# Nobita421/signature-Gan

Hardware: AMD Instinct MI355X
Metric: signature images/sec (G+D train step, bs64 64x64 z=100) (higher is better)
Workload: dtype f32; 1 GPU; configs[1]: reference conv G/D 64x64x1, z=100, batch 64 per GPU, f32, n_critic=1; global_batch=64, parallelism=dp1

## Files before the change

include/siggan.h:

```cpp
#ifndef SIGGAN_H
#define SIGGAN_H

#include <stddef.h>
#include <stdint.h>

#ifdef __cplusplus
extern "C" {
#endif

#define SIGGAN_ABI_VERSION 4

enum {
    SIGGAN_OK = 0,
    SIGGAN_E_INVALID = -1,
    SIGGAN_E_STATE = -2,
    SIGGAN_E_HIP = -3,
    SIGGAN_E_NOMEM = -4
};

typedef struct siggan_ctx siggan_ctx;

typedef struct siggan_config {
    int32_t device;
    int32_t latent_dim;
    int32_t image_size;
    int32_t image_channels;
    int32_t max_batch;
    float   dropout;
    float   leaky_slope;
    uint64_t seed;
    int32_t dtype;
    float   f16_grad_scale;
    int32_t spectral_norm;
    float   g_leaky_slope;
} siggan_config;
enum { SIGGAN_DTYPE_F32 = 0, SIGGAN_DTYPE_BF16 = 1, SIGGAN_DTYPE_F16 = 2 };

typedef struct siggan_storage {
    float *g_params, *g_grads, *g_exp_avg, *g_exp_avg_sq, *g_adam_steps;
    float *g_bn_running_mean, *g_bn_running_var;
    int64_t *g_bn_batches;
    float *d_params, *d_grads, *d_exp_avg, *d_exp_avg_sq, *d_adam_steps;
    float *d_sn_u, *d_sn_v;
} siggan_storage;

typedef struct siggan_hyper {
    double lr, beta1, beta2, eps;
    float label_smoothing;
    float clip_max_norm;
    float grad_scale;
} siggan_hyper;

enum {
    SIGGAN_M_D_LOSS = 0, SIGGAN_M_D_LOSS_REAL, SIGGAN_M_D_LOSS_FAKE, SIGGAN_M_D_REAL_MEAN,
    SIGGAN_M_D_FAKE_MEAN, SIGGAN_M_D_REAL_ACC, SIGGAN_M_D_FAKE_ACC, SIGGAN_M_D_GRAD_NORM,
    SIGGAN_M_G_LOSS, SIGGAN_M_G_FAKE_MEAN, SIGGAN_M_G_GRAD_NORM,
    SIGGAN_M_D_SKIPPED, SIGGAN_M_G_SKIPPED,
    SIGGAN_M_COUNT = 16
};

int siggan_abi_version(void);
const char *siggan_last_error(void);
int siggan_create(const siggan_config *cfg, siggan_ctx **out);
int siggan_destroy(siggan_ctx *ctx);

int64_t siggan_param_count(const siggan_ctx *ctx, int which);
int32_t siggan_param_tensors(const siggan_ctx *ctx, int which);
int siggan_param_span(const siggan_ctx *ctx, int which, int32_t idx, int64_t *offset, int64_t *numel);
int64_t siggan_bn_count(const siggan_ctx *ctx);
int64_t siggan_sn_count(const siggan_ctx *ctx, int which);
int32_t siggan_bn_layers(const siggan_ctx *ctx);
int64_t siggan_workspace_bytes(const siggan_ctx *ctx);

int siggan_bind(siggan_ctx *ctx, const siggan_storage *st);
int siggan_params_changed(siggan_ctx *ctx);
int siggan_seed(siggan_ctx *ctx, uint64_t seed, uint64_t offset);
int siggan_rng_state(siggan_ctx *ctx, uint64_t *seed, uint64_t *offset);
#define SIGGAN_MODE_GRAPH 1
#define SIGGAN_MODE_OVERLAP 2
int siggan_set_mode(siggan_ctx *ctx, int32_t mode);

enum { SIGGAN_STEP_TRAINER = 0, SIGGAN_STEP_ABLATION = 1 };
int siggan_set_step_variant(siggan_ctx *ctx, int32_t variant);

int siggan_g_forward(siggan_ctx *ctx, const float *z_dev, int32_t batch, int32_t training,
                     float *images_dev, void *stream);

int siggan_d_forward(siggan_ctx *ctx, const float *x_dev, int32_t batch, int32_t training,
                     const float *masks_dev, float *probs_dev, float *features_dev, void *stream);

int siggan_d_step(siggan_ctx *ctx, const float *real_dev, int32_t batch, const float *z_dev,
                  const float *masks_dev, const siggan_hyper *hp, float *metrics_dev,
                  float *metrics_host, void *stream);
int siggan_g_step(siggan_ctx *ctx, int32_t batch, const float *z_dev, const siggan_hyper *hp,
                  float *metrics_dev, float *metrics_host, void *stream);

#define SIGGAN_COMM_ID_BYTES 128
int siggan_comm_unique_id(void *id_out);
int siggan_comm_init(siggan_ctx *ctx, int32_t rank, int32_t world, const void *id);
int siggan_comm_destroy(siggan_ctx *ctx);
int32_t siggan_comm_world(const siggan_ctx *ctx);
int siggan_comm_broadcast(siggan_ctx *ctx, void *buf_dev, int64_t bytes, int32_t root, void *stream);

int siggan_d_grads(siggan_ctx *ctx, const float *real_dev, int32_t batch, const float *z_dev,
                   const float *masks_dev, const siggan_hyper *hp, float *metrics_dev, void *stream);
int siggan_step_begin(siggan_ctx *ctx, const float *real_dev, int32_t batch, const float *z_dev,
                      const float *masks_dev, const float *zg_dev, const siggan_hyper *hp,
                      float *metrics_dev, void *stream);
int siggan_stage_real(siggan_ctx *ctx, const float *real_dev, int32_t batch, void *stream);
int siggan_d_apply(siggan_ctx *ctx, const siggan_hyper *hp, float *metrics_dev, float *metrics_host,
                   void *stream);
int siggan_g_grads(siggan_ctx *ctx, int32_t batch, const float *z_dev, const siggan_hyper *hp,
                   float *metrics_dev, void *stream);
int siggan_g_apply(siggan_ctx *ctx, const siggan_hyper *hp, float *metrics_dev, float *metrics_host,
                   void *stream);

int siggan_op_conv4x4s2(siggan_ctx *ctx, int32_t form, const void *in_dev, const float *w_dev,
                        void *out_dev, int32_t batch, int32_t h_in, int32_t c_in, int32_t c_out,
                        void *stream);
int siggan_op_conv4x4s2_wgrad(siggan_ctx *ctx, const void *small_dev, const void *large_dev,
                              float *dw_dev, int32_t batch, int32_t h_small, int32_t c_small,
                              int32_t c_large, void *stream);
int siggan_op_adam(siggan_ctx *ctx, float *p_dev, float *g_dev, float *m_dev, float *v_dev,
                   int64_t n, int32_t step, const siggan_hyper *hp, void *stream);
int siggan_op_randn(siggan_ctx *ctx, float *out_dev, int64_t n, void *stream);
int siggan_augment_batch(int32_t device, const uint8_t *cache_dev, int64_t n_images, const int32_t *index_dev,
                         const int32_t *params_dev, const int16_t *tables_dev, const float *lut_dev,
                         float *out_dev, int32_t batch, int32_t size, int32_t augment, int32_t fill,
                         void *stream);
int siggan_device_info(int32_t device, int32_t *compute_units, int32_t *clock_khz, int64_t *hbm_bytes);
int siggan_prof_enable(siggan_ctx *ctx, int32_t on);
int32_t siggan_prof_slots(void);
int siggan_prof_read(siggan_ctx *ctx, int32_t idx, char *name, int32_t name_cap, int64_t *launches,
                     double *ms, double *flops, double *bytes);
int siggan_prof_launch(siggan_ctx *ctx, int64_t idx, int32_t *fields, int32_t n, int64_t *count);

int siggan_debug_tensor(siggan_ctx *ctx, const char *name, int32_t index, float *out_dev, int64_t n, void *stream);

#ifdef __cplusplus
}
#endif
#endif
```

signature-gan_amd/_lib.py:

```python
import ctypes as C
import os

import torch

_HERE = os.path.dirname(os.path.abspath(__file__))
LIB_PATH = os.environ.get("SIGGAN_LIB_PATH") or os.path.join(_HERE, "libsiggan_hip.so")
ABI_VERSION = 4
M_COUNT = 16
EPILOGUES = ("raw", "bias_lrelu_drop", "affine_relu", "lrelu_bwd", "bn_bwd_stats")
METRIC_INDEX = {"d_loss": 0, "d_loss_real": 1, "d_loss_fake": 2, "d_real_mean": 3, "d_fake_mean": 4,
                "d_real_acc": 5, "d_fake_acc": 6, "d_grad_norm": 7, "g_loss": 8, "g_fake_mean": 9,
                "g_grad_norm": 10, "d_skipped": 11, "g_skipped": 12}


class Config(C.Structure):
    _fields_ = [("device", C.c_int32), ("latent_dim", C.c_int32), ("image_size", C.c_int32),
                ("image_channels", C.c_int32), ("max_batch", C.c_int32), ("dropout", C.c_float),
                ("leaky_slope", C.c_float), ("seed", C.c_uint64), ("dtype", C.c_int32), ("f16_grad_scale", C.c_float),
                ("spectral_norm", C.c_int32), ("g_leaky_slope", C.c_float)]


DTYPES = {"f32": 0, "fp32": 0, "float32": 0, "bf16": 1, "bfloat16": 1, "f16": 2, "fp16": 2, "float16": 2}


class Storage(C.Structure):
    _fields_ = [(n, C.c_void_p) for n in (
        "g_params", "g_grads", "g_exp_avg", "g_exp_avg_sq", "g_adam_steps", "g_bn_running_mean",
        "g_bn_running_var", "g_bn_batches", "d_params", "d_grads", "d_exp_avg", "d_exp_avg_sq", "d_adam_steps",
        "d_sn_u", "d_sn_v")]


class Hyper(C.Structure):
    _fields_ = [("lr", C.c_double), ("beta1", C.c_double), ("beta2", C.c_double), ("eps", C.c_double),
                ("label_smoothing", C.c_float), ("clip_max_norm", C.c_float), ("grad_scale", C.c_float)]


class MlpConfig(C.Structure):
    _fields_ = [("device", C.c_int32), ("latent_dim", C.c_int32), ("image_size", C.c_int32), ("n_hidden", C.c_int32),
                ("hidden", C.c_int32 * 4), ("max_batch", C.c_int32), ("leaky_slope", C.c_float), ("seed", C.c_uint64)]


class MlpStorage(C.Structure):
    _fields_ = [(n, C.c_void_p) for n in (
        "g_params", "g_grads", "g_exp_avg", "g_exp_avg_sq", "g_adam_steps", "g_bn_running_mean",
        "g_bn_running_var", "g_bn_batches", "d_params", "d_grads", "d_exp_avg", "d_exp_avg_sq", "d_adam_steps")]


_P, _I32, _I64 = C.c_void_p, C.c_int32, C.c_int64
_SIGNATURES = {
    "siggan_abi_version": (C.c_int, []),
    "siggan_last_error": (C.c_char_p, []),
    "siggan_create": (C.c_int, [C.POINTER(Config), C.POINTER(_P)]),
    "siggan_destroy": (C.c_int, [_P]),
    "siggan_param_count": (_I64, [_P, C.c_int]),
    "siggan_param_tensors": (_I32, [_P, C.c_int]),
    "siggan_param_span": (C.c_int, [_P, C.c_int, _I32, C.POINTER(_I64), C.POINTER(_I64)]),
    "siggan_bn_count": (_I64, [_P]),
    "siggan_bn_layers": (_I32, [_P]),
    "siggan_sn_count": (_I64, [_P, C.c_int]),
    "siggan_workspace_bytes": (_I64, [_P]),
    "siggan_bind": (C.c_int, [_P, C.POINTER(Storage)]),
    "siggan_params_changed": (C.c_int, [_P]),
    "siggan_seed": (C.c_int, [_P, C.c_uint64, C.c_uint64]),
    "siggan_rng_state": (C.c_int, [_P, C.POINTER(C.c_uint64), C.POINTER(C.c_uint64)]),
    "siggan_set_mode": (C.c_int, [_P, _I32]),
    "siggan_set_step_variant": (C.c_int, [_P, _I32]),
    "siggan_g_forward": (C.c_int, [_P, _P, _I32, _I32, _P, _P]),
    "siggan_d_forward": (C.c_int, [_P, _P, _I32, _I32, _P, _P, _P, _P]),
    "siggan_d_step": (C.c_int, [_P, _P, _I32, _P, _P, C.POINTER(Hyper), _P, _P, _P]),
    "siggan_g_step": (C.c_int, [_P, _I32, _P, C.POINTER(Hyper), _P, _P, _P]),
    "siggan_d_grads": (C.c_int, [_P, _P, _I32, _P, _P, C.POINTER(Hyper), _P, _P]),
    "siggan_step_begin": (C.c_int, [_P, _P, _I32, _P, _P, _P, C.POINTER(Hyper), _P, _P]),
    "siggan_stage_real": (C.c_int, [_P, _P, _I32, _P]),
    "siggan_d_apply": (C.c_int, [_P, C.POINTER(Hyper), _P, _P, _P]),
    "siggan_g_grads": (C.c_int, [_P, _I32, _P, C.POINTER(Hyper), _P, _P]),
    "siggan_g_apply": (C.c_int, [_P, C.POINTER(Hyper), _P, _P, _P]),
    "siggan_op_conv4x4s2": (C.c_int, [_P, _I32, _P, _P, _P, _I32, _I32, _I32, _I32, _P]),
    "siggan_op_conv4x4s2_wgrad": (C.c_int, [_P, _P, _P, _P, _I32, _I32, _I32, _I32, _P]),
    "siggan_op_adam": (C.c_int, [_P, _P, _P, _P, _P, _I64, _I32, C.POINTER(Hyper), _P]),
    "siggan_op_randn": (C.c_int, [_P, _P, _I64, _P]),
    "siggan_augment_batch": (C.c_int, [_I32, _P, _I64, _P, _P, _P, _P, _P, _I32, _I32, _I32, _I32, _P]),
    "siggan_comm_unique_id": (C.c_int, [_P]),
    "siggan_comm_init": (C.c_int, [_P, _I32, _I32, _P]),
    "siggan_comm_destroy": (C.c_int, [_P]),
    "siggan_comm_world": (_I32, [_P]),
    "siggan_comm_broadcast": (C.c_int, [_P, _P, _I64, _I32, _P]),
    "siggan_device_info": (C.c_int, [_I32, C.POINTER(_I32), C.POINTER(_I32), C.POINTER(_I64)]),
    "siggan_prof_enable": (C.c_int, [_P, _I32]),
    "siggan_prof_slots": (_I32, []),
    "siggan_prof_launch": (C.c_int, [_P, _I64, C.POINTER(_I32), _I32, C.POINTER(_I64)]),
    "siggan_prof_read": (C.c_int, [_P, _I32, C.c_char_p, _I32, C.POINTER(_I64), C.POINTER(C.c_double), C.POINTER(C.c_double),
                                   C.POINTER(C.c_double)]),
    "siggan_debug_tensor": (C.c_int, [_P, C.c_char_p, _I32, _P, _I64, _P]),
    "mlpgan_create": (C.c_int, [C.POINTER(MlpConfig), C.POINTER(_P)]),
    "mlpgan_destroy": (C.c_int, [_P]),
    "mlpgan_param_count": (_I64, [_P, C.c_int]),
    "mlpgan_param_tensors": (_I32, [_P, C.c_int]),
    "mlpgan_bn_count": (_I64, [_P]),
    "mlpgan_bind": (C.c_int, [_P, C.POINTER(MlpStorage)]),
    "mlpgan_seed": (C.c_int, [_P, C.c_uint64, C.c_uint64]),
    "mlpgan_g_forward": (C.c_int, [_P, _P, _I32, _I32, _P, _P]),
    "mlpgan_d_forward": (C.c_int, [_P, _P, _I32, _P, _P]),
    "mlpgan_d_step": (C.c_int, [_P, _P, _I32, _P, C.POINTER(Hyper), _P, _P]),
    "mlpgan_g_step": (C.c_int, [_P, _I32, _P, C.POINTER(Hyper), _P, _P]),
    "mlpgan_op_gemm": (C.c_int, [_I32, _I32, _P, _P, _P, _I32, _I32, _I32, _P]),
}
EXPORTS = tuple(_SIGNATURES)

_lib = None


def load():
    global _lib
    if _lib is not None:
        return _lib
    if not os.path.exists(LIB_PATH):
        raise RuntimeError(
            f"{LIB_PATH} is missing: build it with `python -c 'import __graft_entry__ as g; g.build()'` "
            "(or `make -C signature-gan_amd/csrc`). This path has no CPU/PyTorch fallback.")
    lib = C.CDLL(LIB_PATH)
    for name, (res, args) in _SIGNATURES.items():
        fn = getattr(lib, name)
        fn.restype, fn.argtypes = res, args
    if lib.siggan_abi_version() != ABI_VERSION:
        raise RuntimeError(f"libsiggan_hip.so ABI {lib.siggan_abi_version()} != expected {ABI_VERSION}; rebuild")
    _lib = lib
    return lib


class SigganError(RuntimeError):
    pass


def check(rc):
    if rc == 0:
        return
    msg = load().siggan_last_error().decode("utf-8", "replace")
    if rc == -1:
        raise ValueError(msg)
    raise SigganError(f"siggan error {rc}: {msg}")
```

signature-gan_amd/csrc/gconv.h:

```cpp
#pragma once
#include <hip/hip_runtime.h>
#include <stdint.h>
#include <vector>

#include "act.h"

namespace siggan {

enum Epilogue : int {
    EPI_RAW = 0,
    EPI_BIAS_LRELU_DROP,
    EPI_AFFINE_RELU,
    EPI_LRELU_BWD,
    EPI_BN_BWD_STATS,
};

struct GConvArgs {
    int dt;
    const void* in;
    const void* wp;
    void* out;
    int B, Hi, Wi, Ci, Co;
    int lgHr, lgWr;
    int Ho, Wo;
    int form;
    int M;
    int epi;
    const float* bias;
    const float* noise;
    const float* scale;
    const float* shift;
    const void* aref;
    const float* bnp;
    float* stat0;
    float* stat1;
    int64_t stat_cap;
    const float* cls_w;
    float* cls_part;
    float slope;
    float gslope;
    float* slab;
    int64_t slab_floats;
    size_t slab_stride;
    const float* zeros;
};

struct BnBwdParams { f32x4 sc, sf, mu, rs; };
__device__ __forceinline__ BnBwdParams bn_bwd_params(const float* __restrict__ bnp, int Co, int co) {
    BnBwdParams q;
    q.sc = *reinterpret_cast<const f32x4*>(bnp + co); q.sf = *reinterpret_cast<const f32x4*>(bnp + Co + co);
    q.mu = *reinterpret_cast<const f32x4*>(bnp + 2 * Co + co); q.rs = *reinterpret_cast<const f32x4*>(bnp + 3 * Co + co);
    return q;
}
template <class T, bool LK>
__device__ __forceinline__ void bn_bwd_stat_terms(const f32x4 v, const f32x4 y, const BnBwdParams& q, float gs, f32x4& s0, f32x4& s1) {
#pragma unroll
    for (int e = 0; e < 4; ++e) {
        const float vq = (float)(T)v[e];
        const float d = g_dact<LK>(fmaf(y[e], q.sc[e], q.sf[e]), vq, gs);
        s0[e] += d;
        s1[e] = fmaf(d, (y[e] - q.mu[e]) * q.rs[e], s1[e]);
    }
}
__host__ __device__ inline bool gen_lk(const GConvArgs& a) {
    return a.gslope != 0.f && (a.epi == EPI_AFFINE_RELU || a.epi == EPI_BN_BWD_STATS);
}

struct WgradArgs {
    int dt;
    const void* S;
    const void* L;
    float* slab;
    float* dw;
    float* db;
    int B, Cs, Cl;
    int lgHs, lgWs, lgCl;
    int K;
    int kchunk;
    const float* zeros;
};

struct Prof {
    struct Rec {
        int id; double flops, bytes; hipEvent_t e0, e1;
        int form, epi_req, epi, M, Ci, Co;
    };
    static constexpr int NID = 8;
    std::vector<Rec> recs;
    static const char* name(int id);
    void begin(int id, double flops, double bytes, hipStream_t st);
    void shape(const GConvArgs& a, int epi_req);
    void clear();
};
extern Prof* g_prof;

int launch_gconv(const GConvArgs& a, hipStream_t st);
void launch_gconv16(int cfg, const GConvArgs& a, dim3 grid, hipStream_t st, hipEvent_t e0, hipEvent_t e1, int kq = 1);
void launch_wgrad16(bool small, const WgradArgs& a, dim3 grid, hipStream_t st, hipEvent_t e0, hipEvent_t e1);
int launch_wgrad(WgradArgs a, int max_splits, hipStream_t st);

}
```

signature-gan_amd/csrc/gconv.hip:

```cpp
#include "gconv.h"
#include <hip/hip_ext.h>

namespace siggan {


static constexpr int BK = 32;
static constexpr int PAD = 4;

__device__ __forceinline__ int xcd_remap(int bid, int nwg) {
    const int q = nwg >> 3, r = nwg & 7, xcd = bid & 7, idx = bid >> 3;
    return (xcd < r ? xcd * (q + 1) : r * (q + 1) + (xcd - r) * q) + idx;
}

template <int BM, int BN, int WM, int WN, int BK = 32, int DEEP = 0, int KQ = 1, bool LK = false>
__global__ __launch_bounds__(256 * KQ) void k_gconv(const GConvArgs a) {
    constexpr int TM = BM / (32 * WM), TN = BN / (32 * WN);
    constexpr int PA = BM / 32, PB = BN / 32;
    constexpr int KC = BK / 32;
    constexpr int LD = BK + 4;
    __shared__ __attribute__((aligned(16))) float smem[KQ * 2 * LD * (BM + BN)];
    const int quad = KQ > 1 ? (int)(threadIdx.x >> 8) : 0;
    float* const sA = smem + quad * (2 * LD * (BM + BN));
    float* const sB = sA + 2 * LD * BM;

    const int tid = threadIdx.x & 255, lane = tid & 63, wave = tid >> 6;
    const int li = lane & 31, lh = lane >> 5;
    const int wm = wave / WN, wn = wave % WN;
    const float* const a_in = static_cast<const float*>(a.in);
    const float* const a_wp = static_cast<const float*>(a.wp);

    const int tiles_n = a.Co / BN;
    const int bid = xcd_remap(blockIdx.x, gridDim.x);
    const int m0 = (bid / tiles_n) * BM, n0 = (bid % tiles_n) * BN;
    const int cls = blockIdx.z, ph = cls >> 1, pw = cls & 1;
    const int Hr = 1 << a.lgHr, Wr = 1 << a.lgWr;
    const int ntaps = a.form == 0 ? 16 : 4;
    const int Ktot = ntaps * a.Ci;
    const int lgcpt = 31 - __builtin_clz(a.Ci / BK);
    const int nk_all = ntaps << lgcpt;
    const int kper = (nk_all + gridDim.y * KQ - 1) / (gridDim.y * KQ);
    const int k_lo = (blockIdx.y * KQ + quad) * kper;
    const int k_hi = min(nk_all, k_lo + kper);
    const int nk = k_hi - k_lo;

    const int kc = tid & 7, rloc = tid >> 3;
    const float* a_base[PA];
    int a_ih0[PA], a_iw0[PA];
#pragma unroll
    for (int p = 0; p < PA; ++p) {
        const int m = m0 + rloc + 32 * p;
        if (m < a.M) {
            const int n = m >> (a.lgHr + a.lgWr);
            const int rh = (m >> a.lgWr) & (Hr - 1), rw = m & (Wr - 1);
            a_base[p] = a_in + (size_t)n * a.Hi * a.Wi * a.Ci + kc * 4;
            if (a.form == 0) { a_ih0[p] = 2 * rh - 1; a_iw0[p] = 2 * rw - 1; }
            else             { a_ih0[p] = rh + ph;    a_iw0[p] = rw + pw; }
        } else {
            a_base[p] = a_in; a_ih0[p] = -(1 << 20); a_iw0[p] = -(1 << 20);
        }
    }
    const float* wcur = a_wp + ((size_t)cls * a.Co + n0 + rloc) * Ktot + kc * 4 + (size_t)k_lo * BK;

    const float* a_cur[PA];
    int a_step[PA];
    int l_tap = k_lo >> lgcpt, l_cc = k_lo & ((1 << lgcpt) - 1);
    auto set_tap = [&]() __attribute__((always_inline)) {
        int dh, dw;
        if (a.form == 0) { dh = l_tap >> 2; dw = l_tap & 3; } else { dh = -(l_tap >> 1); dw = -(l_tap & 1); }
#pragma unroll
        for (int p = 0; p < PA; ++p) {
            const int ih = a_ih0[p] + dh, iw = a_iw0[p] + dw;
            const bool ok = (unsigned)ih < (unsigned)a.Hi && (unsigned)iw < (unsigned)a.Wi;
            a_cur[p] = ok ? a_base[p] + ((size_t)(ih * a.Wi + iw) * a.Ci + l_cc * BK) : a.zeros;
            a_step[p] = ok ? BK : 0;
        }
    };
    constexpr int NSET = DEEP ? 2 : 1;
    f32x4 ra[NSET][PA][KC], rb[NSET][PB][KC];
    auto load_tile = [&](int set = 0) __attribute__((always_inline)) {
#pragma unroll
        for (int p = 0; p < PA; ++p) {
#pragma unroll
            for (int q = 0; q < KC; ++q) ra[set][p][q] = *reinterpret_cast<const f32x4*>(a_cur[p] + 32 * q);
            a_cur[p] += a_step[p];
        }
#pragma unroll
        for (int p = 0; p < PB; ++p)
#pragma unroll
            for (int q = 0; q < KC; ++q) rb[set][p][q] = *reinterpret_cast<const f32x4*>(wcur + (size_t)(32 * p) * Ktot + 32 * q);
        wcur += BK;
        if (++l_cc == (1 << lgcpt)) { l_cc = 0; ++l_tap; set_tap(); }
    };
    auto store_tile = [&](int buf, int set = 0) __attribute__((always_inline)) {
        float* dA = sA + buf * LD * BM + rloc * LD + kc * 4;
        float* dB = sB + buf * LD * BN + rloc * LD + kc * 4;
#pragma unroll
        for (int p = 0; p < PA; ++p)
#pragma unroll
            for (int q = 0; q < KC; ++q) *reinterpret_cast<f32x4*>(dA + 32 * p * LD + 32 * q) = ra[set][p][q];
#pragma unroll
        for (int p = 0; p < PB; ++p)
#pragma unroll
            for (int q = 0; q < KC; ++q) *reinterpret_cast<f32x4*>(dB + 32 * p * LD + 32 * q) = rb[set][p][q];
    };

    f32x16 acc[TM][TN];
#pragma unroll
    for (int i = 0; i < TM; ++i)
#pragma unroll
        for (int j = 0; j < TN; ++j)
#pragma unroll
            for (int r = 0; r < 16; ++r) acc[i][j][r] = 0.f;

    if (DEEP && nk >= 5) {
        auto tile = [&](const int h, const int kt, const bool st, const bool ld) __attribute__((always_inline)) {
            const float* pA = sA + h * LD * BM + (wm * (32 * TM) + li) * LD + 4 * lh;
            const float* pB = sB + h * LD * BN + (wn * (32 * TN) + li) * LD + 4 * lh;
            f32x4 fa[2][TM], fb[2][TN];
#pragma unroll
            for (int i = 0; i < TM; ++i) fa[0][i] = *reinterpret_cast<const f32x4*>(pA + 32 * i * LD);
#pragma unroll
            for (int j = 0; j < TN; ++j) fb[0][j] = *reinterpret_cast<const f32x4*>(pB + 32 * j * LD);
#pragma unroll
            for (int c = 0; c < BK / 8; ++c) {
                const int cur = c & 1, nxt = cur ^ 1;
                if (c + 1 < BK / 8) {
#pragma unroll
                    for (int i = 0; i < TM; ++i) fa[nxt][i] = *reinterpret_cast<const f32x4*>(pA + 32 * i * LD + 8 * (c + 1));
#pragma unroll
                    for (int j = 0; j < TN; ++j) fb[nxt][j] = *reinterpret_cast<const f32x4*>(pB + 32 * j * LD + 8 * (c + 1));
                }
                __builtin_amdgcn_sched_barrier(0);
#pragma unroll
                for (int t = 0; t < 4; ++t)
#pragma unroll
                    for (int i = 0; i < TM; ++i)
#pragma unroll
                        for (int j = 0; j < TN; ++j)
                            acc[i][j] = __builtin_amdgcn_mfma_f32_32x32x2f32(fa[cur][i][t], fb[cur][j][t], acc[i][j], 0, 0, 0);
                if (c == 0 && st) store_tile(h ^ 1, h ^ 1);
                if (c == 1 && ld) load_tile(h ^ 1);
            }
            __syncthreads();
        };
        set_tap();
        load_tile(0);
        load_tile(1);
        store_tile(0, 0);
        load_tile(0);
        __syncthreads();
        int kt = 0;
        for (; kt + 4 < nk; kt += 2) {
            tile(0, kt, true, true);
            tile(1, kt + 1, true, true);
        }
        for (; kt < nk; kt += 2) {
            tile(0, kt, kt + 1 < nk, kt + 3 < nk);
            if (kt + 1 < nk) tile(1, kt + 1, kt + 2 < nk, kt + 4 < nk);
        }
    } else {
    if (nk > 0) {
        set_tap();
        load_tile();
        store_tile(0);
        if (nk > 1) load_tile();
    }
    __syncthreads();

    for (int kt = 0; kt < nk; ++kt) {
        const int buf = kt & 1;
        const float* pA = sA + buf * LD * BM + (wm * (32 * TM) + li) * LD + 4 * lh;
        const float* pB = sB + buf * LD * BN + (wn * (32 * TN) + li) * LD + 4 * lh;
        f32x4 fa[2][TM], fb[2][TN];
#pragma unroll
        for (int i = 0; i < TM; ++i) fa[0][i] = *reinterpret_cast<const f32x4*>(pA + 32 * i * LD);
#pragma unroll
        for (int j = 0; j < TN; ++j) fb[0][j] = *reinterpret_cast<const f32x4*>(pB + 32 * j * LD);
#pragma unroll
        for (int c = 0; c < BK / 8; ++c) {
            const int cur = c & 1, nxt = cur ^ 1;
            if (c + 1 < BK / 8) {
#pragma unroll
                for (int i = 0; i < TM; ++i) fa[nxt][i] = *reinterpret_cast<const f32x4*>(pA + 32 * i * LD + 8 * (c + 1));
#pragma unroll
                for (int j = 0; j < TN; ++j) fb[nxt][j] = *reinterpret_cast<const f32x4*>(pB + 32 * j * LD + 8 * (c + 1));
            }
            __builtin_amdgcn_sched_barrier(0);
#pragma unroll
            for (int t = 0; t < 4; ++t)
#pragma unroll
                for (int i = 0; i < TM; ++i)
#pragma unroll
                    for (int j = 0; j < TN; ++j)
                        acc[i][j] = __builtin_amdgcn_mfma_f32_32x32x2f32(fa[cur][i][t], fb[cur][j][t], acc[i][j], 0, 0, 0);
            if (c == 0 && kt + 1 < nk) store_tile(buf ^ 1);
            if (c == 1 && kt + 2 < nk) load_tile();
        }
        __syncthreads();
    }
    }

    float* const outp = gridDim.y > 1 ? a.slab + (size_t)blockIdx.y * a.slab_stride : static_cast<float*>(a.out);
    const int epi = gridDim.y > 1 ? (int)EPI_RAW : a.epi;
    constexpr int LDT = BN + 4;
    static_assert(BM * LDT <= 2 * LD * (BM + BN), "output tile must fit the staging buffers");
    float* const sT = smem;
    if (KQ > 1) {
        float* const red = smem + 2 * LD * (BM + BN);
        if (quad == 1) {
#pragma unroll
            for (int i = 0; i < TM; ++i)
#pragma unroll
                for (int j = 0; j < TN; ++j)
#pragma unroll
                    for (int r = 0; r < 16; ++r) red[(((wave * TM + i) * TN + j) * 16 + r) * 64 + lane] = acc[i][j][r];
        }
        __syncthreads();
        if (quad == 0) {
#pragma unroll
            for (int i = 0; i < TM; ++i)
#pragma unroll
                for (int j = 0; j < TN; ++j)
#pragma unroll
                    for (int r = 0; r < 16; ++r) acc[i][j][r] += red[(((wave * TM + i) * TN + j) * 16 + r) * 64 + lane];
        }
    }
    if (quad == 0) {
#pragma unroll
        for (int i = 0; i < TM; ++i)
#pragma unroll
            for (int j = 0; j < TN; ++j)
#pragma unroll
                for (int r = 0; r < 16; ++r)
                    sT[(wm * (32 * TM) + 32 * i + (r & 3) + 8 * (r >> 2) + 4 * lh) * LDT + wn * (32 * TN) + 32 * j + li] = acc[i][j][r];
    }
    __syncthreads();
    if (quad != 0 && epi != EPI_BN_BWD_STATS) return;
    constexpr int C4 = BN / 4, RPP = 256 / C4;
    const int c4 = tid % C4, r0 = tid / C4;
    const int co = n0 + c4 * 4;
    BnBwdParams bq;
    f32x4 st0 = {0.f, 0.f, 0.f, 0.f}, st1 = st0;
    if (epi == EPI_BN_BWD_STATS) bq = bn_bwd_params(a.bnp, a.Co, co);
    const f32x4 bias4 = epi == EPI_BIAS_LRELU_DROP ? *reinterpret_cast<const f32x4*>(a.bias + co) : f32x4{0.f, 0.f, 0.f, 0.f};
    f32x4 sc4 = {1.f, 1.f, 1.f, 1.f}, sh4 = {0.f, 0.f, 0.f, 0.f};
    if (epi == EPI_AFFINE_RELU) { sc4 = *reinterpret_cast<const f32x4*>(a.scale + co); sh4 = *reinterpret_cast<const f32x4*>(a.shift + co); }
    const bool use_noise = (epi == EPI_BIAS_LRELU_DROP || epi == EPI_LRELU_BWD) && a.noise != nullptr;
#pragma unroll
    for (int p = 0; p < BM / RPP; ++p) {
        const int row = r0 + RPP * p, m = m0 + row;
        if (m >= a.M || quad != 0) continue;
        const int n = m >> (a.lgHr + a.lgWr);
        size_t opix;
        if (a.form == 0) {
            opix = (size_t)m;
        } else {
            const int rh = (m >> a.lgWr) & (Hr - 1), rw = m & (Wr - 1);
            opix = ((size_t)n * a.Ho + 2 * rh + ph) * a.Wo + 2 * rw + pw;
        }
        const size_t o = opix * a.Co + co;
        f32x4 v = *reinterpret_cast<const f32x4*>(sT + row * LDT + c4 * 4);
        if (epi == EPI_BN_BWD_STATS) {
            bn_bwd_stat_terms<float, LK>(v, *reinterpret_cast<const f32x4*>(static_cast<const float*>(a.aref) + o), bq, a.gslope, st0, st1);
        } else if (epi == EPI_BIAS_LRELU_DROP) {
#pragma unroll
            for (int e = 0; e < 4; ++e) { float t = v[e] + bias4[e]; v[e] = t > 0.f ? t : t * a.slope; }
            if (use_noise) {
                const f32x4 nz = *reinterpret_cast<const f32x4*>(a.noise + (size_t)n * a.Co + co);
#pragma unroll
                for (int e = 0; e < 4; ++e) v[e] *= nz[e];
            }
        } else if (epi == EPI_AFFINE_RELU) {
#pragma unroll
            for (int e = 0; e < 4; ++e) v[e] = g_act<LK>(fmaf(v[e], sc4[e], sh4[e]), a.gslope);
        } else if (epi == EPI_LRELU_BWD) {
            const f32x4 ar = *reinterpret_cast<const f32x4*>(static_cast<const float*>(a.aref) + o);
#pragma unroll
            for (int e = 0; e < 4; ++e) v[e] *= ar[e] > 0.f ? 1.f : a.slope;
            if (use_noise) {
                const f32x4 nz = *reinterpret_cast<const f32x4*>(a.noise + (size_t)n * a.Co + co);
#pragma unroll
                for (int e = 0; e < 4; ++e) v[e] *= nz[e];
            }
        }
        *reinterpret_cast<f32x4*>(outp + o) = v;
    }
    if (epi == EPI_BN_BWD_STATS) {
        __syncthreads();
        if (quad == 0) {
            *reinterpret_cast<f32x4*>(sT + (size_t)tid * 8) = st0;
            *reinterpret_cast<f32x4*>(sT + (size_t)tid * 8 + 4) = st1;
        }
        __syncthreads();
        if (quad == 0 && r0 == 0) {
#pragma unroll 4
            for (int k = 1; k < RPP; ++k) {
                st0 += *reinterpret_cast<const f32x4*>(sT + (size_t)(k * C4 + c4) * 8);
                st1 += *reinterpret_cast<const f32x4*>(sT + (size_t)(k * C4 + c4) * 8 + 4);
            }
            const size_t prow = (size_t)cls * (gridDim.x / tiles_n) + bid / tiles_n;
            *reinterpret_cast<f32x4*>(a.stat0 + prow * a.Co + co) = st0;
            *reinterpret_cast<f32x4*>(a.stat1 + prow * a.Co + co) = st1;
        }
    }
}

template <int CI, bool LK>
__global__ __launch_bounds__(256) void k_gconv_up4(const GConvArgs a) {
    constexpr int BM = 128, BN = 32, LD = BK + 4, LP = CI + 4, NCC = CI / BK;
    constexpr int PATCH_PIX = 264;
    constexpr int SMEM = (PATCH_PIX * LP + 2 * 4 * BN * LD) > (BM * 4 * BN) ? (PATCH_PIX * LP + 2 * 4 * BN * LD) : (BM * 4 * BN);
    __shared__ __attribute__((aligned(16))) float smem[SMEM];
    float* const sP = smem;
    float* const sB = smem + PATCH_PIX * LP;
    const int tid = threadIdx.x, lane = tid & 63, wave = tid >> 6;
    const int li = lane & 31, lh = lane >> 5;
    const int m0 = xcd_remap(blockIdx.x, gridDim.x) * BM;
    const int Hr = 1 << a.lgHr, Wr = 1 << a.lgWr, Wp = Wr + 2;
    const int Ktot = 4 * CI;
    const int n_img = m0 >> (a.lgHr + a.lgWr), rh0 = (m0 >> a.lgWr) & (Hr - 1), rows = BM >> a.lgWr;

    {
        const float* const img = static_cast<const float*>(a.in) + (size_t)n_img * a.Hi * a.Wi * CI;
        const int nchunk = (rows + 2) * Wp * (CI / 4);
        constexpr int NI = (PATCH_PIX * (CI / 4) + 255) / 256;
        f32x4 v[NI];
#pragma unroll
        for (int q = 0; q < NI; ++q) {
            const int i = tid + 256 * q;
            const int pix = i / (CI / 4), ch = i - pix * (CI / 4);
            const int pr = pix / Wp, pc = pix - pr * Wp;
            const int ih = rh0 - 1 + pr, iw = pc - 1;
            const bool ok = i < nchunk && (unsigned)ih < (unsigned)a.Hi && (unsigned)iw < (unsigned)a.Wi;
            const float* src = ok ? img + ((size_t)ih * a.Wi + iw) * CI + ch * 4 : a.zeros;
            v[q] = *reinterpret_cast<const f32x4*>(src);
        }
#pragma unroll
        for (int q = 0; q < NI; ++q) {
            const int i = tid + 256 * q;
            if (i < nchunk) {
                const int pix = i / (CI / 4), ch = i - pix * (CI / 4);
                *reinterpret_cast<f32x4*>(sP + pix * LP + ch * 4) = v[q];
            }
        }
    }
    const int kc = tid & 7, rloc = tid >> 3;
    const float* const w_row = static_cast<const float*>(a.wp) + (size_t)rloc * Ktot + kc * 4;
    f32x4 rb[4];
    int l_k = 0;
    auto load_tile = [&]() __attribute__((always_inline)) {
        const int cls = l_k / NCC, cc = l_k - cls * NCC;
#pragma unroll
        for (int t = 0; t < 4; ++t)
            rb[t] = *reinterpret_cast<const f32x4*>(w_row + (size_t)cls * a.Co * Ktot + t * CI + cc * BK);
        ++l_k;
    };
    auto store_tile = [&](int buf) __attribute__((always_inline)) {
#pragma unroll
        for (int t = 0; t < 4; ++t)
            *reinterpret_cast<f32x4*>(sB + ((buf * 4 + t) * BN + rloc) * LD + kc * 4) = rb[t];
    };

    f32x16 acc[4];
#pragma unroll
    for (int cls = 0; cls < 4; ++cls)
#pragma unroll
        for (int r = 0; r < 16; ++r) acc[cls][r] = 0.f;

    load_tile();
    store_tile(0);
    load_tile();
    __syncthreads();

    const int ml = wave * 32 + li;
    const float* const pP = sP + (((ml >> a.lgWr) + 1) * Wp + (ml & (Wr - 1)) + 1) * LP + 4 * lh;

#pragma unroll
    for (int cls = 0; cls < 4; ++cls) {
        const int ph = cls >> 1, pw = cls & 1;
        for (int cc = 0; cc < NCC; ++cc) {
            const int kt = cls * NCC + cc, buf = kt & 1;
            const float* pA[4];
#pragma unroll
            for (int t = 0; t < 4; ++t) pA[t] = pP + ((ph - (t >> 1)) * Wp + (pw - (t & 1))) * LP + cc * BK;
            const float* pB = sB + (buf * 4 * BN + li) * LD + 4 * lh;
            f32x4 fa[2][4], fb[2][4];
#pragma unroll
            for (int t = 0; t < 4; ++t) {
                fa[0][t] = *reinterpret_cast<const f32x4*>(pA[t]);
                fb[0][t] = *reinterpret_cast<const f32x4*>(pB + t * BN * LD);
            }
#pragma unroll
            for (int c = 0; c < BK / 8; ++c) {
                const int cur = c & 1, nxt = cur ^ 1;
                if (c + 1 < BK / 8) {
#pragma unroll
                    for (int t = 0; t < 4; ++t) {
                        fa[nxt][t] = *reinterpret_cast<const f32x4*>(pA[t] + 8 * (c + 1));
                        fb[nxt][t] = *reinterpret_cast<const f32x4*>(pB + t * BN * LD + 8 * (c + 1));
                    }
                }
                __builtin_amdgcn_sched_barrier(0);
#pragma unroll
                for (int t = 0; t < 4; ++t)
#pragma unroll
                    for (int u = 0; u < 4; ++u)
                        acc[cls] = __builtin_amdgcn_mfma_f32_32x32x2f32(fa[cur][t][u], fb[cur][t][u], acc[cls], 0, 0, 0);
                if (c == 0 && kt + 1 < 4 * NCC) store_tile(buf ^ 1);
                if (c == 1 && kt + 2 < 4 * NCC) load_tile();
            }
            __syncthreads();
        }
    }

    const float sc = a.epi == EPI_AFFINE_RELU ? a.scale[li] : 1.f, sf = a.epi == EPI_AFFINE_RELU ? a.shift[li] : 0.f;
    const int Wo = 2 * Wr;
    float* const so = smem;
#pragma unroll
    for (int r = 0; r < 16; ++r) {
        const int mr = wave * 32 + (r & 3) + 8 * (r >> 2) + 4 * lh;
        const int rl = mr >> a.lgWr, rw = mr & (Wr - 1);
#pragma unroll
        for (int cls = 0; cls < 4; ++cls) {
            float v = acc[cls][r];
            if (a.epi == EPI_AFFINE_RELU) v = g_act<LK>(fmaf(v, sc, sf), a.gslope);
            so[(((2 * rl + (cls >> 1)) * Wo) + 2 * rw + (cls & 1)) * BN + li] = v;
        }
    }
    __syncthreads();
    f32x4* const dst = reinterpret_cast<f32x4*>(static_cast<float*>(a.out) + ((size_t)n_img * a.Ho + 2 * rh0) * a.Wo * BN);
    const f32x4* const src = reinterpret_cast<const f32x4*>(so);
#pragma unroll
    for (int q = 0; q < (BM * 4 * BN / 4) / 256; ++q) dst[q * 256 + tid] = src[q * 256 + tid];
}

template <class T, bool LK>
__global__ __launch_bounds__(256) void k_splitk_epilogue(const GConvArgs a, int nsplit, int64_t total4) {
    const int64_t i = (int64_t)blockIdx.x * 256 + threadIdx.x;
    if (a.epi == EPI_BN_BWD_STATS) {
        __shared__ __attribute__((aligned(16))) float sh[256 * 8];
        const int C4 = a.Co / 4, c4 = threadIdx.x & (C4 - 1);
        f32x4 s0 = {0.f, 0.f, 0.f, 0.f}, s1 = s0;
        if (i < total4) {
            const f32x4* sl = reinterpret_cast<const f32x4*>(a.slab);
            const size_t stride4 = a.slab_stride / 4;
            f32x4 v = sl[i];
            for (int z = 1; z < nsplit; ++z) v += sl[(size_t)z * stride4 + i];
            bn_bwd_stat_terms<T, LK>(v, ld4<T>(static_cast<const T*>(a.aref) + i * 4), bn_bwd_params(a.bnp, a.Co, c4 * 4), a.gslope, s0, s1);
            st4<T>(static_cast<T*>(a.out) + i * 4, v);
        }
        *reinterpret_cast<f32x4*>(sh + threadIdx.x * 8) = s0;
        *reinterpret_cast<f32x4*>(sh + threadIdx.x * 8 + 4) = s1;
        __syncthreads();
        if ((int)threadIdx.x < C4) {
            for (int k = 1; k < 256 / C4; ++k) {
                s0 += *reinterpret_cast<const f32x4*>(sh + (k * C4 + c4) * 8);
                s1 += *reinterpret_cast<const f32x4*>(sh + (k * C4 + c4) * 8 + 4);
            }
            *reinterpret_cast<f32x4*>(a.stat0 + (size_t)blockIdx.x * a.Co + c4 * 4) = s0;
            *reinterpret_cast<f32x4*>(a.stat1 + (size_t)blockIdx.x * a.Co + c4 * 4) = s1;
        }
        return;
    }
    if (i >= total4) return;
    const float4* sl = reinterpret_cast<const float4*>(a.slab);
    const size_t stride4 = a.slab_stride / 4;
    float4 v = sl[i];
    for (int z = 1; z < nsplit; ++z) {
        const float4 w = sl[(size_t)z * stride4 + i];
        v.x += w.x; v.y += w.y; v.z += w.z; v.w += w.w;
    }
    const int C4 = a.Co / 4;
    const int64_t per_img = (int64_t)C4 * a.Ho * a.Wo;
    const bool p2 = (C4 & (C4 - 1)) == 0 && (per_img & (per_img - 1)) == 0;
    const int c = (p2 ? (int)(i & (C4 - 1)) : (int)(i % C4)) * 4;
    const int64_t n = p2 ? i >> (63 - __builtin_clzll(per_img)) : i / per_img;
    float* e = reinterpret_cast<float*>(&v);
    if (a.epi == EPI_BIAS_LRELU_DROP) {
#pragma unroll
        for (int k = 0; k < 4; ++k) {
            float x = e[k] + a.bias[c + k];
            x = x > 0.f ? x : x * a.slope;
            if (a.noise) x *= a.noise[n * a.Co + c + k];
            e[k] = x;
        }
    } else if (a.epi == EPI_AFFINE_RELU) {
#pragma unroll
        for (int k = 0; k < 4; ++k) e[k] = g_act<LK>(fmaf(e[k], a.scale[c + k], a.shift[c + k]), a.gslope);
    } else if (a.epi == EPI_LRELU_BWD) {
        const f32x4 ar = ld4<T>(static_cast<const T*>(a.aref) + i * 4);
        const float* r = reinterpret_cast<const float*>(&ar);
#pragma unroll
        for (int k = 0; k < 4; ++k) {
            float x = e[k] * (r[k] > 0.f ? 1.f : a.slope);
            if (a.noise) x *= a.noise[n * a.Co + c + k];
            e[k] = x;
        }
    }
    st4<T>(static_cast<T*>(a.out) + i * 4, f32x4{v.x, v.y, v.z, v.w});
    if (a.cls_w) {
        __shared__ float shc[4];
        const f32x4 w4 = *reinterpret_cast<const f32x4*>(a.cls_w + (size_t)(p2 ? (i & (per_img - 1)) : (i % per_img)) * 4);
        float d = (float)(T)v.x * w4[0];
        d = fmaf((float)(T)v.y, w4[1], d); d = fmaf((float)(T)v.z, w4[2], d); d = fmaf((float)(T)v.w, w4[3], d);
#pragma unroll
        for (int o = 32; o > 0; o >>= 1) d += __shfl_down(d, o, 64);
        if ((threadIdx.x & 63) == 0) shc[threadIdx.x >> 6] = d;
        __syncthreads();
        if (threadIdx.x == 0) a.cls_part[blockIdx.x] = ((shc[0] + shc[1]) + shc[2]) + shc[3];
    }
}

Prof* g_prof = nullptr;

const char* Prof::name(int id) {
    static const char* n[NID] = {"k_gconv<128,128>", "k_gconv<128,64>", "k_gconv<64,64>", "k_gconv<128,32>",
                                 "k_wgrad<64,64>", "k_gconv_up4", "k_wgrad<32,128>", "?"};
    return n[id < 0 || id >= NID ? NID - 1 : id];
}
void Prof::begin(int id, double flops, double bytes, hipStream_t) {
    Rec r; r.id = id; r.flops = flops; r.bytes = bytes;
    r.form = r.epi_req = r.epi = r.M = r.Ci = r.Co = -1;
    (void)hipEventCreate(&r.e0); (void)hipEventCreate(&r.e1);
    recs.push_back(r);
}
void Prof::shape(const GConvArgs& a, int epi_req) {
    Rec& r = recs.back();
    r.form = a.form; r.epi_req = epi_req; r.epi = a.epi; r.M = a.M; r.Ci = a.Ci; r.Co = a.Co;
}
void Prof::clear() {
    for (auto& r : recs) { (void)hipEventDestroy(r.e0); (void)hipEventDestroy(r.e1); }
    recs.clear();
}

static double gconv_bytes(const GConvArgs& a) {
    const double es = (double)dt_size(a.dt);
    const double in = (double)a.B * a.Hi * a.Wi * a.Ci, out = (double)a.B * a.Ho * a.Wo * a.Co, w = 16.0 * a.Ci * a.Co;
    return es * (in + w + out * (a.epi == EPI_LRELU_BWD ? 2.0 : 1.0));
}
static double wgrad_bytes(const WgradArgs& a) {
    const double es = (double)dt_size(a.dt);
    return es * ((double)a.K * a.Cs + 4.0 * a.K * a.Cl) + 4.0 * 16.0 * a.Cs * a.Cl;
}

template <int BM, int BN, int WM, int WN, int BKT = 32, int DEEP = 0, int KQ = 1>
static int launch_cfg(const GConvArgs& a_in, hipStream_t st, int id, int nsplit) {
    GConvArgs a = a_in;
    const int tiles = ((a.M + BM - 1) / BM) * (a.Co / BN);
    const int ncls = a.form == 0 ? 1 : 4;
    const int64_t total4 = (int64_t)a.B * a.Ho * a.Wo * a.Co / 4;
    int rows = 0;
    if (a.epi == EPI_BN_BWD_STATS) {
        if (nsplit > 1 && (256 % (a.Co / 4)) != 0) nsplit = 1;
        rows = nsplit > 1 ? (int)((total4 + 255) / 256) : ((a.M + BM - 1) / BM) * ncls;
        if ((int64_t)2 * rows * a.Co > a.stat_cap) { a.epi = EPI_RAW; rows = 0; }
        else a.stat1 = a.stat0 + (size_t)rows * a.Co;
    }
    if (a.cls_w) {
        const int64_t per_img4 = (int64_t)a.Ho * a.Wo * a.Co / 4;
        if (nsplit > 1 && a.epi != EPI_BN_BWD_STATS && total4 % 256 == 0 && per_img4 % 256 == 0) rows = (int)(per_img4 / 256);
        else a.cls_w = nullptr;
    }
    dim3 grid(tiles, nsplit, ncls);
    if (g_prof) {
        g_prof->begin(id, 2.0 * a.M * a.Co * (double)((a.form == 0 ? 16 : 4) * a.Ci) * ncls, gconv_bytes(a), st);
        g_prof->shape(a, a_in.epi);
    }
    hipEvent_t e0 = g_prof ? g_prof->recs.back().e0 : nullptr, e1 = g_prof ? g_prof->recs.back().e1 : nullptr;
    if (a.dt != DT_F32) {
        launch_gconv16(id, a, grid, st, e0, e1, KQ);
    } else if (gen_lk(a)) {
        hipExtLaunchKernelGGL((k_gconv<BM, BN, WM, WN, BKT, DEEP, KQ, true>), grid, dim3(256 * KQ), 0, st, e0, e1, 0, a);
    } else if (g_prof) {
        hipExtLaunchKernelGGL((k_gconv<BM, BN, WM, WN, BKT, DEEP, KQ>), grid, dim3(256 * KQ), 0, st, e0, e1, 0, a);
    } else {
        hipLaunchKernelGGL((k_gconv<BM, BN, WM, WN, BKT, DEEP, KQ>), grid, dim3(256 * KQ), 0, st, a);
    }
    if (nsplit > 1)
        SIGGAN_GS_SWITCH(gen_lk(a) ? 1.f : 0.f, LK, SIGGAN_DT_SWITCH(a.dt, T, hipLaunchKernelGGL((k_splitk_epilogue<T, LK>),
            dim3((unsigned)((total4 + 255) / 256)), dim3(256), 0, st, a, nsplit, total4)));
    return rows;
}

int launch_gconv(const GConvArgs& a_in, hipStream_t st) {
    GConvArgs a = a_in;
    if (a.epi == EPI_BN_BWD_STATS && (a.stat0 == nullptr || a.stat_cap <= 0)) return -1;
    const int ncls = a.form == 0 ? 1 : 4;
    auto blocks = [&](int bm, int bn) { return ((a.M + bm - 1) / bm) * (a.Co / bn) * ncls; };
    const int nk = (a.form == 0 ? 16 : 4) * (a.Ci / BK);
    auto splits = [&](int nblk) {
        int ns = 1;
        if (a.slab && nblk < 384) {
            ns = (512 + nblk - 1) / nblk;
            if (ns > nk / 4) ns = nk / 4;
            if (ns > 8) ns = 8;
            const int64_t out_floats = (int64_t)a.B * a.Ho * a.Wo * a.Co;
            if (ns > 1 && (int64_t)ns * out_floats > a.slab_floats) ns = (int)(a.slab_floats / out_floats);
            if (ns < 1) ns = 1;
        }
        a.slab_stride = (size_t)a.B * a.Ho * a.Wo * a.Co;
        return ns;
    };
    if (a.Co >= 64) {
        if (a.Co >= 128 && blocks(128, 128) >= 512) return launch_cfg<128, 128, 2, 2, 32, 1>(a, st, 0, 1);
        const int ns = splits(blocks(64, 64));
        if (ns == 2 && (nk & 1) == 0) return launch_cfg<64, 64, 2, 2, 32, 1, 2>(a, st, 2, 1);
        if (ns == 4 && !a.cls_w && a.dt != DT_F32 && (nk & 1) == 0) return launch_cfg<64, 64, 2, 2, 32, 1, 2>(a, st, 2, 1);
        return launch_cfg<64, 64, 2, 2, 32, 1>(a, st, 2, ns);
    }
    if (a.dt == DT_F32 && a.form == 1 && a.Co == 32 && (a.epi == EPI_RAW || a.epi == EPI_AFFINE_RELU) && (a.Ci == 32 || a.Ci == 64) &&
        a.M / 128 >= (a.Ci == 32 ? 384 : 768) && a.M % 128 == 0 &&
        ((1 << (a.lgHr + a.lgWr)) % 128) == 0 && a.lgWr >= 4 && a.lgWr <= 6) {
        dim3 grid(a.M / 128);
        if (g_prof) {
            g_prof->begin(5, 2.0 * a.M * a.Co * (double)(4 * a.Ci) * 4, gconv_bytes(a), st);
            g_prof->shape(a, a.epi);
        }
        hipEvent_t e0 = g_prof ? g_prof->recs.back().e0 : nullptr, e1 = g_prof ? g_prof->recs.back().e1 : nullptr;
        if (gen_lk(a)) {
            if (a.Ci == 32) hipExtLaunchKernelGGL((k_gconv_up4<32, true>), grid, dim3(256), 0, st, e0, e1, 0, a);
            else hipExtLaunchKernelGGL((k_gconv_up4<64, true>), grid, dim3(256), 0, st, e0, e1, 0, a);
        } else {
            if (a.Ci == 32) hipExtLaunchKernelGGL((k_gconv_up4<32, false>), grid, dim3(256), 0, st, e0, e1, 0, a);
            else hipExtLaunchKernelGGL((k_gconv_up4<64, false>), grid, dim3(256), 0, st, e0, e1, 0, a);
        }
        return 0;
    }
    const int ns = splits(blocks(128, 32));
    return launch_cfg<128, 32, 4, 1, 32, 1>(a, st, 3, ns);
}

template <int BM, int BN, int WM, int WN>
__global__ __launch_bounds__(256) void k_wgrad(const WgradArgs a) {
    constexpr int TM = BM / (32 * WM), TN = BN / (32 * WN);
    constexpr int LDA = BM + PAD, LDB = BN + PAD;
    constexpr int CA = BM / 4, RA = 256 / CA, PA = BK / RA;
    constexpr int CB = BN / 4, RB = 256 / CB, PB = BK / RB;
    __shared__ __attribute__((aligned(16))) float smem[2 * BK * (LDA + LDB)];
    float* const sA = smem;
    float* const sB = smem + 2 * BK * LDA;

    const int tid = threadIdx.x, lane = tid & 63, wave = tid >> 6;
    const int li = lane & 31, lh = lane >> 5;
    const int wm = wave / WN, wn = wave % WN;
    const int N = 16 << a.lgCl;
    const int tiles_n = N / BN;
    const int lin = blockIdx.z * gridDim.x + blockIdx.x;
    const int lid = xcd_remap(lin, gridDim.x * gridDim.z);
    const int bx = lid % gridDim.x, bz = lid / gridDim.x;
    const int i0 = (bx / tiles_n) * BM, j0 = (bx % tiles_n) * BN;
    const int kbeg = bz * a.kchunk;
    const int kend = min(a.K, kbeg + a.kchunk);
    const int nk = (kend - kbeg + BK - 1) / BK;
    const int Hs = 1 << a.lgHs, Ws = 1 << a.lgWs, Hl = 2 * Hs, Wl = 2 * Ws, Cl = 1 << a.lgCl;

    const int ca = tid % CA, ka = tid / CA;
    const int cb = tid % CB, kb = tid / CB;
    const float* const a_S = static_cast<const float*>(a.S);
    const float* const a_L = static_cast<const float*>(a.L);
    const int jj = j0 + cb * 4, tap = jj >> a.lgCl, lch = jj & (Cl - 1);
    const int kh = tap >> 2, kw = tap & 3;

    f32x4 ra[2][PA], rb[2][PB];
    size_t a_off[PA];
    int a_pix[PA], b_pix[PB];
#pragma unroll
    for (int p = 0; p < PA; ++p) { a_pix[p] = kbeg + ka + RA * p; a_off[p] = (size_t)a_pix[p] * a.Cs + i0 + ca * 4; }
#pragma unroll
    for (int p = 0; p < PB; ++p) b_pix[p] = kbeg + kb + RB * p;
    const int a_adv = BK * a.Cs;
    const int lgWl = a.lgWs + 1;
#define WG_LOAD_TILE(KT, SET)                                                                         \
    {                                                                                                 \
        _Pragma("unroll") for (int p = 0; p < PA; ++p) {                                              \
            const float* src = a_pix[p] < kend ? a_S + a_off[p] : a.zeros;                            \
            ra[SET][p] = *reinterpret_cast<const f32x4*>(src);                                       \
            a_off[p] += a_adv; a_pix[p] += BK;                                                        \
        }                                                                                             \
        _Pragma("unroll") for (int p = 0; p < PB; ++p) {                                              \
            const int pix = b_pix[p];                                                                 \
            const int y = pix >> a.lgWs;                                              \
            const int ih = 2 * (y & (Hs - 1)) - 1 + kh, iw = 2 * (pix & (Ws - 1)) - 1 + kw;           \
            const bool ok = pix < kend && (unsigned)ih < (unsigned)Hl && (unsigned)iw < (unsigned)Wl; \
                          \
            const unsigned off = (((unsigned)(2 * y - 1 + kh) << lgWl) + (unsigned)iw) << a.lgCl;     \
            const float* src = ok ? a_L + ((size_t)off + lch) : a.zeros;                              \
            rb[SET][p] = *reinterpret_cast<const f32x4*>(src);                                       \
            b_pix[p] += BK;                                                                           \
        }                                                                                             \
    }
#define WG_STORE_TILE(BUF, SET)                                                                       \
    {                                                                                                 \
        _Pragma("unroll") for (int p = 0; p < PA; ++p)                                                \
            *reinterpret_cast<f32x4*>(sA + (BUF) * BK * LDA + (ka + RA * p) * LDA + ca * 4) = ra[SET][p]; \
        _Pragma("unroll") for (int p = 0; p < PB; ++p)                                                \
            *reinterpret_cast<f32x4*>(sB + (BUF) * BK * LDB + (kb + RB * p) * LDB + cb * 4) = rb[SET][p]; \
    }

    f32x16 acc[TM][TN];
#pragma unroll
    for (int i = 0; i < TM; ++i)
#pragma unroll
        for (int j = 0; j < TN; ++j)
#pragma unroll
            for (int r = 0; r < 16; ++r) acc[i][j][r] = 0.f;

    constexpr int NQ = 256 / BM, KQ = BK / NQ;
    const bool bias_blk = a.db != nullptr && j0 == 0;
    const int bcol = tid % BM, kq = tid / BM;
    float bsum = 0.f;
#define WG_TILE(BUF, ST, LD)                                                                          \
    {                                                                                                 \
        if (bias_blk) {                                                                               \
            const float* col = sA + (BUF) * BK * LDA + kq * KQ * LDA + bcol;                          \
            _Pragma("unroll") for (int k = 0; k < KQ; ++k) bsum += col[k * LDA];                      \
        }                                                                                             \
        const float* pA = sA + (BUF) * BK * LDA + lh * LDA + wm * (32 * TM) + li;                     \
        const float* pB = sB + (BUF) * BK * LDB + lh * LDB + wn * (32 * TN) + li;                     \
                          \
        float fa[2][4][TM], fb[2][4][TN];                                                             \
        _Pragma("unroll") for (int q = 0; q < 4; ++q) {                                               \
            _Pragma("unroll") for (int i = 0; i < TM; ++i) fa[0][q][i] = pA[(2 * q) * LDA + 32 * i];  \
            _Pragma("unroll") for (int j = 0; j < TN; ++j) fb[0][q][j] = pB[(2 * q) * LDB + 32 * j];  \
        }                                                                                             \
        _Pragma("unroll") for (int c = 0; c < BK / 8; ++c) {                                          \
            const int cur = c & 1, nxt = cur ^ 1;                                                     \
            if (c + 1 < BK / 8) {                                                                     \
                _Pragma("unroll") for (int q = 0; q < 4; ++q) {                                       \
                    _Pragma("unroll") for (int i = 0; i < TM; ++i) fa[nxt][q][i] = pA[(8 * c + 8 + 2 * q) * LDA + 32 * i]; \
                    _Pragma("unroll") for (int j = 0; j < TN; ++j) fb[nxt][q][j] = pB[(8 * c + 8 + 2 * q) * LDB + 32 * j]; \
                }                                                                                     \
            }                                                                                         \
            __builtin_amdgcn_sched_barrier(0);                                                        \
            _Pragma("unroll") for (int q = 0; q < 4; ++q)                                             \
                _Pragma("unroll") for (int i = 0; i < TM; ++i)                                        \
                    _Pragma("unroll") for (int j = 0; j < TN; ++j)                                    \
                        acc[i][j] = __builtin_amdgcn_mfma_f32_32x32x2f32(fa[cur][q][i], fb[cur][q][j], acc[i][j], 0, 0, 0); \
            if (c == 0) { ST }                                                                        \
            if (c == 1) { LD }                                                                        \
        }                                                                                             \
        __syncthreads();                                                                              \
    }
    if (nk >= 5) {
        WG_LOAD_TILE(0, 0)
        WG_LOAD_TILE(1, 1)
        WG_STORE_TILE(0, 0)
        WG_LOAD_TILE(2, 0)
        __syncthreads();
        int kt = 0;
        for (; kt + 4 < nk; kt += 2) {
            WG_TILE(0, WG_STORE_TILE(1, 1), WG_LOAD_TILE(kt + 3, 1))
            WG_TILE(1, WG_STORE_TILE(0, 0), WG_LOAD_TILE(kt + 4, 0))
        }
        for (; kt < nk; kt += 2) {
            WG_TILE(0, if (kt + 1 < nk) WG_STORE_TILE(1, 1), if (kt + 3 < nk) WG_LOAD_TILE(kt + 3, 1))
            if (kt + 1 < nk) WG_TILE(1, if (kt + 2 < nk) WG_STORE_TILE(0, 0), if (kt + 4 < nk) WG_LOAD_TILE(kt + 4, 0))
        }
    } else {
        if (nk > 0) {
            WG_LOAD_TILE(0, 0)
            WG_STORE_TILE(0, 0)
            if (nk > 1) WG_LOAD_TILE(1, 0)
        }
        __syncthreads();
        for (int kt = 0; kt < nk; ++kt) {
            if (kt & 1) WG_TILE(1, if (kt + 1 < nk) WG_STORE_TILE(0, 0), if (kt + 2 < nk) WG_LOAD_TILE(kt + 2, 0))
            else WG_TILE(0, if (kt + 1 < nk) WG_STORE_TILE(1, 0), if (kt + 2 < nk) WG_LOAD_TILE(kt + 2, 0))
        }
    }
#undef WG_TILE

#undef WG_LOAD_TILE
#undef WG_STORE_TILE
    if (bias_blk) {
        smem[kq * BM + bcol] = bsum;
        __syncthreads();
        if (tid < BM) {
            float t = smem[tid];
#pragma unroll
            for (int q = 1; q < NQ; ++q) t += smem[q * BM + tid];
            if (gridDim.z == 1) a.db[i0 + tid] = t;
            else a.slab[(size_t)gridDim.z * a.Cs * N + (size_t)bz * a.Cs + i0 + tid] = t;
        }
    }
    if (gridDim.z == 1 && a.dw) {
#pragma unroll
        for (int i = 0; i < TM; ++i)
#pragma unroll
            for (int r = 0; r < 16; ++r) {
                const int row = i0 + wm * (32 * TM) + 32 * i + (r & 3) + 8 * (r >> 2) + 4 * lh;
#pragma unroll
                for (int j = 0; j < TN; ++j) {
                    const int col = j0 + wn * (32 * TN) + 32 * j + li;
                    a.dw[((size_t)row * Cl + (col & (Cl - 1))) * 16 + (col >> a.lgCl)] = acc[i][j][r];
                }
            }
        return;
    }
    float* const out = a.slab + (size_t)bz * a.Cs * N;
#pragma unroll
    for (int i = 0; i < TM; ++i)
#pragma unroll
        for (int r = 0; r < 16; ++r) {
            const int row = i0 + wm * (32 * TM) + 32 * i + (r & 3) + 8 * (r >> 2) + 4 * lh;
#pragma unroll
            for (int j = 0; j < TN; ++j)
                out[(size_t)row * N + j0 + wn * (32 * TN) + 32 * j + li] = acc[i][j][r];
        }
}

static void launch_wgrad_reduce(const float* slab, float* dw, float* db, int nsplit, int Cs, int Cl, hipStream_t st);

int launch_wgrad(WgradArgs a, int max_splits, hipStream_t st) {
    const int N = 16 << a.lgCl;
    const bool small = a.Cs < 64;
    const int tiles = small ? (N / 128) : (a.Cs / 64) * (N / 64);
    int ktiles = (a.K + BK - 1) / BK;
    int nsplit = (512 + tiles - 1) / tiles;
    if (nsplit > ktiles / 4) nsplit = ktiles / 4;
    if (nsplit > max_splits) nsplit = max_splits;
    if (nsplit < 1) nsplit = 1;
    int per = (ktiles + nsplit - 1) / nsplit;
    a.kchunk = per * BK;
    nsplit = (ktiles + per - 1) / per;
    dim3 grid(tiles, 1, nsplit);
    if (g_prof) g_prof->begin(small ? 6 : 4, 2.0 * a.Cs * (double)N * a.K, wgrad_bytes(a), st);
    hipEvent_t e0 = g_prof ? g_prof->recs.back().e0 : nullptr, e1 = g_prof ? g_prof->recs.back().e1 : nullptr;
    if (a.dt != DT_F32) {
        launch_wgrad16(small, a, grid, st, e0, e1);
    } else if (g_prof) {
        if (small) hipExtLaunchKernelGGL((k_wgrad<32, 128, 1, 4>), grid, dim3(256), 0, st, e0, e1, 0, a);
        else hipExtLaunchKernelGGL((k_wgrad<64, 64, 2, 2>), grid, dim3(256), 0, st, e0, e1, 0, a);
    } else if (small) {
        hipLaunchKernelGGL((k_wgrad<32, 128, 1, 4>), grid, dim3(256), 0, st, a);
    } else {
        hipLaunchKernelGGL((k_wgrad<64, 64, 2, 2>), grid, dim3(256), 0, st, a);
    }
    if (nsplit > 1) launch_wgrad_reduce(a.slab, a.dw, a.db, nsplit, a.Cs, 1 << a.lgCl, st);
    return nsplit;
}

__global__ __launch_bounds__(1024) void k_wgrad_reduce(const float* __restrict__ slab, float* __restrict__ dw, float* __restrict__ db,
                                                       int nsplit, int Cs, int lgCl) {
    __shared__ float sh[16][64];
    const int N = 16 << lgCl, Cl = 1 << lgCl;
    const size_t total = (size_t)Cs * N;
    const int cl = threadIdx.x & 63, zl = threadIdx.x >> 6, SL = blockDim.x >> 6;
    const size_t wblocks = total / 64;
    const bool bias = blockIdx.x >= wblocks;
    const size_t idx = bias ? (size_t)(blockIdx.x - wblocks) * 64 + cl : (size_t)blockIdx.x * 64 + cl;
    const float* src = bias ? slab + (size_t)nsplit * total : slab;
    const size_t zstride = bias ? (size_t)Cs : total;
    const bool live = !bias || idx < (size_t)Cs;
    float acc = 0.f;
    if (live) {
#pragma unroll 8
        for (int z = zl; z < nsplit; z += SL) acc += src[(size_t)z * zstride + idx];
    }
    if (SL > 1) {
        sh[zl][cl] = acc;
        __syncthreads();
        if (zl != 0) return;
        for (int k = 1; k < SL; ++k) acc += sh[k][cl];
    }
    if (!live) return;
    if (bias) { db[idx] = acc; return; }
    const int j = (int)(idx & (size_t)(N - 1)), s_ = (int)(idx >> (4 + lgCl));
    const int tap = j >> lgCl, l = j & (Cl - 1);
    dw[((size_t)s_ * Cl + l) * 16 + tap] = acc;
}

static int ilog2(int v) { int l = 0; while ((1 << l) < v) ++l; return l; }

static void launch_wgrad_reduce(const float* slab, float* dw, float* db, int nsplit, int Cs, int Cl, hipStream_t st) {
    const size_t total = (size_t)Cs * 16 * Cl;
    int SL = 1;
    while (SL < 16 && SL < nsplit) SL *= 2;
    const unsigned blocks = (unsigned)(total / 64) + (db ? (unsigned)((Cs + 63) / 64) : 0u);
    hipLaunchKernelGGL(k_wgrad_reduce, dim3(blocks), dim3(64 * SL), 0, st, slab, dw, db, nsplit, Cs, ilog2(Cl));
}

}
```

signature-gan_amd/csrc/siggan.hip:

```cpp
#include <hip/hip_runtime.h>
#include <dlfcn.h>
#include <math.h>
#include <stdarg.h>
#include <stdio.h>
#include <stdlib.h>
#include <string.h>
#include <new>
#include <vector>

#include "../../include/siggan.h"
#include "gconv.h"
#include "ops.h"

using namespace siggan;

static thread_local char g_err[512] = "";
static int fail(int code, const char* fmt, ...) {
    va_list ap;
    va_start(ap, fmt);
    vsnprintf(g_err, sizeof g_err, fmt, ap);
    va_end(ap);
    return code;
}
int siggan_set_error(int code, const char* fmt, ...) {
    va_list ap;
    va_start(ap, fmt);
    vsnprintf(g_err, sizeof g_err, fmt, ap);
    va_end(ap);
    return code;
}
#define HIPCHK(x)                                                                                   \
    do {                                                                                            \
        hipError_t e_ = (x);                                                                        \
        if (e_ != hipSuccess) return fail(SIGGAN_E_HIP, "%s -> %s (%s:%d)", #x, hipGetErrorString(e_), __FILE__, __LINE__); \
    } while (0)
#define LAUNCHCHK()                                                                                 \
    do {                                                                                            \
        hipError_t e_ = hipGetLastError();                                                          \
        if (e_ != hipSuccess) return fail(SIGGAN_E_HIP, "kernel launch -> %s (%s:%d)", hipGetErrorString(e_), __FILE__, __LINE__); \
    } while (0)

struct DevGuard {
    int prev = -1, dev;
    hipError_t err = hipSuccess;
    explicit DevGuard(int d) : dev(d) {
        if (hipGetDevice(&prev) != hipSuccess) prev = -1;
        if (prev != dev) err = hipSetDevice(dev);
    }
    ~DevGuard() { if (prev >= 0 && prev != dev) (void)hipSetDevice(prev); }
};

static const float BN_MOMENTUM = 0.1f, BN_EPS = 1e-5f;
static const int MAXL = 6;
static const int64_t PARTIAL_FLOATS = (int64_t)2 << 20;
#define EV_FLAGS (hipEventDisableTiming | hipEventDisableSystemFence)
#define ENTER(c)                                                     \
    if (!(c)) return fail(SIGGAN_E_INVALID, "null context");          \
    DevGuard dg_((c)->cfg.device);                                    \
    HIPCHK(dg_.err)

static int ilog2i(int v) { int l = 0; while ((1 << l) < v) ++l; return l; }

typedef struct ncclComm* ncclComm_t;
typedef struct { char internal[128]; } ncclUniqueId_t;
enum { NCCL_SUCCESS = 0, NCCL_CHAR = 0, NCCL_FLOAT32 = 7, NCCL_SUM = 0 };
struct Rccl {
    void* h = nullptr;
    int (*GetUniqueId)(ncclUniqueId_t*) = nullptr;
    int (*CommInitRank)(ncclComm_t*, int, ncclUniqueId_t, int) = nullptr;
    int (*CommDestroy)(ncclComm_t) = nullptr;
    int (*AllReduce)(const void*, void*, size_t, int, int, ncclComm_t, hipStream_t) = nullptr;
    int (*Broadcast)(const void*, void*, size_t, int, int, ncclComm_t, hipStream_t) = nullptr;
    const char* (*GetErrorString)(int) = nullptr;
    const char* err = nullptr;
};
static Rccl* rccl() {
    static Rccl r;
    if (r.h || r.err) return &r;
    const char* names[] = {"librccl.so.1", "librccl.so"};
    for (const char* n : names) if (!r.h) r.h = dlopen(n, RTLD_NOW | RTLD_NOLOAD);
    for (const char* n : names) if (!r.h) r.h = dlopen(n, RTLD_NOW | RTLD_GLOBAL);
    if (!r.h) { r.err = "librccl.so was not found (load it, or import torch, before siggan_comm_*)"; return &r; }
    r.GetUniqueId = (decltype(r.GetUniqueId))dlsym(r.h, "ncclGetUniqueId");
    r.CommInitRank = (decltype(r.CommInitRank))dlsym(r.h, "ncclCommInitRank");
    r.CommDestroy = (decltype(r.CommDestroy))dlsym(r.h, "ncclCommDestroy");
    r.AllReduce = (decltype(r.AllReduce))dlsym(r.h, "ncclAllReduce");
    r.Broadcast = (decltype(r.Broadcast))dlsym(r.h, "ncclBroadcast");
    r.GetErrorString = (decltype(r.GetErrorString))dlsym(r.h, "ncclGetErrorString");
    if (!r.GetUniqueId || !r.CommInitRank || !r.CommDestroy || !r.AllReduce || !r.Broadcast || !r.GetErrorString)
        r.err = "librccl.so lacks one of ncclGetUniqueId / CommInitRank / CommDestroy / AllReduce / Broadcast / GetErrorString";
    return &r;
}
#define NCCLCHK(x)                                                                                  \
    do {                                                                                            \
        int e_ = (x);                                                                               \
        if (e_ != NCCL_SUCCESS) return fail(SIGGAN_E_HIP, "%s -> %s (%s:%d)", #x, rccl()->GetErrorString(e_), __FILE__, __LINE__); \
    } while (0)

struct PhaseKey {
    int phase, B, has_z, has_masks, g_dirty, d_dirty, spec_g, has_zg, pre_real, variant, coll;
    float* mt;
    double lr, beta1, beta2, eps;
    double fused_t;
    int pack;
    int ride;
    int rode;
    float ls, clip, gs;
    bool operator==(const PhaseKey& o) const {
        return phase == o.phase && B == o.B && has_z == o.has_z && has_masks == o.has_masks && g_dirty == o.g_dirty &&
               d_dirty == o.d_dirty && spec_g == o.spec_g && has_zg == o.has_zg && pre_real == o.pre_real && variant == o.variant && coll == o.coll && mt == o.mt && lr == o.lr && beta1 == o.beta1 && beta2 == o.beta2 && eps == o.eps && ls == o.ls &&
               clip == o.clip && gs == o.gs && fused_t == o.fused_t && pack == o.pack && ride == o.ride && rode == o.rode;
    }
};

struct siggan_ctx {
    siggan_config cfg;
    int S, latent, Lg, Ld, Bm;
    int dt;
    size_t es;
    bool sn;
    SnTable snt;
    float *sn_tbuf, *sn_wbuf, *sn_sig, *sn_us, *sn_vs, *sn_dots, *sn_g[2], *d_w1s;
    int variant;
    bool abl_masks;
    bool fc_fused;
    float gscale;
    int gC[MAXL + 1];
    int dC[MAXL + 1];
    int F;
    std::vector<int64_t> g_off, g_num, d_off, d_num;
    int64_t g_total, d_total, bn_total;
    int64_t g_bn_off[MAXL + 1];
    siggan_storage st;
    bool bound;
    bool g_dirty, d_dirty;
    char* ws; size_t ws_bytes;
    float *z, *g_bn[MAXL + 1], *g_bne[MAXL + 1];
    char *fc_y, *g_y[MAXL + 1], *g_a[MAXL + 1], *g_da[MAXL + 1];
    char *g_ae[MAXL + 1];
    float *img, *dpre;
    char *d_a[MAXL + 1], *d_dv[MAXL + 1];
    float *d_noise[MAXL + 1];
    float *logits, *probs, *dlogit;
    float* lparts;
    int lP[2];
    char *g_up[MAXL + 1], *g_dn[MAXL + 1], *d_dn[MAXL + 1], *d_up[MAXL + 1];
    float *wcp;
    float *slab, *slab_k, *slab_k2, *slab_k3, *partial, *partial_b, *partial_c, *z_g, *img_g, *metrics, *zeros, *wfc_t, *wfin_t, *d_w1t, *real_stage, *mask_stage;
    char *op_pack;
    int64_t slab_floats, slab_k_floats;
    DevState* dev;
    int pending;
    float* metrics_last;
    static constexpr int NEV = 96;
    int mode;
    hipStream_t s_m, s_a, s_b, s_c, s_n;
    hipEvent_t ev_gfwd, ev_dreal, ev_ar, ev_sys[2];
    bool early_ar;
    bool dreal_orphan;
    hipError_t lane_err;
    const char* refused;
    ncclComm_t comm; int comm_rank, comm_world; int comm_err;
    int staged_B;
    bool gfwd_joined;
    bool dreal_joined;
    bool dreal_noise2;
    float* slab_b;
    const float* staged_src;
    int dreal_B;
    int zg_stash;
    int g_fwd_pending;
    int conv1_rode;
    float* ride_ctr;
    unsigned* ride_late;
    unsigned* ride_late_dev;
    int g_rode, g_pre_real;
    double adam_t[2];
    bool adam_t_known[2];
    int g_r0;
    int ga_last_B;
    hipEvent_t ev[NEV], ev_fenced[NEV], ev_bridge[2];
    int evi;
    std::vector<std::pair<PhaseKey, hipGraphExec_t>> graphs;
};

static inline int gi_fc_w() { return 0; }
static inline int gi_fc_b() { return 1; }
static inline int gi_bn0_w() { return 2; }
static inline int gi_bn0_b() { return 3; }
static inline int gi_up_w(int l) { return 4 + 3 * (l - 1); }
static inline int gi_bn_w(int l) { return l == 0 ? 2 : 5 + 3 * (l - 1); }
static inline int gi_bn_b(int l) { return l == 0 ? 3 : 6 + 3 * (l - 1); }
static inline int gi_fin_w(const siggan_ctx* c) { return 4 + 3 * c->Lg; }
static inline int gi_fin_b(const siggan_ctx* c) { return 5 + 3 * c->Lg; }
static inline int di_w(int l) { return 2 * (l - 1); }
static inline int di_b(int l) { return 2 * (l - 1) + 1; }
static inline int di_cls_w(const siggan_ctx* c) { return 2 * c->Ld; }
static inline int di_cls_b(const siggan_ctx* c) { return 2 * c->Ld + 1; }

#define GP(c, i) ((c)->st.g_params + (c)->g_off[i])
#define GG(c, i) ((c)->st.g_grads + (c)->g_off[i])
#define DP(c, i) ((c)->st.d_params + (c)->d_off[i])
#define DG(c, i) ((c)->st.d_grads + (c)->d_off[i])

extern "C" int siggan_abi_version(void) { return SIGGAN_ABI_VERSION; }
extern "C" const char* siggan_last_error(void) { return g_err; }

static void build_layout(siggan_ctx* c) {
    static const int g64[] = {256, 128, 64, 32, 32}, g128[] = {512, 256, 128, 64, 32, 32};
    static const int d64[] = {1, 64, 128, 256, 512}, d128[] = {1, 64, 128, 256, 512, 512};
    if (c->S == 64) { c->Lg = 4; c->Ld = 4; memcpy(c->gC, g64, sizeof g64); memcpy(c->dC, d64, sizeof d64); }
    else            { c->Lg = 5; c->Ld = 5; memcpy(c->gC, g128, sizeof g128); memcpy(c->dC, d128, sizeof d128); }
    c->F = c->gC[0] * 16;
    auto push = [](std::vector<int64_t>& off, std::vector<int64_t>& num, int64_t& tot, int64_t n) {
        off.push_back(tot); num.push_back(n); tot += n;
    };
    c->g_total = 0;
    push(c->g_off, c->g_num, c->g_total, (int64_t)c->F * c->latent);
    push(c->g_off, c->g_num, c->g_total, c->F);
    push(c->g_off, c->g_num, c->g_total, c->F);
    push(c->g_off, c->g_num, c->g_total, c->F);
    for (int l = 1; l <= c->Lg; ++l) {
        push(c->g_off, c->g_num, c->g_total, (int64_t)c->gC[l - 1] * c->gC[l] * 16);
        push(c->g_off, c->g_num, c->g_total, c->gC[l]);
        push(c->g_off, c->g_num, c->g_total, c->gC[l]);
    }
    push(c->g_off, c->g_num, c->g_total, (int64_t)c->gC[c->Lg] * 9);
    push(c->g_off, c->g_num, c->g_total, 1);
    c->d_total = 0;
    for (int l = 1; l <= c->Ld; ++l) {
        push(c->d_off, c->d_num, c->d_total, (int64_t)c->dC[l] * c->dC[l - 1] * 16);
        push(c->d_off, c->d_num, c->d_total, c->dC[l]);
    }
    push(c->d_off, c->d_num, c->d_total, (int64_t)c->dC[c->Ld] * 16);
    push(c->d_off, c->d_num, c->d_total, 1);
    c->bn_total = 0;
    c->g_bn_off[0] = 0; c->bn_total = c->F;
    for (int l = 1; l <= c->Lg; ++l) { c->g_bn_off[l] = c->bn_total; c->bn_total += c->gC[l]; }
}

extern "C" int siggan_create(const siggan_config* cfg, siggan_ctx** out) {
    if (!cfg || !out) return fail(SIGGAN_E_INVALID, "null argument");
    if (cfg->image_size != 64 && cfg->image_size != 128)
        return fail(SIGGAN_E_INVALID, "output_size must be 64 or 128, got %d", cfg->image_size);
    if (cfg->image_channels != 1) return fail(SIGGAN_E_INVALID, "only image_channels == 1 is built, got %d", cfg->image_channels);
    if (cfg->latent_dim < 1 || cfg->latent_dim > 4096) return fail(SIGGAN_E_INVALID, "latent_dim out of range: %d", cfg->latent_dim);
    if (cfg->max_batch < 1 || cfg->max_batch > 4096) return fail(SIGGAN_E_INVALID, "max_batch out of range: %d", cfg->max_batch);
    if (!(cfg->dropout >= 0.f && cfg->dropout < 1.f)) return fail(SIGGAN_E_INVALID, "dropout must be in [0,1)");
    if (cfg->dtype != SIGGAN_DTYPE_F32 && cfg->dtype != SIGGAN_DTYPE_BF16 && cfg->dtype != SIGGAN_DTYPE_F16)
        return fail(SIGGAN_E_INVALID, "dtype must be SIGGAN_DTYPE_F32, _BF16 or _F16, got %d", cfg->dtype);
    if (!(cfg->f16_grad_scale >= 0.f) || cfg->f16_grad_scale > 65536.f)
        return fail(SIGGAN_E_INVALID, "f16_grad_scale must be in [0, 65536] (0 = default)");
    if (!(cfg->g_leaky_slope >= 0.f) || !isfinite(cfg->g_leaky_slope))
        return fail(SIGGAN_E_INVALID, "g_leaky_slope must be finite and >= 0 (0 = ReLU), got %g", (double)cfg->g_leaky_slope);
    DevGuard dg(cfg->device);
    HIPCHK(dg.err);
    siggan_ctx* c = new (std::nothrow) siggan_ctx();
    if (!c) return fail(SIGGAN_E_NOMEM, "out of host memory");
    c->cfg = *cfg; c->S = cfg->image_size; c->latent = cfg->latent_dim; c->Bm = cfg->max_batch;
    c->dt = cfg->dtype; c->es = dt_size(c->dt);
    c->fc_fused = cfg->max_batch <= 256 && (cfg->latent_dim & 3) == 0;
    c->variant = SIGGAN_STEP_TRAINER; c->abl_masks = false;
    c->sn = cfg->spectral_norm != 0;
    c->gscale = c->dt == DT_F16 ? (cfg->f16_grad_scale > 0.f ? cfg->f16_grad_scale : 1024.f) : 1.0f;
    c->bound = false; c->g_dirty = c->d_dirty = true; c->pending = 0; c->metrics_last = nullptr;
    build_layout(c);

    const int64_t Bm = c->Bm, Bd = 2 * Bm;
    size_t off = 0;
    char* base = nullptr;
    auto carve = [&](float** p, int64_t nfloats) {
        if (base) *p = (float*)(base + off);
        off += ((size_t)nfloats * sizeof(float) + 255) & ~(size_t)255;
    };
    auto carve_t = [&](char** p, int64_t nelem) {
        if (base) *p = base + off;
        off += ((size_t)nelem * c->es + 255) & ~(size_t)255;
    };
    c->slab_floats = (int64_t)16 << 20;
    c->slab_k_floats = (int64_t)16 << 20;
    for (int pass = 0; pass < 2; ++pass) {
        off = 0;
        carve(&c->z, Bm * c->latent);
        carve_t(&c->fc_y, Bm * c->F);
        for (int l = 0; l <= c->Lg; ++l) {
            const int64_t H = 4 << l, n = Bm * H * H * c->gC[l];
            if (l == 0) c->g_y[0] = c->fc_y; else carve_t(&c->g_y[l], n);
            carve_t(&c->g_a[l], n);
            if (c->dt != DT_F32) carve_t(&c->g_ae[l], n); else if (pass == 1) c->g_ae[l] = c->g_a[l];
            carve_t(&c->g_da[l], n);
            carve(&c->g_bn[l], 6 * (int64_t)(l == 0 ? c->F : c->gC[l]));
            carve(&c->g_bne[l], 4 * (int64_t)(l == 0 ? c->F : c->gC[l]));
        }
        if (pass == 1) c->g_y[0] = c->fc_y;
        carve(&c->img, Bm * c->S * c->S);
        carve(&c->dpre, Bm * c->S * c->S);
        for (int l = 1; l <= c->Ld; ++l) {
            const int64_t H = c->S >> l, n = Bd * H * H * c->dC[l];
            carve_t(&c->d_a[l], n);
            carve_t(&c->d_dv[l], n);
            carve(&c->d_noise[l], Bd * c->dC[l]);
        }
        carve(&c->logits, Bd); carve(&c->probs, Bd); carve(&c->dlogit, Bd);
        carve(&c->lparts, (int64_t)Bd * 16);
        for (int l = 1; l <= c->Lg; ++l) {
            carve_t(&c->g_up[l], (int64_t)c->gC[l - 1] * c->gC[l] * 16);
            carve_t(&c->g_dn[l], (int64_t)c->gC[l - 1] * c->gC[l] * 16);
        }
        for (int l = 2; l <= c->Ld; ++l) {
            carve_t(&c->d_dn[l], (int64_t)c->dC[l - 1] * c->dC[l] * 16);
            carve_t(&c->d_up[l], (int64_t)c->dC[l - 1] * c->dC[l] * 16);
        }
        carve(&c->wcp, (int64_t)c->dC[c->Ld] * 16);
        carve(&c->slab, c->slab_floats);
        carve(&c->slab_k, c->slab_k_floats);
        if (c->dt != DT_F32) carve(&c->slab_b, c->slab_floats); else if (pass == 1) c->slab_b = c->slab;
        carve(&c->slab_k2, c->slab_k_floats);
        if (c->dt != DT_F32) carve(&c->slab_k3, c->slab_k_floats); else if (pass == 1) c->slab_k3 = c->slab_k2;
        carve(&c->partial, PARTIAL_FLOATS);
        carve(&c->partial_b, PARTIAL_FLOATS);
        carve(&c->partial_c, PARTIAL_FLOATS);
        carve(&c->z_g, Bm * c->latent);
        carve(&c->img_g, Bm * c->S * c->S);
        carve(&c->real_stage, Bm * c->S * c->S);
        { int64_t sumC = 0; for (int l = 1; l <= c->Ld; ++l) sumC += c->dC[l]; carve(&c->mask_stage, 3 * Bm * sumC); }
        if (c->sn) {
            int64_t ut = 1, vt = (int64_t)c->dC[c->Ld] * 16;
            for (int l = 1; l <= c->Ld; ++l) { ut += c->dC[l]; vt += (int64_t)c->dC[l - 1] * 16; }
            carve(&c->sn_tbuf, vt); carve(&c->sn_wbuf, ut);
            carve(&c->sn_sig, 3 * 2 * SnTable::MAXS);
            carve(&c->sn_us, 3 * ut); carve(&c->sn_vs, 3 * vt);
            carve(&c->sn_dots, 2 * SnTable::MAXS * 64);
            carve(&c->sn_g[0], c->d_total); carve(&c->sn_g[1], c->d_total);
            carve(&c->d_w1s, (int64_t)c->dC[1] * 16);
        }
        carve(&c->metrics, SIGGAN_M_COUNT);
        carve_t(&c->op_pack, (int64_t)512 * 512 * 16);
        carve(&c->zeros, 64);
        carve(&c->wfc_t, (int64_t)c->F * c->latent);
        carve(&c->wfin_t, (int64_t)9 * c->gC[c->Lg]);
        carve(&c->d_w1t, (int64_t)16 * c->dC[1]);
        carve(&c->ride_ctr, 64);
        float* devp = nullptr;
        carve(&devp, 64);
        if (pass == 1) c->dev = (DevState*)devp;
        if (pass == 0) {
            c->ws_bytes = off;
            hipError_t e = hipMalloc((void**)&base, off);
            if (e != hipSuccess) { delete c; return fail(SIGGAN_E_NOMEM, "hipMalloc(%zu) -> %s", off, hipGetErrorString(e)); }
            c->ws = base;
        }
    }
    HIPCHK(hipMemset(c->ws, 0, c->ws_bytes));
    DevState h; memset(&h, 0, sizeof h);
    h.seed = cfg->seed; h.rng_ctr = 0; h.grad_mul = 1.f;
    HIPCHK(hipMemcpy(c->dev, &h, sizeof h, hipMemcpyHostToDevice));
    c->mode = SIGGAN_MODE_OVERLAP;
    c->evi = 0;
    HIPCHK(hipStreamCreateWithFlags(&c->s_m, hipStreamNonBlocking));
    HIPCHK(hipStreamCreateWithFlags(&c->s_a, hipStreamNonBlocking));
    HIPCHK(hipStreamCreateWithFlags(&c->s_b, hipStreamNonBlocking));
    HIPCHK(hipStreamCreateWithFlags(&c->s_c, hipStreamNonBlocking));
    HIPCHK(hipStreamCreateWithFlags(&c->s_n, hipStreamNonBlocking));
    HIPCHK(hipEventCreateWithFlags(&c->ev_gfwd, EV_FLAGS));
    HIPCHK(hipEventCreateWithFlags(&c->ev_dreal, EV_FLAGS));
    HIPCHK(hipEventCreateWithFlags(&c->ev_ar, hipEventDisableTiming));
    for (int i = 0; i < 2; ++i) HIPCHK(hipEventCreateWithFlags(&c->ev_sys[i], hipEventDisableTiming));
    c->early_ar = false;
    c->staged_B = c->dreal_B = 0; c->staged_src = nullptr; c->dreal_joined = c->dreal_noise2 = c->gfwd_joined = false;
    c->dreal_orphan = false; c->lane_err = hipSuccess;
    c->comm = nullptr; c->comm_rank = 0; c->comm_world = 1; c->comm_err = 0;
    c->g_fwd_pending = 0; c->conv1_rode = 0;
    c->g_rode = c->g_pre_real = 0;
    HIPCHK(hipHostMalloc((void**)&c->ride_late, sizeof(unsigned), hipHostMallocCoherent | hipHostMallocMapped));
    *c->ride_late = 0u;
    HIPCHK(hipHostGetDevicePointer((void**)&c->ride_late_dev, c->ride_late, 0));
    c->zg_stash = 0;
    c->ga_last_B = 0; c->g_r0 = 0;
    c->adam_t_known[0] = c->adam_t_known[1] = false;
    for (int i = 0; i < siggan_ctx::NEV; ++i) HIPCHK(hipEventCreateWithFlags(&c->ev[i], EV_FLAGS));
    for (int i = 0; i < siggan_ctx::NEV; ++i) HIPCHK(hipEventCreateWithFlags(&c->ev_fenced[i], hipEventDisableTiming));
    for (int i = 0; i < 2; ++i) HIPCHK(hipEventCreateWithFlags(&c->ev_bridge[i], hipEventDisableTiming));
    *out = c;
    return SIGGAN_OK;
}

extern "C" int siggan_destroy(siggan_ctx* c) {
    if (!c) return SIGGAN_OK;
    DevGuard dg(c->cfg.device);
    (void)hipDeviceSynchronize();
    if (c->comm) { (void)rccl()->CommDestroy(c->comm); c->comm = nullptr; }
    for (auto& e : c->graphs) (void)hipGraphExecDestroy(e.second);
    for (int i = 0; i < siggan_ctx::NEV; ++i) if (c->ev[i]) (void)hipEventDestroy(c->ev[i]);
    for (int i = 0; i < siggan_ctx::NEV; ++i) if (c->ev_fenced[i]) (void)hipEventDestroy(c->ev_fenced[i]);
    for (int i = 0; i < 2; ++i) if (c->ev_bridge[i]) (void)hipEventDestroy(c->ev_bridge[i]);
    if (c->s_m) (void)hipStreamDestroy(c->s_m);
    if (c->s_a) (void)hipStreamDestroy(c->s_a);
    if (c->s_b) (void)hipStreamDestroy(c->s_b);
    if (c->s_c) (void)hipStreamDestroy(c->s_c);
    if (c->s_n) (void)hipStreamDestroy(c->s_n);
    if (c->ev_ar) (void)hipEventDestroy(c->ev_ar);
    for (int i = 0; i < 2; ++i) if (c->ev_sys[i]) (void)hipEventDestroy(c->ev_sys[i]);
    if (c->ev_gfwd) (void)hipEventDestroy(c->ev_gfwd);
    if (c->ev_dreal) (void)hipEventDestroy(c->ev_dreal);
    if (c->ws) (void)hipFree(c->ws);
    if (c->ride_late) (void)hipHostFree(c->ride_late);
    delete c;
    return SIGGAN_OK;
}

extern "C" int64_t siggan_param_count(const siggan_ctx* c, int which) { return !c ? -1 : (which == 0 ? c->g_total : c->d_total); }
extern "C" int32_t siggan_param_tensors(const siggan_ctx* c, int which) {
    return !c ? -1 : (int32_t)(which == 0 ? c->g_off.size() : c->d_off.size());
}
extern "C" int siggan_param_span(const siggan_ctx* c, int which, int32_t idx, int64_t* offset, int64_t* numel) {
    if (!c || !offset || !numel) return fail(SIGGAN_E_INVALID, "null argument");
    const auto& o = which == 0 ? c->g_off : c->d_off;
    const auto& n = which == 0 ? c->g_num : c->d_num;
    if (idx < 0 || idx >= (int32_t)o.size()) return fail(SIGGAN_E_INVALID, "tensor index %d out of range", idx);
    *offset = o[idx]; *numel = n[idx];
    return SIGGAN_OK;
}
extern "C" int64_t siggan_bn_count(const siggan_ctx* c) { return c ? c->bn_total : -1; }
extern "C" int64_t siggan_sn_count(const siggan_ctx* c, int which) {
    if (!c) return -1;
    int64_t ut = 1, vt = (int64_t)c->dC[c->Ld] * 16;
    for (int l = 1; l <= c->Ld; ++l) { ut += c->dC[l]; vt += (int64_t)c->dC[l - 1] * 16; }
    return which == 0 ? ut : vt;
}
extern "C" int32_t siggan_bn_layers(const siggan_ctx* c) { return c ? c->Lg + 1 : -1; }
extern "C" int64_t siggan_workspace_bytes(const siggan_ctx* c) { return c ? (int64_t)c->ws_bytes : -1; }

static void drop_dreal(siggan_ctx* c) {
    if (c->dreal_B) { c->dreal_orphan = true; c->dreal_B = 0; }
}
static int settle(siggan_ctx* c, hipStream_t s) {
    if (c->dreal_orphan) {
        HIPCHK(hipStreamWaitEvent(s, c->ev_dreal, 0));
        c->dreal_orphan = false;
    }
    return SIGGAN_OK;
}

extern "C" int siggan_bind(siggan_ctx* c, const siggan_storage* st) {
    if (!c || !st) return fail(SIGGAN_E_INVALID, "null argument");
    const void* need[] = {st->g_params, st->g_bn_running_mean, st->g_bn_running_var, st->d_params};
    for (const void* p : need)
        if (!p) return fail(SIGGAN_E_INVALID, "siggan_bind: parameters and BatchNorm buffers are required");
    const void* all[] = {st->g_params, st->g_grads, st->g_exp_avg, st->g_exp_avg_sq, st->d_params, st->d_grads,
                         st->d_exp_avg, st->d_exp_avg_sq};
    for (const void* p : all)
        if (((uintptr_t)p & 15) != 0) return fail(SIGGAN_E_INVALID, "siggan_bind: arenas must be 16-byte aligned");
    c->st = *st;
    if (c->sn) {
        if (!st->d_sn_u || !st->d_sn_v) return fail(SIGGAN_E_INVALID, "siggan_bind: a spectral-norm context needs d_sn_u / d_sn_v");
        SnTable& t = c->snt; memset(&t, 0, sizeof t);
        t.n = c->Ld + 1;
        int uo = 0, vo = 0;
        t.pre_k[0] = t.pre_r[0] = 0;
        for (int i = 0; i < t.n; ++i) {
            SnLayer& L = t.layer[i];
            const bool cls = i == c->Ld;
            const int pi = cls ? di_cls_w(c) : di_w(i + 1);
            L.W = st->d_params + c->d_off[pi]; L.w_off = c->d_off[pi];
            L.rows = cls ? 1 : c->dC[i + 1]; L.K = cls ? c->dC[c->Ld] * 16 : c->dC[i] * 16;
            L.u_off = uo; L.v_off = vo; uo += L.rows; vo += L.K;
            t.pre_k[i + 1] = t.pre_k[i] + (L.K + 255) / 256;
            t.pre_r[i + 1] = t.pre_r[i] + (L.rows + 3) / 4;
        }
        t.u = st->d_sn_u; t.v = st->d_sn_v; t.tbuf = c->sn_tbuf; t.wbuf = c->sn_wbuf; t.sig = c->sn_sig;
        t.u_saved = c->sn_us; t.v_saved = c->sn_vs; t.dots = c->sn_dots; t.u_total = uo; t.v_total = vo;
    }
    c->bound = true; c->g_dirty = c->d_dirty = true; c->pending = 0; c->staged_B = 0; c->conv1_rode = 0;
    c->adam_t_known[0] = c->adam_t_known[1] = false;
    c->early_ar = false;
    drop_dreal(c);
    return SIGGAN_OK;
}
extern "C" int siggan_params_changed(siggan_ctx* c) {
    if (!c) return fail(SIGGAN_E_INVALID, "null context");
    c->g_dirty = c->d_dirty = true;
    c->conv1_rode = 0;
    c->adam_t_known[0] = c->adam_t_known[1] = false;
    c->early_ar = false;
    drop_dreal(c);
    return SIGGAN_OK;
}
extern "C" int siggan_seed(siggan_ctx* c, uint64_t seed, uint64_t offset) {
    if (!c) return fail(SIGGAN_E_INVALID, "null context");
    DevGuard dg_(c->cfg.device); HIPCHK(dg_.err);
    unsigned long long v[2] = {seed, offset};
    HIPCHK(hipMemcpy(c->dev, v, sizeof v, hipMemcpyHostToDevice));
    drop_dreal(c);
    return SIGGAN_OK;
}

extern "C" int siggan_rng_state(siggan_ctx* c, uint64_t* seed, uint64_t* offset) {
    ENTER(c);
    if (!seed || !offset) return fail(SIGGAN_E_INVALID, "null argument");
    HIPCHK(hipDeviceSynchronize());
    unsigned long long v[2];
    HIPCHK(hipMemcpy(v, c->dev, sizeof v, hipMemcpyDeviceToHost));
    *seed = v[0]; *offset = v[1];
    return SIGGAN_OK;
}

static int check_bn_batch(const siggan_ctx* c, int batch) {
    if (batch == 1)
        return fail(SIGGAN_E_INVALID, "Expected more than 1 value per channel when training, got input size torch.Size([1, %d])", c->F);
    return SIGGAN_OK;
}
static int check_call(siggan_ctx* c, int batch, bool need_bound = true) {
    if (!c) return fail(SIGGAN_E_INVALID, "null context");
    if (need_bound && !c->bound) return fail(SIGGAN_E_STATE, "siggan_bind has not been called");
    if (batch < 1 || batch > c->Bm) return fail(SIGGAN_E_INVALID, "batch %d outside [1, max_batch=%d]", batch, c->Bm);
    return SIGGAN_OK;
}

static void repack(siggan_ctx* c, hipStream_t sg, hipStream_t sd, bool do_g, bool do_d, int sn_slot = 0, const float* conv1_x = nullptr,
                   int conv1_r0 = 0, int conv1_B = 0) {
    if (do_g) {
        PrepTable t; t.njobs = 0; t.overflow = 0;
        PrepJob j; memset(&j, 0, sizeof j);
        if (!c->fc_fused) {
            j.type = PREP_FC_T; j.O = c->latent; j.I = c->gC[0]; j.src = GP(c, gi_fc_w()); j.dst = c->wfc_t;
            prep_add(t, j, (long long)c->latent * c->F);
        }
        for (int l = 1; l <= c->Lg; ++l) {
            const long long n = (long long)c->gC[l - 1] * c->gC[l] * 16;
            memset(&j, 0, sizeof j);
            j.src = GP(c, gi_up_w(l)); j.dt = c->dt;
            j.type = PREP_PACK_UP; j.I = c->gC[l - 1]; j.O = c->gC[l]; j.dst = (float*)c->g_up[l];
            prep_add(t, j, n);
            j.type = PREP_PACK_DOWN; j.O = c->gC[l - 1]; j.I = c->gC[l]; j.dst = (float*)c->g_dn[l];
            prep_add(t, j, n);
        }
        for (int l = 0; l <= c->Lg; ++l) {
            const int C = l == 0 ? c->F : c->gC[l];
            memset(&j, 0, sizeof j);
            j.type = PREP_BN_EVAL; j.O = C; j.perm = l == 0 ? c->gC[0] : 0;
            j.src = GP(c, gi_bn_w(l)); j.src2 = GP(c, gi_bn_b(l));
            j.src3 = c->st.g_bn_running_mean + c->g_bn_off[l]; j.src4 = c->st.g_bn_running_var + c->g_bn_off[l];
            j.dst = c->g_bne[l];
            prep_add(t, j, C);
        }
        memset(&j, 0, sizeof j);
        j.type = PREP_TAPS; j.I = 9; j.O = c->gC[c->Lg]; j.src = GP(c, gi_fin_w(c)); j.dst = c->wfin_t;
        prep_add(t, j, 9 * j.O);
        if (!launch_prepare(t, BN_EPS, sg)) c->lane_err = hipErrorInvalidValue;
    }
    if (do_d) {
        PrepTable t; t.njobs = 0; t.overflow = 0;
        PrepJob j;
        for (int l = 2; l <= c->Ld; ++l) {
            const long long n = (long long)c->dC[l - 1] * c->dC[l] * 16;
            memset(&j, 0, sizeof j);
            j.src = DP(c, di_w(l)); j.dt = c->dt;
            if (c->sn) j.mul = c->sn_sig + (sn_slot * 2 + 1) * SnTable::MAXS + (l - 1);
            j.type = PREP_PACK_DOWN; j.O = c->dC[l]; j.I = c->dC[l - 1]; j.dst = (float*)c->d_dn[l];
            prep_add(t, j, n);
            j.type = PREP_PACK_UP; j.I = c->dC[l]; j.O = c->dC[l - 1]; j.dst = (float*)c->d_up[l];
            prep_add(t, j, n);
        }
        memset(&j, 0, sizeof j);
        j.type = PREP_CLS; j.O = c->dC[c->Ld]; j.src = DP(c, di_cls_w(c)); j.dst = c->wcp;
        if (c->sn) j.mul = c->sn_sig + (sn_slot * 2 + 1) * SnTable::MAXS + c->Ld;
        prep_add(t, j, (long long)c->dC[c->Ld] * 16);
        if (c->sn) {
            memset(&j, 0, sizeof j);
            j.type = PREP_SCALE; j.O = c->dC[1] * 16; j.src = DP(c, di_w(1)); j.dst = c->d_w1s;
            j.mul = c->sn_sig + (sn_slot * 2 + 1) * SnTable::MAXS;
            prep_add(t, j, j.O);
        }
        memset(&j, 0, sizeof j);
        j.type = PREP_TAPS; j.I = 16; j.O = c->dC[1]; j.src = DP(c, di_w(1)); j.dst = c->d_w1t;
        if (c->sn) j.mul = c->sn_sig + (sn_slot * 2 + 1) * SnTable::MAXS;
        prep_add(t, j, j.O * 16);
        bool ok;
        if (conv1_x && !c->sn) {
            const int64_t H = c->S >> 1;
            char* out = c->d_a[1] + (size_t)((int64_t)conv1_r0 * H * H * c->dC[1]) * c->es;
            ok = launch_prepare_conv1(t, BN_EPS, c->dt, conv1_x, DP(c, di_w(1)), DP(c, di_b(1)), c->cfg.leaky_slope, out, conv1_B, c->S, sd);
        } else {
            ok = launch_prepare(t, BN_EPS, sd);
        }
        if (!ok) c->lane_err = hipErrorInvalidValue;
    }
}

static bool ap_table_g(siggan_ctx* c, ApTable& t) {
    if (!c->fc_fused || c->gC[c->Lg] * 9 > 1024) return false;
    for (int l = 0; l <= c->Lg; ++l) if (c->gC[l] % 16) return false;
    t.njobs = 0; t.overflow = 0;
    ApJob j;
    memset(&j, 0, sizeof j);
    j.type = AP_FLAT; j.off = c->g_off[gi_fc_w()]; j.n = c->g_num[gi_fc_w()] + c->g_num[gi_fc_b()];
    ap_add(t, j);
    for (int l = 0; l <= c->Lg; ++l) {
        if (l > 0) {
            memset(&j, 0, sizeof j);
            j.type = AP_CONV; j.A = c->gC[l - 1]; j.Bc = c->gC[l]; j.dt = c->dt; j.off = c->g_off[gi_up_w(l)];
            j.dst = (float*)c->g_dn[l]; j.dst2 = (float*)c->g_up[l];
            ap_add(t, j);
        }
        memset(&j, 0, sizeof j);
        j.type = AP_BN; j.A = l == 0 ? c->F : c->gC[l]; j.Bc = l == 0 ? c->gC[0] : 0;
        j.off = c->g_off[gi_bn_w(l)]; j.off2 = c->g_off[gi_bn_b(l)];
        j.rmean = c->st.g_bn_running_mean + c->g_bn_off[l]; j.rvar = c->st.g_bn_running_var + c->g_bn_off[l];
        j.dst = c->g_bne[l];
        ap_add(t, j);
    }
    memset(&j, 0, sizeof j);
    j.type = AP_TAPS; j.A = c->gC[c->Lg]; j.Bc = 9; j.off = c->g_off[gi_fin_w(c)]; j.n = 9 * c->gC[c->Lg];
    j.off2 = c->g_off[gi_fin_b(c)]; j.n2 = 1; j.dst = c->wfin_t;
    ap_add(t, j);
    return !t.overflow;
}
static bool ap_table_d(siggan_ctx* c, ApTable& t, int nride) {
    if (c->sn || c->dC[1] * 16 > 1024 || c->dC[1] > 256) return false;
    for (int l = 1; l <= c->Ld; ++l) if (c->dC[l] % 16) return false;
    t.njobs = 0; t.overflow = 0;
    ApJob j;
    memset(&j, 0, sizeof j);
    j.type = AP_TAPS; j.A = c->dC[1]; j.Bc = 16; j.off = c->d_off[di_w(1)]; j.n = 16 * c->dC[1];
    j.off2 = c->d_off[di_b(1)]; j.n2 = c->dC[1]; j.dst = c->d_w1t; j.wait = nride;
    ap_add(t, j);
    for (int l = 2; l <= c->Ld; ++l) {
        memset(&j, 0, sizeof j);
        j.type = AP_CONV; j.A = c->dC[l]; j.Bc = c->dC[l - 1]; j.dt = c->dt; j.off = c->d_off[di_w(l)];
        j.dst = (float*)c->d_dn[l]; j.dst2 = (float*)c->d_up[l];
        ap_add(t, j);
        memset(&j, 0, sizeof j);
        j.type = AP_FLAT; j.off = c->d_off[di_b(l)]; j.n = c->dC[l];
        ap_add(t, j);
    }
    memset(&j, 0, sizeof j);
    j.type = AP_T16; j.A = c->dC[c->Ld]; j.off = c->d_off[di_cls_w(c)]; j.dst = c->wcp;
    ap_add(t, j);
    memset(&j, 0, sizeof j);
    j.type = AP_FLAT; j.off = c->d_off[di_cls_b(c)]; j.n = 1;
    ap_add(t, j);
    return !t.overflow;
}

static int lane_check(siggan_ctx* c) {
    if (c->comm_err)
        return fail(SIGGAN_E_HIP, "ncclAllReduce of the gradient bucket failed (the optimiser update was skipped): %s",
                    rccl()->GetErrorString(c->comm_err));
    if (c->ride_late && __atomic_load_n(c->ride_late, __ATOMIC_ACQUIRE))
        return fail(SIGGAN_E_STATE, "riders did not report: the optimiser update's owner of the first Discriminator block stopped "
                                    "waiting for them (a G step's first block may have used twice-updated weights)");
    if (c->refused) return fail(SIGGAN_E_STATE, "%s", c->refused);
    if (c->lane_err == hipSuccess) return SIGGAN_OK;
    const hipError_t e = c->lane_err; c->lane_err = hipSuccess;
    return fail(SIGGAN_E_HIP, "an event record / stream wait / prepare table of the step failed: %s", hipGetErrorString(e));
}
struct Lanes {
    siggan_ctx* c;
    hipStream_t m, a, b;
    bool ext;
    hipEvent_t tail_wait;
    hipEvent_t fork_event(hipStream_t to) { return (ext && to != m) ? next() : nullptr; }
    void fork_after(hipStream_t to, hipEvent_t done) {
        if (to == m) return;
        if (done) note(hipStreamWaitEvent(to, done, 0)); else fork(to);
    }
    hipEvent_t next() { hipEvent_t e = (c->comm ? c->ev_fenced : c->ev)[c->evi]; c->evi = (c->evi + 1) % siggan_ctx::NEV; return e; }
    void fork(hipStream_t to) {
        if (to == m) return;
        hipEvent_t e = next();
        note(hipEventRecord(e, m)); note(hipStreamWaitEvent(to, e, 0));
    }
    void join(hipStream_t from) {
        if (from == m) return;
        hipEvent_t e = next();
        note(hipEventRecord(e, from)); note(hipStreamWaitEvent(m, e, 0));
    }
    void note(hipError_t e) { if (e != hipSuccess && c->lane_err == hipSuccess) c->lane_err = e; }
    void record(hipEvent_t e, hipStream_t s) { note(hipEventRecord(e, s)); }
    void wait(hipStream_t s, hipEvent_t e) { note(hipStreamWaitEvent(s, e, 0)); }
};

static GConvArgs gconv_args(siggan_ctx* c) {
    GConvArgs a; memset(&a, 0, sizeof a);
    a.dt = c->dt; a.gslope = c->cfg.g_leaky_slope;
    a.slab = c->slab_k; a.slab_floats = c->slab_k_floats; a.zeros = c->zeros;
    return a;
}

static void g_forward_pass(siggan_ctx* c, const float* z, int B, bool training, float* img, hipStream_t s,
                           float* partial = nullptr, float* slab_k = nullptr, uint32_t rng_sid = 0, float* z_out = nullptr,
                           hipEvent_t done = nullptr) {
    if (!partial) partial = c->partial;
    char* const* const A = training ? c->g_a : c->g_ae;
    const float gs = c->cfg.g_leaky_slope;
    if (c->fc_fused && launch_fc_fwd_fused(c->dt, z, GP(c, gi_fc_w()), GP(c, gi_fc_b()), c->fc_y, A[0], GP(c, gi_bn0_w()),
                                          GP(c, gi_bn0_b()), c->st.g_bn_running_mean, c->st.g_bn_running_var, c->st.g_bn_batches,
                                          c->g_bn[0], training ? nullptr : c->g_bne[0], z_out, c->dev, rng_sid, B, c->latent,
                                          c->gC[0], BN_MOMENTUM, BN_EPS, gs, s)) {
    } else if (!training) {
        launch_fc_fwd(c->dt, z, c->wfc_t, GP(c, gi_fc_b()), A[0], B, c->latent, c->gC[0], gs, s, c->g_bne[0], c->dev, rng_sid, z_out);
    } else {
        launch_fc_fwd(c->dt, z, c->wfc_t, GP(c, gi_fc_b()), c->fc_y, B, c->latent, c->gC[0], gs, s, nullptr, c->dev, rng_sid, z_out);
        launch_bn_train_stats(c->dt, c->fc_y, B, c->F, GP(c, gi_bn0_w()), GP(c, gi_bn0_b()), c->st.g_bn_running_mean,
                              c->st.g_bn_running_var, c->st.g_bn_batches, c->g_bn[0], partial, c->gC[0], BN_MOMENTUM,
                              BN_EPS, s);
        launch_bn_relu(c->dt, c->fc_y, A[0], B, c->F, c->g_bn[0], gs, s);
    }
    for (int l = 1; l <= c->Lg; ++l) {
        const int Hi = 4 << (l - 1), Ci = c->gC[l - 1], Co = c->gC[l];
        GConvArgs a = gconv_args(c);
        if (slab_k) a.slab = slab_k;
        a.in = A[l - 1]; a.wp = c->g_up[l]; a.B = B; a.Hi = Hi; a.Wi = Hi; a.Ci = Ci; a.Co = Co;
        a.lgHr = ilog2i(Hi); a.lgWr = a.lgHr; a.Ho = 2 * Hi; a.Wo = 2 * Hi; a.form = 1; a.M = B * Hi * Hi;
        const int C = Co;
        const int64_t off = c->g_bn_off[l];
        if (training) {
            a.out = c->g_y[l]; a.epi = EPI_RAW;
            launch_gconv(a, s);
            const int64_t R = (int64_t)B * 4 * Hi * Hi;
            launch_bn_train_stats(c->dt, c->g_y[l], R, C, GP(c, gi_bn_w(l)), GP(c, gi_bn_b(l)), c->st.g_bn_running_mean + off,
                                  c->st.g_bn_running_var + off, c->st.g_bn_batches + l, c->g_bn[l], partial, 0,
                                  BN_MOMENTUM, BN_EPS, s);
            if (l < c->Lg) launch_bn_relu(c->dt, c->g_y[l], A[l], R, C, c->g_bn[l], gs, s);
        } else {
            a.out = A[l]; a.epi = EPI_AFFINE_RELU; a.scale = c->g_bne[l]; a.shift = c->g_bne[l] + C;
            launch_gconv(a, s);
        }
    }
    if (training)
        launch_final_fwd(c->dt, c->g_y[c->Lg], c->wfin_t, GP(c, gi_fin_b(c)), img, B, c->S, c->gC[c->Lg], gs, s, c->g_bn[c->Lg], done);
    else
        launch_final_fwd(c->dt, A[c->Lg], c->wfin_t, GP(c, gi_fin_b(c)), img, B, c->S, c->gC[c->Lg], gs, s, nullptr, done);
    c->ga_last_B = training ? B : 0;
}

static void d_forward_rows(siggan_ctx* c, const float* x, int r0, int nB, bool dropout, hipStream_t s, float* slab_k,
                           bool fuse_cls = false, bool conv1_done = false) {
    const float slope = c->cfg.leaky_slope;
    auto act = [&](int l) { const int64_t H = c->S >> l; return c->d_a[l] + (size_t)((int64_t)r0 * H * H * c->dC[l]) * c->es; };
    auto nz = [&](int l) { return dropout ? c->d_noise[l] + (int64_t)r0 * c->dC[l] : nullptr; };
    if (!conv1_done)
        launch_conv1_fwd(c->dt, x, nB, x, c->sn ? c->d_w1s : DP(c, di_w(1)), DP(c, di_b(1)), nz(1), slope, act(1), nB, c->S, c->dC[1], s);
    for (int l = 2; l <= c->Ld; ++l) {
        const int Hi = c->S >> (l - 1), Ho = Hi / 2;
        GConvArgs a = gconv_args(c);
        a.slab = slab_k;
        a.in = act(l - 1); a.wp = c->d_dn[l]; a.out = act(l);
        a.B = nB; a.Hi = Hi; a.Wi = Hi; a.Ci = c->dC[l - 1]; a.Co = c->dC[l];
        a.lgHr = ilog2i(Ho); a.lgWr = a.lgHr; a.Ho = Ho; a.Wo = Ho; a.form = 0; a.M = nB * Ho * Ho;
        a.epi = EPI_BIAS_LRELU_DROP; a.bias = DP(c, di_b(l)); a.noise = nz(l); a.slope = slope;
        const int P_max = c->dC[c->Ld] * 16 / 1024;
        if (l == c->Ld && fuse_cls && P_max >= 1 && P_max <= 16) { a.cls_w = c->wcp; a.cls_part = c->lparts + (size_t)r0 * P_max; }
        const int P = launch_gconv(a, s);
        if (l == c->Ld) c->lP[r0 == 0 ? 0 : 1] = a.cls_w ? P : 0;
    }
    if (c->lP[r0 == 0 ? 0 : 1] == 0)
        launch_cls_fwd(c->dt, act(c->Ld), c->wcp, DP(c, di_cls_b(c)), c->logits + r0, nB, c->dC[c->Ld] * 16, s);
}

struct BceSpec { int n0; float y0, y1; float* mt; int is_g; };

static void d_backward_pass(siggan_ctx* c, Lanes& L, const float* x0, int n0, const float* x1, int Bd, bool dropout,
                            bool want_wgrad, bool want_dimage, const BceSpec& bce, int r0 = 0, float* garena = nullptr,
                            bool early_allreduce = false) {
    const float slope = c->cfg.leaky_slope;
    const int Ld = c->Ld;
    float* const ga = garena ? garena : c->st.d_grads;
    auto G_ = [&](int i) { return ga + c->d_off[i]; };
    auto act = [&](int l) { const int64_t H = c->S >> l; return c->d_a[l] + (size_t)((int64_t)r0 * H * H * c->dC[l]) * c->es; };
    auto dvp = [&](int l) { const int64_t H = c->S >> l; return c->d_dv[l] + (size_t)((int64_t)r0 * H * H * c->dC[l]) * c->es; };
    auto nz = [&](int l) { return dropout ? c->d_noise[l] + (int64_t)r0 * c->dC[l] : nullptr; };
    hipStream_t const sb = want_wgrad ? L.b : L.m;
    const int hP = c->lP[r0 == 0 ? 0 : 1];
    const int P = (r0 == 0 && Bd > bce.n0 && bce.n0 > 0 && c->lP[1] != hP) ? -1 : hP;
    if (P < 0) { c->lane_err = hipErrorInvalidValue; return; }
    const float* const parts = P ? c->lparts + (size_t)r0 * P : nullptr;
    const float* const bc = DP(c, di_cls_b(c));
    if (sb != L.m) {
        L.fork(L.b);
        launch_bce(c->logits + r0, Bd, bce.n0, bce.y0, bce.y1, c->probs + r0, c->dlogit + r0, bce.mt, bce.is_g, sb, c->gscale, parts, P, bc);
    }
    launch_cls_bwd(c->dt, c->logits + r0, bce.n0, bce.y0, bce.y1, c->wcp, act(Ld), nz(Ld), slope, dvp(Ld), Bd,
                   c->dC[Ld], L.m, c->gscale, c->probs + r0, c->dlogit + r0, bce.mt, bce.is_g, sb == L.m, parts, P, bc);
    if (want_wgrad)
        launch_cls_wgrad(c->dt, c->dlogit + r0, act(Ld), G_(di_cls_w(c)), G_(di_cls_b(c)), Bd, c->dC[Ld], sb);
    for (int l = Ld; l >= 2; --l) {
        const int Ho = c->S >> l, Hi = 2 * Ho, Co = c->dC[l], Ci = c->dC[l - 1];
        const bool w_main = want_wgrad && l == 2 && c->dt != DT_F32 && garena == nullptr;
        auto wgrad_l = [&](hipStream_t st, float* slab) {
            WgradArgs w; memset(&w, 0, sizeof w); w.zeros = c->zeros; w.dt = c->dt;
            w.S = dvp(l); w.L = act(l - 1); w.slab = slab; w.dw = G_(di_w(l)); w.B = Bd; w.Cs = Co; w.Cl = Ci;
            w.lgHs = ilog2i(Ho); w.lgWs = w.lgHs; w.lgCl = ilog2i(Ci); w.K = Bd * Ho * Ho;
            w.db = G_(di_b(l));
            const int max_splits = (int)(c->slab_floats / ((int64_t)Co * (16 * Ci + 1)));
            launch_wgrad(w, max_splits, st);
        };
        if (want_wgrad && !w_main) {
            L.fork(L.a);
            wgrad_l(L.a, c->slab);
            if (early_allreduce && l == Ld && c->comm && !c->comm_err && garena == nullptr) {
                hipEvent_t ea = c->ev_sys[0], eb = c->ev_sys[1];
                L.record(ea, L.a); L.record(eb, sb);
                L.wait(c->s_n, ea); L.wait(c->s_n, eb);
                const int64_t o = c->d_off[di_w(l)];
                const int rc = rccl()->AllReduce(ga + o, ga + o, (size_t)(c->d_total - o), NCCL_FLOAT32, NCCL_SUM, c->comm, c->s_n);
                if (rc != NCCL_SUCCESS) c->comm_err = rc;
                else { L.record(c->ev_ar, c->s_n); c->early_ar = true; }
            }
        }
        GConvArgs a = gconv_args(c);
        a.in = dvp(l); a.wp = c->d_up[l]; a.out = dvp(l - 1);
        a.B = Bd; a.Hi = Ho; a.Wi = Ho; a.Ci = Co; a.Co = Ci;
        a.lgHr = ilog2i(Ho); a.lgWr = a.lgHr; a.Ho = Hi; a.Wo = Hi; a.form = 1; a.M = Bd * Ho * Ho;
        a.epi = EPI_LRELU_BWD; a.aref = act(l - 1); a.noise = nz(l - 1); a.slope = slope;
        launch_gconv(a, L.m);
        if (w_main) {
            L.fork(L.b);
            launch_conv1_wgrad(c->dt, dvp(1), x0, n0, x1, G_(di_w(1)), G_(di_b(1)), c->partial_b, Bd, c->S, c->dC[1], L.b);
            wgrad_l(L.m, c->slab_b);
        }
    }
    if (want_wgrad && c->dt != DT_F32 && garena == nullptr) {
        L.join(L.a);
        L.join(L.b);
    } else if (want_wgrad) {
        launch_conv1_wgrad(c->dt, dvp(1), x0, n0, x1, G_(di_w(1)), G_(di_b(1)), c->partial_b, Bd, c->S, c->dC[1], L.m);
        L.join(L.b);
        if (L.tail_wait) L.wait(L.m, L.tail_wait);
        L.join(L.a);
    }
    if (want_dimage)
        launch_conv1_dgrad_tanh(c->dt, dvp(1), c->d_w1t, x0, c->dpre, Bd, c->S, c->dC[1], L.m);
}

static void g_backward_pass(siggan_ctx* c, Lanes& L, const float* z, int B) {
    const float gs = c->cfg.g_leaky_slope;
    const int Lg = c->Lg, S = c->S;
    int pre_rows = 0;
    for (int l = Lg; l >= 1; --l) {
        const int Hi = 4 << (l - 1), Ho = 2 * Hi, Ci = c->gC[l - 1], Co = c->gC[l];
        const int64_t R = (int64_t)B * Ho * Ho;
        hipEvent_t const ef = L.fork_event(L.a);
        if (l == Lg) {
            launch_final_bwd_reduce(c->dt, c->dpre, c->wfin_t, c->g_y[l], B, S, Co, c->g_bn[l], c->partial, c->partial_b, gs, L.m);
            launch_final_bn_bwd_apply(c->dt, c->dpre, c->wfin_t, c->g_y[l], c->g_da[l], B, S, Co, c->g_bn[l], c->partial, c->partial_b,
                                      GG(c, gi_fin_w(c)), GG(c, gi_fin_b(c)), GG(c, gi_bn_w(l)), GG(c, gi_bn_b(l)), gs, L.m, ef);
        } else
            launch_bn_bwd(c->dt, c->g_da[l], c->g_y[l], R, Co, c->g_bn[l], c->partial, GG(c, gi_bn_w(l)), GG(c, gi_bn_b(l)), 0, gs, L.m, pre_rows, ef);
        L.fork_after(L.a, ef);
        WgradArgs w; memset(&w, 0, sizeof w); w.zeros = c->zeros; w.dt = c->dt;
        w.S = c->g_a[l - 1]; w.L = c->g_da[l]; w.slab = c->slab; w.dw = GG(c, gi_up_w(l)); w.B = B; w.Cs = Ci; w.Cl = Co;
        w.lgHs = ilog2i(Hi); w.lgWs = w.lgHs; w.lgCl = ilog2i(Co); w.K = B * Hi * Hi;
        const int max_splits = (int)(c->slab_floats / ((int64_t)Ci * (16 * Co + 1)));
        launch_wgrad(w, max_splits, L.a);
        GConvArgs a = gconv_args(c);
        a.in = c->g_da[l]; a.wp = c->g_dn[l]; a.out = c->g_da[l - 1];
        a.B = B; a.Hi = Ho; a.Wi = Ho; a.Ci = Co; a.Co = Ci;
        a.lgHr = ilog2i(Hi); a.lgWr = a.lgHr; a.Ho = Hi; a.Wo = Hi; a.form = 0; a.M = B * Hi * Hi; a.epi = EPI_RAW;
        if (l >= 2) {
            a.epi = EPI_BN_BWD_STATS; a.aref = c->g_y[l - 1]; a.bnp = c->g_bn[l - 1]; a.stat0 = c->partial; a.stat_cap = PARTIAL_FLOATS;
        }
        pre_rows = launch_gconv(a, L.m);
        if (pre_rows < 0) {
            c->refused = "the Generator's input-gradient GEMM was refused: its BatchNorm-backward sums had no carve (stat_cap)";
            pre_rows = 0;
        }
    }
    if (!(c->fc_fused && launch_fc_bwd_fused(c->dt, c->g_da[0], c->fc_y, z, c->g_bn[0], GG(c, gi_fc_w()), GG(c, gi_fc_b()),
                                             GG(c, gi_bn0_w()), GG(c, gi_bn0_b()), B, c->latent, c->gC[0], gs, L.m))) {
        launch_bn_bwd(c->dt, c->g_da[0], c->fc_y, B, c->F, c->g_bn[0], c->partial, GG(c, gi_bn0_w()), GG(c, gi_bn0_b()),
                      c->gC[0], gs, L.m);
        launch_fc_wgrad(c->dt, c->g_da[0], z, GG(c, gi_fc_w()), GG(c, gi_fc_b()), B, c->latent, c->gC[0], L.m);
    }
    L.join(L.a);
}

static void make_noise(siggan_ctx* c, const float* masks, int B, int p0, int p1, hipStream_t s, uint32_t ctr_add = 0) {
    const float keep = 1.0f - c->cfg.dropout;
    int64_t sumC = 0;
    for (int l = 1; l <= c->Ld; ++l) sumC += c->dC[l];
    if (!masks) {
        float* out[8]; int64_t n[8], e0[8]; uint32_t sid[8];
        for (int l = 1; l <= c->Ld; ++l) {
            const int64_t nl = (int64_t)B * c->dC[l];
            out[l - 1] = c->d_noise[l] + p0 * nl; n[l - 1] = nl * (p1 - p0); e0[l - 1] = p0 * nl; sid[l - 1] = 16 + l;
        }
        launch_dropnoise_multi(c->Ld, out, n, e0, sid, keep, c->dev, s, ctr_add);
        return;
    }
    int64_t pre = 0;
    for (int l = 1; l <= c->Ld; ++l) {
        const int64_t n = (int64_t)B * c->dC[l];
        for (int p = p0; p < p1; ++p)
            launch_mask_to_noise(masks + (int64_t)p * B * sumC + (int64_t)B * pre, c->d_noise[l] + p * n, n, keep, s);
        pre += c->dC[l];
    }
}

static int check_hyper(const siggan_hyper* hp) {
    if (!hp) return fail(SIGGAN_E_INVALID, "null hyper-parameters");
    if (!(hp->lr >= 0.0) || !(hp->beta1 >= 0.0 && hp->beta1 < 1.0) || !(hp->beta2 >= 0.0 && hp->beta2 < 1.0) || !(hp->eps >= 0.0))
        return fail(SIGGAN_E_INVALID, "invalid Adam hyper-parameters");
    return SIGGAN_OK;
}

static const float SN_EPS = 1e-12f;

static void phase_d_grads_sn(siggan_ctx* c, Lanes& L, const PhaseKey& k) {
    const int B = k.B;
    const bool drop = c->cfg.dropout > 0.f;
    repack(c, L.m, L.m, k.g_dirty != 0, false);
    if (k.pre_real)
        L.note(hipMemcpyAsync(c->real_stage, c->staged_src, (size_t)B * c->S * c->S * sizeof(float), hipMemcpyDeviceToDevice, L.m));
    if (drop) make_noise(c, k.has_masks ? c->mask_stage : nullptr, B, 0, 2, L.m);
    const float* fake = c->img;
    if (k.variant == SIGGAN_STEP_ABLATION) {
        g_forward_pass(c, k.has_zg ? c->z_g : nullptr, B, true, c->img_g, L.m, nullptr, nullptr, 2, c->z_g);
        L.record(c->ev_gfwd, L.m);
        fake = c->img_g;
    } else {
        g_forward_pass(c, k.has_z ? c->z : nullptr, B, false, c->img, L.m, nullptr, nullptr, 1, c->z);
    }
    launch_sn_sigma(c->snt, 1, 0, SN_EPS, L.m);
    repack(c, L.m, L.m, false, true, 0);
    d_forward_rows(c, c->real_stage, 0, B, drop, L.m, c->slab_k);
    launch_sn_sigma(c->snt, 1, 1, SN_EPS, L.m);
    repack(c, L.m, L.m, false, true, 1);
    d_forward_rows(c, fake, B, B, drop, L.m, c->slab_k);
    launch_bce(c->logits, 2 * B, B, k.ls, 0.f, c->probs, c->dlogit, k.mt, 0, L.m, c->gscale);
    d_backward_pass(c, L, fake, B, fake, B, drop, true, false, BceSpec{B, 0.f, 0.f, nullptr, 0}, B, c->sn_g[1]);
    repack(c, L.m, L.m, false, true, 0);
    d_backward_pass(c, L, c->real_stage, B, c->real_stage, B, drop, true, false, BceSpec{B, k.ls, k.ls, nullptr, 0}, 0, c->sn_g[0]);
    c->snt.slot[0] = 0; c->snt.slot[1] = 1;
    launch_sn_combine(c->snt, c->sn_g[0], c->sn_g[1], c->st.d_grads, c->d_total, 2, L.m);
}

static void phase_d_grads(siggan_ctx* c, Lanes& L, const PhaseKey& k) {
    c->early_ar = false;
    if (c->sn) return phase_d_grads_sn(c, L, k);
    const int B = k.B;
    const bool drop = c->cfg.dropout > 0.f;
    const bool nolane = k.pre_real == 2 && !k.d_dirty && (!drop || c->dreal_noise2);
    const float* xreal = c->real_stage;
    if (nolane) {
        repack(c, L.m, L.m, k.g_dirty != 0, false);
        xreal = c->staged_src;
    } else {
    L.fork(L.a);
    repack(c, L.m, L.a, k.g_dirty != 0, k.d_dirty != 0);
    if (k.pre_real)
        L.note(hipMemcpyAsync(c->real_stage, c->staged_src, (size_t)B * c->S * c->S * sizeof(float), hipMemcpyDeviceToDevice, L.a));
    if (drop && !(k.pre_real == 2 && c->dreal_noise2))
        make_noise(c, k.has_masks ? c->mask_stage : nullptr, B, k.pre_real == 2 ? 1 : 0, 2, L.a);
    if (k.pre_real != 2) d_forward_rows(c, c->real_stage, 0, B, drop, L.a, c->slab_k2, true);
    }
    const float* fake = c->img;
    const bool spec_fwd = k.spec_g && k.variant != SIGGAN_STEP_ABLATION;
    const bool spec_early = spec_fwd && c->dt != DT_F32;
    hipEvent_t e_early = nullptr, e_eval = nullptr;
    if (spec_early) { e_early = L.next(); L.record(e_early, L.m); }
    if (k.variant == SIGGAN_STEP_ABLATION) {
        g_forward_pass(c, k.has_zg ? c->z_g : nullptr, B, true, c->img_g, L.m, nullptr, nullptr, 2, c->z_g);
        L.record(c->ev_gfwd, L.m);
        fake = c->img_g;
    } else {
        if (spec_fwd && !spec_early && nolane) e_eval = L.fork_event(c->s_c);
        g_forward_pass(c, k.has_z ? c->z : nullptr, B, false, c->img, L.m, nullptr, nullptr, 1, c->z, e_eval);
    }
    if (spec_early) {
        L.wait(c->s_c, e_early);
        g_forward_pass(c, k.has_zg ? c->z_g : nullptr, B, true, c->img_g, c->s_c, c->partial_c, c->slab_k3, 2, c->z_g);
        L.record(c->ev_gfwd, c->s_c);
    }
    if (!nolane) L.join(L.a);
    hipEvent_t e_spec = nullptr;
    if (spec_fwd && !spec_early) { e_spec = e_eval; if (!e_spec) { e_spec = L.next(); L.record(e_spec, L.m); } }
    const bool join_early = k.pre_real == 2 && !c->dreal_joined && drop && c->dreal_noise2;
    if (join_early) L.wait(L.m, c->ev_dreal);
    d_forward_rows(c, fake, B, B, drop, L.m, c->slab_k, true);
    if (k.pre_real == 2 && !c->dreal_joined && !join_early) L.wait(L.m, c->ev_dreal);
    c->dreal_joined = c->dreal_noise2 = false;
    if (spec_fwd && !spec_early) {
        L.wait(c->s_c, e_spec);
        g_forward_pass(c, k.has_zg ? c->z_g : nullptr, B, true, c->img_g, c->s_c, c->partial_c, c->slab_k2, 2, c->z_g);
        L.record(c->ev_gfwd, c->s_c);
    }
    c->gfwd_joined = false;
    if (spec_fwd && c->dt == DT_F32) { L.tail_wait = c->ev_gfwd; c->gfwd_joined = true; }
    d_backward_pass(c, L, xreal, B, fake, 2 * B, drop, true, false, BceSpec{B, k.ls, 0.f, k.mt, 0}, 0, nullptr, k.coll != 0);
    L.tail_wait = nullptr;
    if (spec_fwd && c->dt != DT_F32) { L.wait(L.m, c->ev_gfwd); c->gfwd_joined = true; }
}

static void phase_g_grads(siggan_ctx* c, Lanes& L, const PhaseKey& k) {
    const int B = k.B;
    const float* zg; float* img;
    const bool d_pack = !c->sn && k.d_dirty != 0;
    bool conv1_done = false;
    if (k.spec_g) {
        if (!c->gfwd_joined) L.wait(L.m, c->ev_gfwd);
        c->gfwd_joined = false;
        conv1_done = k.rode || (d_pack && k.variant != SIGGAN_STEP_ABLATION);
        repack(c, L.m, L.m, false, d_pack, 0, (conv1_done && !k.rode) ? c->img_g : nullptr, B, B);
        zg = c->z_g; img = c->img_g;
    } else {
        L.fork(L.a);
        repack(c, L.m, L.a, k.g_dirty != 0, d_pack);
        g_forward_pass(c, k.has_z ? c->z : nullptr, B, true, c->img, L.m, nullptr, nullptr, 2, c->z);
        L.join(L.a);
        zg = c->z; img = c->img;
    }
    const bool abl = k.variant == SIGGAN_STEP_ABLATION;
    const bool gdrop = abl && c->cfg.dropout > 0.f;
    if (c->sn) {
        launch_sn_sigma(c->snt, abl ? 1 : 0, 2, SN_EPS, L.m);
        repack(c, L.m, L.m, false, true, 2);
    }
    if (gdrop) {
        int64_t sumC = 0;
        for (int l = 1; l <= c->Ld; ++l) sumC += c->dC[l];
        make_noise(c, k.has_masks ? c->mask_stage + (int64_t)2 * B * sumC : nullptr, B, 0, 1, L.m);
    }
    const float gy = abl ? k.ls : 1.0f;
    const int r0g = (!abl && !c->sn) ? B : 0;
    c->g_r0 = r0g;
    const bool real_early = k.pre_real && r0g != 0;
    if (real_early) {
        const bool drop = c->cfg.dropout > 0.f;
        L.fork(c->s_c);
        if (drop) make_noise(c, nullptr, B, 0, 2, c->s_c, 1);
        c->dreal_noise2 = drop;
        d_forward_rows(c, c->staged_src, 0, B, drop, c->s_c, c->slab_k2, true);
        L.record(c->ev_dreal, c->s_c);
    }
    d_forward_rows(c, img, r0g, B, gdrop, L.m, c->slab_k, true, conv1_done);
    d_backward_pass(c, L, img, B, img, B, gdrop, false, true, BceSpec{B, gy, gy, k.mt, 1}, r0g);
    if (k.pre_real && !real_early) {
        const bool drop = c->cfg.dropout > 0.f;
        L.fork(c->s_c);
        if (drop) make_noise(c, nullptr, B, 0, 1, c->s_c, 1);
        d_forward_rows(c, c->staged_src, 0, B, drop, c->s_c, c->slab_k2, true);
        L.record(c->ev_dreal, c->s_c);
    }
    g_backward_pass(c, L, zg, B);
    if (real_early && c->dt != DT_F32) { L.wait(L.m, c->ev_dreal); c->dreal_joined = true; }
}

static void phase_apply(siggan_ctx* c, Lanes& L, const PhaseKey& k) {
    const int which = k.phase == 2 ? 1 : 0;
    float* p = which == 0 ? c->st.g_params : c->st.d_params;
    float* g = which == 0 ? c->st.g_grads : c->st.d_grads;
    float* m = which == 0 ? c->st.g_exp_avg : c->st.d_exp_avg;
    float* v = which == 0 ? c->st.g_exp_avg_sq : c->st.d_exp_avg_sq;
    float* steps = which == 0 ? c->st.g_adam_steps : c->st.d_adam_steps;
    const int64_t n = which == 0 ? c->g_total : c->d_total;
    const int nt = (int)(which == 0 ? c->g_off.size() : c->d_off.size());
    const bool clip = k.clip > 0.f;
    float gs = k.gs / c->gscale;
    if (c->comm) {
        if (c->comm_err) return;
        if (which == 1 && c->early_ar) {
            const int64_t o = c->d_off[di_w(c->Ld)];
            const int e = rccl()->AllReduce(g, g, (size_t)o, NCCL_FLOAT32, NCCL_SUM, c->comm, L.m);
            c->early_ar = false;
            if (e != NCCL_SUCCESS) { c->comm_err = e; return; }
            L.wait(L.m, c->ev_ar);
        } else {
        const int e = rccl()->AllReduce(g, g, (size_t)n, NCCL_FLOAT32, NCCL_SUM, c->comm, L.m);
        if (e != NCCL_SUCCESS) { c->comm_err = e; return; }
        }
        gs *= 1.0f / (float)c->comm_world;
    }
    const bool guard = c->dt == DT_F16;
    if (clip || guard) launch_grad_sumsq(g, n, c->dev, c->partial, L.m);
    if (k.fused_t > 0.0 && k.pack) {
        ApTable t;
        ApRide rd; memset(&rd, 0, sizeof rd);
        if (k.ride) {
            if (!c->gfwd_joined) { L.wait(L.m, c->ev_gfwd); c->gfwd_joined = true; }
            const int64_t H = c->S >> 1;
            rd.x = c->img_g; rd.out = c->d_a[1] + (size_t)((int64_t)k.ride * H * H * c->dC[1]) * c->es; rd.B = k.ride; rd.S = c->S;
            rd.dt = c->dt; rd.slope = c->cfg.leaky_slope; rd.w_off = c->d_off[di_w(1)]; rd.b_off = c->d_off[di_b(1)];
            rd.counter = (unsigned*)c->ride_ctr; rd.late = c->ride_late_dev;
        }
        const bool ok = (which == 0 ? ap_table_g(c, t) : ap_table_d(c, t, k.ride ? k.ride * (c->S / 4) : 0)) &&
            launch_adam_pack(t, p, g, m, v, c->dev, steps, nt, k.fused_t, k.lr, k.beta1, k.beta2, k.eps, gs, k.clip,
                             k.mt + (which == 0 ? SIGGAN_M_G_GRAD_NORM : SIGGAN_M_D_GRAD_NORM), clip ? c->partial : nullptr,
                             k.mt + (which == 0 ? SIGGAN_M_G_SKIPPED : SIGGAN_M_D_SKIPPED), BN_EPS, k.ride ? &rd : nullptr, L.m);
        if (!ok) c->lane_err = hipErrorInvalidValue;
        return;
    }
    if (k.fused_t > 0.0) {
        launch_adam_fused(p, g, m, v, n, c->dev, steps, nt, k.fused_t, k.lr, k.beta1, k.beta2, k.eps, gs, k.clip,
                          k.mt + (which == 0 ? SIGGAN_M_G_GRAD_NORM : SIGGAN_M_D_GRAD_NORM), clip ? c->partial : nullptr, L.m,
                          k.mt + (which == 0 ? SIGGAN_M_G_SKIPPED : SIGGAN_M_D_SKIPPED));
        return;
    }
    launch_adam_prepare(c->dev, steps, nt, k.lr, k.beta1, k.beta2, gs, k.clip,
                        k.mt + (which == 0 ? SIGGAN_M_G_GRAD_NORM : SIGGAN_M_D_GRAD_NORM), L.m, guard ? 1 : 0,
                        k.mt + (which == 0 ? SIGGAN_M_G_SKIPPED : SIGGAN_M_D_SKIPPED), (clip || guard) ? c->partial : nullptr);
    launch_adam(p, g, m, v, n, c->dev, k.beta1, k.beta2, k.eps, (clip || gs != 1.0f) ? 1 : 0, L.m);
}

static void run_phase_body(siggan_ctx* c, Lanes& L, const PhaseKey& k) {
    if (k.phase == 0) phase_d_grads(c, L, k);
    else if (k.phase == 1) phase_g_grads(c, L, k);
    else phase_apply(c, L, k);
}

static int run_phase(siggan_ctx* c, const PhaseKey& k, hipStream_t u) {
    if (c->refused) return lane_check(c);
    const bool overlap = (c->mode & SIGGAN_MODE_OVERLAP) != 0;
    const bool graph = (c->mode & SIGGAN_MODE_GRAPH) != 0 && g_prof == nullptr;
    if (graph && c->comm && k.phase >= 2) return fail(SIGGAN_E_STATE, "SIGGAN_MODE_GRAPH is not available with a communicator");
    if (graph && c->sn) return fail(SIGGAN_E_STATE, "SIGGAN_MODE_GRAPH is not available with spectral normalisation");
    if (!graph) {
        const bool ext = overlap && g_prof == nullptr;
        Lanes L{c, u, overlap ? c->s_a : u, overlap ? c->s_b : u, ext, nullptr};
        run_phase_body(c, L, k);
        LAUNCHCHK();
        return lane_check(c);
    }
    hipGraphExec_t exec = nullptr;
    for (auto& e : c->graphs)
        if (e.first == k) { exec = e.second; break; }
    if (!exec) {
        Lanes L{c, c->s_m, overlap ? c->s_a : c->s_m, overlap ? c->s_b : c->s_m, false, nullptr};
        hipGraph_t g = nullptr;
        HIPCHK(hipStreamBeginCapture(c->s_m, hipStreamCaptureModeRelaxed));
        run_phase_body(c, L, k);
        hipError_t e1 = hipStreamEndCapture(c->s_m, &g);
        if (e1 != hipSuccess || !g) return fail(SIGGAN_E_HIP, "stream capture failed: %s", hipGetErrorString(e1));
        if (c->refused) { (void)hipGraphDestroy(g); return lane_check(c); }
        hipError_t e2 = hipGraphInstantiate(&exec, g, nullptr, nullptr, 0);
        (void)hipGraphDestroy(g);
        if (e2 != hipSuccess) return fail(SIGGAN_E_HIP, "hipGraphInstantiate: %s", hipGetErrorString(e2));
        if (c->graphs.size() >= 64) { (void)hipGraphExecDestroy(c->graphs.front().second); c->graphs.erase(c->graphs.begin()); }
        c->graphs.emplace_back(k, exec);
    }
    hipEvent_t e_in = c->ev_bridge[0], e_out = c->ev_bridge[1];
    HIPCHK(hipEventRecord(e_in, u));
    HIPCHK(hipStreamWaitEvent(c->s_m, e_in, 0));
    HIPCHK(hipGraphLaunch(exec, c->s_m));
    HIPCHK(hipEventRecord(e_out, c->s_m));
    HIPCHK(hipStreamWaitEvent(u, e_out, 0));
    return SIGGAN_OK;
}

static PhaseKey make_key(siggan_ctx* c, int phase, int B, bool has_z, bool has_masks, const siggan_hyper* hp,
                         float* metrics_dev) {
    PhaseKey k; memset(&k, 0, sizeof k);
    k.phase = phase; k.B = B; k.has_z = has_z; k.has_masks = has_masks;
    k.mt = metrics_dev ? metrics_dev : c->metrics;
    if (phase <= 1) { k.g_dirty = c->g_dirty; k.d_dirty = c->d_dirty; k.ls = hp->label_smoothing; }
    else {
        k.lr = hp->lr; k.beta1 = hp->beta1; k.beta2 = hp->beta2; k.eps = hp->eps;
        k.clip = hp->clip_max_norm > 0.f ? hp->clip_max_norm : 0.f;
        k.gs = hp->grad_scale > 0.f ? hp->grad_scale : 1.0f;
    }
    return k;
}

static int finish_metrics(siggan_ctx* c, float* metrics_dev, float* metrics_host, hipStream_t s) {
    if (metrics_host) {
        HIPCHK(hipMemcpyAsync(metrics_host, metrics_dev ? metrics_dev : c->metrics, SIGGAN_M_COUNT * sizeof(float),
                              hipMemcpyDeviceToHost, s));
        HIPCHK(hipStreamSynchronize(s));
    }
    return SIGGAN_OK;
}

extern "C" int siggan_set_step_variant(siggan_ctx* c, int32_t variant) {
    if (!c) return fail(SIGGAN_E_INVALID, "null context");
    if (variant != SIGGAN_STEP_TRAINER && variant != SIGGAN_STEP_ABLATION) return fail(SIGGAN_E_INVALID, "unknown step variant %d", variant);
    if (c->g_fwd_pending || c->pending) return fail(SIGGAN_E_STATE, "a step is in flight");
    c->variant = variant;
    return SIGGAN_OK;
}

extern "C" int siggan_set_mode(siggan_ctx* c, int32_t mode) {
    if (!c) return fail(SIGGAN_E_INVALID, "null context");
    c->mode = mode;
    return SIGGAN_OK;
}

extern "C" int siggan_g_forward(siggan_ctx* c, const float* z_dev, int32_t batch, int32_t training, float* images_dev,
                                void* stream) {
    ENTER(c);
    int rc = check_call(c, batch);
    if (rc) return rc;
    if (training && (rc = check_bn_batch(c, batch))) return rc;
    if (!z_dev || !images_dev) return fail(SIGGAN_E_INVALID, "null tensor");
    hipStream_t s = (hipStream_t)stream;
    if ((rc = settle(c, s))) return rc;
    repack(c, s, s, c->g_dirty, !c->sn && c->d_dirty);
    c->g_dirty = false; if (!c->sn) c->d_dirty = false;
    g_forward_pass(c, z_dev, batch, training != 0, images_dev, s);
    if (training) c->g_dirty = true;
    LAUNCHCHK();
    return lane_check(c);
}

extern "C" int siggan_d_forward(siggan_ctx* c, const float* x_dev, int32_t batch, int32_t training, const float* masks_dev,
                                float* probs_dev, float* features_dev, void* stream) {
    ENTER(c);
    int rc = check_call(c, batch);
    if (rc) return rc;
    if (!x_dev || (!probs_dev && !features_dev)) return fail(SIGGAN_E_INVALID, "null tensor");
    hipStream_t s = (hipStream_t)stream;
    drop_dreal(c);
    c->conv1_rode = 0;
    if ((rc = settle(c, s))) return rc;
    if (c->sn) launch_sn_sigma(c->snt, training != 0, 2, SN_EPS, s);
    repack(c, s, s, c->g_dirty, c->sn || c->d_dirty, 2);
    c->g_dirty = c->d_dirty = false;
    const bool drop = training != 0 && c->cfg.dropout > 0.f;
    if (drop) { if (!masks_dev) launch_tick(c->dev, s); make_noise(c, masks_dev, batch, 0, 1, s); }
    d_forward_rows(c, x_dev, 0, batch, drop, s, c->slab_k);
    if (probs_dev) launch_bce(c->logits, batch, batch, 0.f, 0.f, probs_dev, nullptr, nullptr, 0, s);
    if (features_dev) launch_cls_features(c->dt, c->d_a[c->Ld], features_dev, batch, c->dC[c->Ld], s);
    LAUNCHCHK();
    return lane_check(c);
}

static int d_grads_common(siggan_ctx* c, const float* real_dev, int32_t batch, const float* z_dev, const float* masks_dev,
                          const siggan_hyper* hp, float* metrics_dev, void* stream, bool spec_g, const float* zg_dev,
                          bool apply_follows = false) {
    ENTER(c);
    int rc = check_call(c, batch);
    if (rc) return rc;
    if ((rc = check_hyper(hp))) return rc;
    if (!real_dev && c->staged_B != batch)
        return fail(SIGGAN_E_INVALID, "null real batch (and no batch of %d images staged by siggan_stage_real)", batch);
    if (!c->st.d_grads) return fail(SIGGAN_E_STATE, "gradient arena was not bound");
    if (c->g_fwd_pending) return fail(SIGGAN_E_STATE, "siggan_step_begin must be followed by siggan_g_grads before the next D step");
    if (spec_g && ((c->mode & SIGGAN_MODE_OVERLAP) == 0 || (c->mode & SIGGAN_MODE_GRAPH) != 0 || g_prof != nullptr)) spec_g = false;
    const bool abl = c->variant == SIGGAN_STEP_ABLATION;
    if (c->sn && !abl) spec_g = false;
    if (batch == 1 && !abl) spec_g = false;
    if (abl) {
        if ((rc = check_bn_batch(c, batch))) return rc;
        if (zg_dev) return fail(SIGGAN_E_INVALID, "the ablation step has one latent batch per iteration: pass it as z_dev");
        zg_dev = z_dev; z_dev = nullptr; spec_g = true;
    }
    hipStream_t s = (hipStream_t)stream;
    const int B = batch;
    const size_t img_bytes = (size_t)B * c->S * c->S * sizeof(float);
    int pre_real = 0;
    if (!real_dev) pre_real = (c->dreal_B == B && !masks_dev) ? 2 : 1;
    if (pre_real == 2) c->dreal_B = 0;
    else drop_dreal(c);
    if ((rc = settle(c, s))) return rc;
    if (real_dev && real_dev != c->real_stage) HIPCHK(hipMemcpyAsync(c->real_stage, real_dev, img_bytes, hipMemcpyDeviceToDevice, s));
    c->staged_B = 0;
    if (z_dev && z_dev != c->z) HIPCHK(hipMemcpyAsync(c->z, z_dev, (size_t)B * c->latent * sizeof(float), hipMemcpyDeviceToDevice, s));
    int64_t sumC = 0;
    for (int l = 1; l <= c->Ld; ++l) sumC += c->dC[l];
    if (masks_dev) HIPCHK(hipMemcpyAsync(c->mask_stage, masks_dev, (size_t)(abl ? 3 : 2) * B * sumC * sizeof(float), hipMemcpyDeviceToDevice, s));
    c->abl_masks = abl && masks_dev != nullptr;
    if (zg_dev) HIPCHK(hipMemcpyAsync(c->z_g, zg_dev, (size_t)B * c->latent * sizeof(float), hipMemcpyDeviceToDevice, s));
    c->zg_stash = (!spec_g && zg_dev) ? B : 0;
    PhaseKey k = make_key(c, 0, B, z_dev != nullptr, masks_dev != nullptr, hp, metrics_dev);
    c->metrics_last = k.mt;
    k.spec_g = spec_g; k.has_zg = spec_g && zg_dev != nullptr; k.pre_real = pre_real; k.variant = c->variant;
    k.coll = apply_follows && c->comm != nullptr && (c->mode & SIGGAN_MODE_GRAPH) == 0;
    if ((rc = run_phase(c, k, s))) return rc;
    c->g_dirty = c->d_dirty = false;
    if (spec_g) { c->g_fwd_pending = B; c->g_dirty = true; }
    c->pending = 1;
    return SIGGAN_OK;
}

extern "C" int siggan_stage_real(siggan_ctx* c, const float* real_dev, int32_t batch, void* stream) {
    ENTER(c);
    int rc = check_call(c, batch);
    if (rc) return rc;
    if (!real_dev) return fail(SIGGAN_E_INVALID, "null real batch");
    drop_dreal(c);
    if ((rc = settle(c, (hipStream_t)stream))) return rc;
    c->staged_src = real_dev;
    c->staged_B = batch;
    return SIGGAN_OK;
}

extern "C" int siggan_d_grads(siggan_ctx* c, const float* real_dev, int32_t batch, const float* z_dev, const float* masks_dev,
                              const siggan_hyper* hp, float* metrics_dev, void* stream) {
    return d_grads_common(c, real_dev, batch, z_dev, masks_dev, hp, metrics_dev, stream, false, nullptr);
}

extern "C" int siggan_step_begin(siggan_ctx* c, const float* real_dev, int32_t batch, const float* z_dev, const float* masks_dev,
                                 const float* zg_dev, const siggan_hyper* hp, float* metrics_dev, void* stream) {
    return d_grads_common(c, real_dev, batch, z_dev, masks_dev, hp, metrics_dev, stream, true, zg_dev, true);
}

static int apply_common(siggan_ctx* c, int which, const siggan_hyper* hp, float* metrics_dev, float* metrics_host, void* stream) {
    ENTER(c);
    int rc = check_call(c, 1);
    if (rc) return rc;
    if ((rc = check_hyper(hp))) return rc;
    if (c->pending != (which == 1 ? 1 : 2))
        return fail(SIGGAN_E_STATE, "siggan_%c_apply without a preceding siggan_%c_grads", which ? 'd' : 'g', which ? 'd' : 'g');
    const float* need[] = {which ? c->st.d_grads : c->st.g_grads, which ? c->st.d_exp_avg : c->st.g_exp_avg,
                           which ? c->st.d_exp_avg_sq : c->st.g_exp_avg_sq, which ? c->st.d_adam_steps : c->st.g_adam_steps};
    for (const float* p : need)
        if (!p) return fail(SIGGAN_E_STATE, "gradient / Adam arenas were not bound");
    hipStream_t s = (hipStream_t)stream;
    if ((rc = settle(c, s))) return rc;
    if (!metrics_dev) metrics_dev = c->metrics_last != c->metrics ? c->metrics_last : nullptr;
    else if (c->metrics_last && metrics_dev != c->metrics_last)
        HIPCHK(hipMemcpyAsync(metrics_dev, c->metrics_last, SIGGAN_M_COUNT * sizeof(float), hipMemcpyDeviceToDevice, (hipStream_t)stream));
    PhaseKey k = make_key(c, which == 1 ? 2 : 3, 0, false, false, hp, metrics_dev);
    const int wi = which == 1 ? 1 : 0;
    if ((c->mode & SIGGAN_MODE_GRAPH) == 0 && c->dt != DT_F16) {
        if (!c->adam_t_known[wi]) {
            float t0 = 0.f;
            HIPCHK(hipStreamSynchronize(s));
            HIPCHK(hipMemcpy(&t0, which == 1 ? c->st.d_adam_steps : c->st.g_adam_steps, sizeof t0, hipMemcpyDeviceToHost));
            c->adam_t[wi] = (double)t0; c->adam_t_known[wi] = true;
        }
        k.fused_t = c->adam_t[wi] + 1.0;
        ApTable probe;
        k.pack = (which == 0 ? ap_table_g(c, probe) : ap_table_d(c, probe, 0)) ? 1 : 0;
        if (which == 1 && k.pack && c->g_fwd_pending && c->variant != SIGGAN_STEP_ABLATION && g_prof == nullptr && c->dt == DT_F32)
            k.ride = c->g_fwd_pending;
    } else {
        c->adam_t_known[wi] = false;
    }
    if ((rc = run_phase(c, k, s))) return rc;
    if (k.fused_t > 0.0) c->adam_t[wi] = k.fused_t;
    if (which == 0) c->g_dirty = !k.pack; else c->d_dirty = !k.pack;
    if (which == 1) c->conv1_rode = k.ride;
    c->pending = 0;
    return finish_metrics(c, metrics_dev, metrics_host, s);
}

extern "C" int siggan_d_apply(siggan_ctx* c, const siggan_hyper* hp, float* metrics_dev, float* metrics_host, void* stream) {
    return apply_common(c, 1, hp, metrics_dev, metrics_host, stream);
}

extern "C" int siggan_d_step(siggan_ctx* c, const float* real_dev, int32_t batch, const float* z_dev, const float* masks_dev,
                             const siggan_hyper* hp, float* metrics_dev, float* metrics_host, void* stream) {
    int rc = d_grads_common(c, real_dev, batch, z_dev, masks_dev, hp, metrics_dev, stream, false, nullptr, true);
    if (rc) return rc;
    return siggan_d_apply(c, hp, metrics_dev, metrics_host, stream);
}

extern "C" int siggan_g_grads(siggan_ctx* c, int32_t batch, const float* z_dev, const siggan_hyper* hp, float* metrics_dev,
                              void* stream) {
    ENTER(c);
    int rc = check_call(c, batch);
    if (rc) return rc;
    if ((rc = check_bn_batch(c, batch))) return rc;
    if ((rc = check_hyper(hp))) return rc;
    if (!c->st.g_grads) return fail(SIGGAN_E_STATE, "gradient arena was not bound");
    hipStream_t s = (hipStream_t)stream;
    if ((rc = settle(c, s))) return rc;
    const int B = batch;
    const bool spec = c->g_fwd_pending != 0;
    if (c->variant == SIGGAN_STEP_ABLATION && !spec)
        return fail(SIGGAN_E_STATE, "ablation step: siggan_g_grads follows the siggan_d_grads / siggan_d_apply of the same iteration");
    if (spec && (c->g_fwd_pending != B || z_dev))
        return fail(SIGGAN_E_STATE, "siggan_g_grads after siggan_step_begin must use the same batch and no explicit z (pass it to step_begin)");
    if (!spec && !z_dev && c->zg_stash == B) z_dev = c->z_g;
    c->zg_stash = 0;
    if (!spec && z_dev && z_dev != c->z) HIPCHK(hipMemcpyAsync(c->z, z_dev, (size_t)B * c->latent * sizeof(float), hipMemcpyDeviceToDevice, s));
    PhaseKey k = make_key(c, 1, B, z_dev != nullptr, false, hp, metrics_dev);
    c->metrics_last = k.mt;
    k.spec_g = spec; k.variant = c->variant; k.has_masks = c->abl_masks;
    k.rode = (spec && c->conv1_rode == B && !c->d_dirty) ? 1 : 0;
    c->conv1_rode = 0;
    c->abl_masks = false;
    k.pre_real = c->staged_B == B && c->dreal_B == 0 && (c->mode & SIGGAN_MODE_OVERLAP) != 0 && (c->mode & SIGGAN_MODE_GRAPH) == 0 &&
                 g_prof == nullptr && c->pending == 0 && !c->sn;
    if ((rc = run_phase(c, k, s))) return rc;
    c->g_rode = k.rode ? B : 0; c->g_pre_real = k.pre_real ? B : 0;
    if (k.pre_real) c->dreal_B = B;
    c->g_fwd_pending = 0;
    c->d_dirty = false;
    c->g_dirty = true;
    c->pending = 2;
    return SIGGAN_OK;
}

extern "C" int siggan_g_apply(siggan_ctx* c, const siggan_hyper* hp, float* metrics_dev, float* metrics_host, void* stream) {
    return apply_common(c, 0, hp, metrics_dev, metrics_host, stream);
}

extern "C" int siggan_g_step(siggan_ctx* c, int32_t batch, const float* z_dev, const siggan_hyper* hp, float* metrics_dev,
                             float* metrics_host, void* stream) {
    int rc = siggan_g_grads(c, batch, z_dev, hp, metrics_dev, stream);
    if (rc) return rc;
    return siggan_g_apply(c, hp, metrics_dev, metrics_host, stream);
}

static bool pow2(int v) { return v > 0 && (v & (v - 1)) == 0; }

extern "C" int siggan_op_conv4x4s2(siggan_ctx* c, int32_t form, const void* in_dev, const float* w_dev, void* out_dev,
                                   int32_t batch, int32_t h_in, int32_t c_in, int32_t c_out, void* stream) {
    if (!c) return fail(SIGGAN_E_INVALID, "null context");
    if (!in_dev || !w_dev || !out_dev) return fail(SIGGAN_E_INVALID, "null tensor");
    if (form != 0 && form != 1) return fail(SIGGAN_E_INVALID, "form must be 0 (down) or 1 (up)");
    if (!pow2(h_in) || !pow2(c_in) || !pow2(c_out) || c_in < 32 || c_out < 32 || c_in > 512 || c_out > 512 || batch < 1)
        return fail(SIGGAN_E_INVALID, "shape not in the model family (pow2 dims, 32 <= C <= 512)");
    if (form == 0 && h_in < 2) return fail(SIGGAN_E_INVALID, "down form needs h_in >= 2");
    DevGuard dg_(c->cfg.device); HIPCHK(dg_.err);
    hipStream_t s = (hipStream_t)stream;
    GConvArgs a = gconv_args(c);
    a.in = in_dev; a.wp = c->op_pack; a.out = out_dev; a.B = batch; a.Hi = h_in; a.Wi = h_in; a.Ci = c_in; a.Co = c_out;
    a.form = form; a.epi = EPI_RAW;
    PrepTable t; t.njobs = 0; t.overflow = 0;
    PrepJob j; memset(&j, 0, sizeof j);
    j.src = w_dev; j.dst = (float*)c->op_pack; j.dt = c->dt;
    if (form == 0) {
        j.type = PREP_PACK_DOWN; j.O = c_out; j.I = c_in;
        a.Ho = a.Wo = h_in / 2; a.lgHr = a.lgWr = ilog2i(h_in / 2); a.M = batch * (h_in / 2) * (h_in / 2);
    } else {
        j.type = PREP_PACK_UP; j.I = c_in; j.O = c_out;
        a.Ho = a.Wo = 2 * h_in; a.lgHr = a.lgWr = ilog2i(h_in); a.M = batch * h_in * h_in;
    }
    prep_add(t, j, (long long)c_in * c_out * 16);
    if (!launch_prepare(t, BN_EPS, s)) return fail(SIGGAN_E_STATE, "prepare table overflow");
    launch_gconv(a, s);
    LAUNCHCHK();
    return SIGGAN_OK;
}

extern "C" int siggan_op_conv4x4s2_wgrad(siggan_ctx* c, const void* small_dev, const void* large_dev, float* dw_dev,
                                         int32_t batch, int32_t h_small, int32_t c_small, int32_t c_large, void* stream) {
    if (!c) return fail(SIGGAN_E_INVALID, "null context");
    if (!small_dev || !large_dev || !dw_dev) return fail(SIGGAN_E_INVALID, "null tensor");
    if (!pow2(h_small) || !pow2(c_small) || !pow2(c_large) || c_small < 32 || c_large < 32 || c_small > 512 || c_large > 512 ||
        batch < 1)
        return fail(SIGGAN_E_INVALID, "shape not in the model family (pow2 dims, 32 <= C <= 512)");
    DevGuard dg_(c->cfg.device); HIPCHK(dg_.err);
    hipStream_t s = (hipStream_t)stream;
    WgradArgs w; memset(&w, 0, sizeof w); w.zeros = c->zeros; w.dt = c->dt;
    w.S = small_dev; w.L = large_dev; w.slab = c->slab; w.dw = dw_dev; w.B = batch; w.Cs = c_small; w.Cl = c_large;
    w.lgHs = w.lgWs = ilog2i(h_small); w.lgCl = ilog2i(c_large); w.K = batch * h_small * h_small;
    const int max_splits = (int)(c->slab_floats / ((int64_t)c_small * (16 * c_large + 1)));
    launch_wgrad(w, max_splits, s);
    LAUNCHCHK();
    return SIGGAN_OK;
}

extern "C" int siggan_op_adam(siggan_ctx* c, float* p, float* g, float* m, float* v, int64_t n, int32_t step,
                              const siggan_hyper* hp, void* stream) {
    if (!c) return fail(SIGGAN_E_INVALID, "null context");
    int rc = check_hyper(hp);
    if (rc) return rc;
    if (!p || !g || !m || !v || n < 1 || step < 1) return fail(SIGGAN_E_INVALID, "bad argument");
    if ((((uintptr_t)p | (uintptr_t)g | (uintptr_t)m | (uintptr_t)v) & 15) != 0) return fail(SIGGAN_E_INVALID, "arenas must be 16-byte aligned");
    DevGuard dg_(c->cfg.device); HIPCHK(dg_.err);
    hipStream_t s = (hipStream_t)stream;
    float* steps = c->partial + ((2 << 20) - 64);
    const float prev = (float)(step - 1);
    HIPCHK(hipMemcpyAsync(steps, &prev, sizeof prev, hipMemcpyHostToDevice, s));
    const bool clip = hp->clip_max_norm > 0.f;
    const float gs = hp->grad_scale > 0.f ? hp->grad_scale : 1.0f;
    if (clip) launch_grad_sumsq(g, n, c->dev, c->partial, s);
    launch_adam_prepare(c->dev, steps, 1, hp->lr, hp->beta1, hp->beta2, gs, hp->clip_max_norm, nullptr, s, 0, nullptr,
                        clip ? c->partial : nullptr);
    launch_adam(p, g, m, v, n, c->dev, hp->beta1, hp->beta2, hp->eps, (clip || gs != 1.0f) ? 1 : 0, s);
    LAUNCHCHK();
    return SIGGAN_OK;
}

extern "C" int siggan_comm_unique_id(void* id_out) {
    if (!id_out) return fail(SIGGAN_E_INVALID, "null argument");
    Rccl* r = rccl();
    if (r->err) return fail(SIGGAN_E_STATE, "%s", r->err);
    ncclUniqueId_t id;
    NCCLCHK(r->GetUniqueId(&id));
    memcpy(id_out, &id, sizeof id);
    return SIGGAN_OK;
}
extern "C" int siggan_comm_init(siggan_ctx* c, int32_t rank, int32_t world, const void* id) {
    ENTER(c);
    if (!id || world < 1 || rank < 0 || rank >= world) return fail(SIGGAN_E_INVALID, "bad rank / world / id");
    if (c->comm) return fail(SIGGAN_E_STATE, "a communicator is already initialised");
    Rccl* r = rccl();
    if (r->err) return fail(SIGGAN_E_STATE, "%s", r->err);
    ncclUniqueId_t uid;
    memcpy(&uid, id, sizeof uid);
    NCCLCHK(r->CommInitRank(&c->comm, world, uid, rank));
    c->comm_rank = rank; c->comm_world = world;
    return SIGGAN_OK;
}
extern "C" int siggan_comm_destroy(siggan_ctx* c) {
    ENTER(c);
    if (!c->comm) return SIGGAN_OK;
    HIPCHK(hipDeviceSynchronize());
    NCCLCHK(rccl()->CommDestroy(c->comm));
    c->comm = nullptr; c->comm_rank = 0; c->comm_world = 1; c->comm_err = 0; c->early_ar = false;
    return SIGGAN_OK;
}
extern "C" int32_t siggan_comm_world(const siggan_ctx* c) { return c ? c->comm_world : -1; }
extern "C" int siggan_comm_broadcast(siggan_ctx* c, void* buf_dev, int64_t bytes, int32_t root, void* stream) {
    ENTER(c);
    if (!buf_dev || bytes < 1 || root < 0 || root >= c->comm_world) return fail(SIGGAN_E_INVALID, "bad argument");
    if (!c->comm) return SIGGAN_OK;
    NCCLCHK(rccl()->Broadcast(buf_dev, buf_dev, (size_t)bytes, NCCL_CHAR, root, c->comm, (hipStream_t)stream));
    return SIGGAN_OK;
}

extern "C" int siggan_device_info(int32_t device, int32_t* compute_units, int32_t* clock_khz, int64_t* hbm_bytes) {
    if (!compute_units || !clock_khz || !hbm_bytes) return fail(SIGGAN_E_INVALID, "null argument");
    hipDeviceProp_t p;
    HIPCHK(hipGetDeviceProperties(&p, device));
    *compute_units = p.multiProcessorCount; *clock_khz = p.clockRate; *hbm_bytes = (int64_t)p.totalGlobalMem;
    return SIGGAN_OK;
}

static Prof g_prof_store;
extern "C" int siggan_prof_enable(siggan_ctx* c, int32_t on) {
    if (!c) return fail(SIGGAN_E_INVALID, "null context");
    DevGuard dg_(c->cfg.device); HIPCHK(dg_.err);
    HIPCHK(hipDeviceSynchronize());
    g_prof_store.clear();
    g_prof = on ? &g_prof_store : nullptr;
    return SIGGAN_OK;
}
extern "C" int32_t siggan_prof_slots(void) { return Prof::NID - 1; }
extern "C" int siggan_prof_read(siggan_ctx* c, int32_t idx, char* name, int32_t name_cap, int64_t* launches, double* ms,
                                double* flops, double* bytes) {
    if (!c || !name || !launches || !ms || !flops || !bytes || idx < 0 || idx >= Prof::NID - 1) return fail(SIGGAN_E_INVALID, "bad argument");
    DevGuard dg_(c->cfg.device); HIPCHK(dg_.err);
    HIPCHK(hipDeviceSynchronize());
    snprintf(name, name_cap, "%s", Prof::name(idx));
    *launches = 0; *ms = 0.0; *flops = 0.0; *bytes = 0.0;
    for (auto& r : g_prof_store.recs) {
        if (r.id != idx) continue;
        float t = 0.f;
        HIPCHK(hipEventElapsedTime(&t, r.e0, r.e1));
        *launches += 1; *ms += t; *flops += r.flops; *bytes += r.bytes;
    }
    return SIGGAN_OK;
}

extern "C" int siggan_prof_launch(siggan_ctx* c, int64_t idx, int32_t* fields, int32_t n, int64_t* count) {
    if (!c || !count || (n > 0 && !fields)) return fail(SIGGAN_E_INVALID, "bad argument");
    *count = (int64_t)g_prof_store.recs.size();
    if (n <= 0) return SIGGAN_OK;
    if (idx < 0 || idx >= *count) return fail(SIGGAN_E_INVALID, "launch %lld of %lld", (long long)idx, (long long)*count);
    const Prof::Rec& r = g_prof_store.recs[(size_t)idx];
    const int32_t v[7] = {r.id, r.form, r.epi_req, r.epi, r.M, r.Ci, r.Co};
    for (int i = 0; i < n && i < 7; ++i) fields[i] = v[i];
    return SIGGAN_OK;
}

extern "C" int siggan_debug_tensor(siggan_ctx* c, const char* name, int32_t idx, float* out_dev, int64_t n, void* stream) {
    if (!c || !name || !out_dev || n < 1) return fail(SIGGAN_E_INVALID, "bad argument");
    const void* src = nullptr; int64_t capv = 0;
    const void** ptr = &src; int64_t* cap = &capv;
    bool typed = true;
    const int64_t Bm = c->Bm, Bd = 2 * Bm, SS = (int64_t)c->S * c->S;
    auto gsz = [&](int l) { const int64_t H = 4 << l; return Bm * H * H * c->gC[l]; };
    auto dsz = [&](int l) { const int64_t H = c->S >> l; return Bd * H * H * c->dC[l]; };
    const bool gl = idx >= 0 && idx <= c->Lg, dl = idx >= 1 && idx <= c->Ld;
    if (!strcmp(name, "g_y") && gl) { *ptr = c->g_y[idx]; *cap = gsz(idx); }
    else if (!strcmp(name, "g_a") && gl) { *ptr = c->g_a[idx]; *cap = gsz(idx); }
    else if (!strcmp(name, "g_da") && gl) { *ptr = c->g_da[idx]; *cap = gsz(idx); }
    else if (!strcmp(name, "d_a") && dl) { *ptr = c->d_a[idx]; *cap = dsz(idx); }
    else if (!strcmp(name, "d_dv") && dl) { *ptr = c->d_dv[idx]; *cap = dsz(idx); }
    else if (!strcmp(name, "d_a_g") && dl) {
        const int64_t H = c->S >> idx, off = (int64_t)c->g_r0 * H * H * c->dC[idx];
        *ptr = c->d_a[idx] + (size_t)off * c->es; *cap = dsz(idx) - off;
    }
    else if (!strcmp(name, "z")) { *ptr = c->z; *cap = Bm * c->latent; typed = false; }
    else if (!strcmp(name, "z_g")) { *ptr = c->z_g; *cap = Bm * c->latent; typed = false; }
    else if (!strcmp(name, "img")) { *ptr = c->img; *cap = Bm * SS; typed = false; }
    else if (!strcmp(name, "dpre")) { *ptr = c->dpre; *cap = Bm * SS; typed = false; }
    else if (!strcmp(name, "logits")) { *ptr = c->logits; *cap = Bd; typed = false; }
    else if (!strcmp(name, "probs")) { *ptr = c->probs; *cap = Bd; typed = false; }
    else if (!strcmp(name, "dlogit")) { *ptr = c->dlogit; *cap = Bd; typed = false; }
    else if (!strcmp(name, "d_noise") && dl) { *ptr = c->d_noise[idx]; *cap = Bd * c->dC[idx]; typed = false; }
    else if (!strcmp(name, "rode") || !strcmp(name, "pre_real") || !strcmp(name, "ride_late")) {
        if (n != 1) return fail(SIGGAN_E_INVALID, "debug scalar %s holds 1 float, %lld asked", name, (long long)n);
        DevGuard dg_(c->cfg.device); HIPCHK(dg_.err);
        HIPCHK(hipStreamSynchronize((hipStream_t)stream));
        const float v = !strcmp(name, "rode") ? (float)c->g_rode : !strcmp(name, "pre_real") ? (float)c->g_pre_real
                                                                                               : (float)__atomic_load_n(c->ride_late, __ATOMIC_ACQUIRE);
        HIPCHK(hipMemcpy(out_dev, &v, sizeof v, hipMemcpyHostToDevice));
        return SIGGAN_OK;
    }
    else return fail(SIGGAN_E_INVALID, "unknown debug tensor %s[%d]", name, idx);
    if (n > capv) return fail(SIGGAN_E_INVALID, "debug tensor %s[%d] holds %lld floats, %lld asked", name, idx, (long long)capv, (long long)n);
    DevGuard dg_(c->cfg.device); HIPCHK(dg_.err);
    if (!strcmp(name, "g_a") && idx == c->Lg && c->ga_last_B) {
        const int64_t H = c->S;
        HIPCHK(hipDeviceSynchronize());
        launch_bn_relu(c->dt, c->g_y[idx], c->g_a[idx], (int64_t)c->ga_last_B * H * H, c->gC[idx], c->g_bn[idx], c->cfg.g_leaky_slope,
                       (hipStream_t)stream);
        LAUNCHCHK();
    }
    if (typed && c->dt != DT_F32) { launch_to_f32(c->dt, src, out_dev, n, (hipStream_t)stream); LAUNCHCHK(); }
    else HIPCHK(hipMemcpyAsync(out_dev, src, (size_t)n * sizeof(float), hipMemcpyDeviceToDevice, (hipStream_t)stream));
    return SIGGAN_OK;
}

extern "C" int siggan_augment_batch(int32_t device, const uint8_t* cache_dev, int64_t n_images, const int32_t* index_dev,
                                    const int32_t* params_dev, const int16_t* tables_dev, const float* lut_dev, float* out_dev,
                                    int32_t batch, int32_t size, int32_t augment, int32_t fill, void* stream) {
    if (!cache_dev || !index_dev || !lut_dev || !out_dev) return fail(SIGGAN_E_INVALID, "null tensor");
    if (augment && (!params_dev || !tables_dev)) return fail(SIGGAN_E_INVALID, "augment needs params and tables");
    if (batch < 1 || n_images < 1 || size < 1 || size > 1024) return fail(SIGGAN_E_INVALID, "bad batch / cache / image size");
    if (fill < 0 || fill > 255) return fail(SIGGAN_E_INVALID, "fill must be a byte value");
    DevGuard dg_(device); HIPCHK(dg_.err);
    launch_augment(cache_dev, n_images, index_dev, params_dev, tables_dev, lut_dev, out_dev, batch, size, augment != 0, fill, (hipStream_t)stream);
    LAUNCHCHK();
    return SIGGAN_OK;
}

extern "C" int siggan_op_randn(siggan_ctx* c, float* out_dev, int64_t n, void* stream) {
    if (!c || !out_dev || n < 1) return fail(SIGGAN_E_INVALID, "bad argument");
    DevGuard dg_(c->cfg.device); HIPCHK(dg_.err);
    hipStream_t s = (hipStream_t)stream;
    launch_tick(c->dev, s);
    launch_randn(out_dev, n, c->dev, 3, s);
    LAUNCHCHK();
    return SIGGAN_OK;
}
```

Baseline: 43750 images/s.

## Run discriminator real-half backward on side stream during generator step

While the generator step runs, the discriminator's backward pass for the real-image rows of the next step is computed early on a side stream. Per-layer weight gradients are split into two K halves, either as separate slab ranges or with register-carry accumulators, so the fake half can finish the job later. The dgrad conv gains a cfg_M override so the row-subset launch picks the same tiling as the full batch. This adds dedicated slab memory, events, key fields and validity checks on label smoothing, dirtiness and the per-layer mode, which raises the risk of stale or mismatched gradients.

```diff
diff --git a/include/siggan.h b/include/siggan.h
--- a/include/siggan.h
+++ b/include/siggan.h
@@ -121,6 +121,13 @@
 int siggan_op_conv4x4s2_wgrad(siggan_ctx *ctx, const void *small_dev, const void *large_dev,
                               float *dw_dev, int32_t batch, int32_t h_small, int32_t c_small,
                               int32_t c_large, void *stream);
+int siggan_op_conv4x4s2_rows(siggan_ctx *ctx, const void *in_dev, const float *w_dev, void *out_dev,
+                             int32_t batch, int32_t cfg_batch, int32_t h_in, int32_t c_in, int32_t c_out,
+                             void *stream);
+int siggan_op_conv4x4s2_wgrad_halves(siggan_ctx *ctx, const void *small_dev, const void *large_dev,
+                                     float *dw_dev, float *db_dev, int32_t batch, int32_t h_small,
+                                     int32_t c_small, int32_t c_large, int32_t halves, int32_t *mode_out,
+                                     void *stream);
 int siggan_op_adam(siggan_ctx *ctx, float *p_dev, float *g_dev, float *m_dev, float *v_dev,
                    int64_t n, int32_t step, const siggan_hyper *hp, void *stream);
 int siggan_op_randn(siggan_ctx *ctx, float *out_dev, int64_t n, void *stream);
diff --git a/signature-gan_amd/_lib.py b/signature-gan_amd/_lib.py
--- a/signature-gan_amd/_lib.py
+++ b/signature-gan_amd/_lib.py
@@ -77,6 +77,8 @@
     "siggan_g_apply": (C.c_int, [_P, C.POINTER(Hyper), _P, _P, _P]),
     "siggan_op_conv4x4s2": (C.c_int, [_P, _I32, _P, _P, _P, _I32, _I32, _I32, _I32, _P]),
     "siggan_op_conv4x4s2_wgrad": (C.c_int, [_P, _P, _P, _P, _I32, _I32, _I32, _I32, _P]),
+    "siggan_op_conv4x4s2_rows": (C.c_int, [_P, _P, _P, _P, _I32, _I32, _I32, _I32, _I32, _P]),
+    "siggan_op_conv4x4s2_wgrad_halves": (C.c_int, [_P, _P, _P, _P, _P, _I32, _I32, _I32, _I32, _I32, C.POINTER(_I32), _P]),
     "siggan_op_adam": (C.c_int, [_P, _P, _P, _P, _P, _I64, _I32, C.POINTER(Hyper), _P]),
     "siggan_op_randn": (C.c_int, [_P, _P, _I64, _P]),
     "siggan_augment_batch": (C.c_int, [_I32, _P, _I64, _P, _P, _P, _P, _P, _I32, _I32, _I32, _I32, _P]),
diff --git a/signature-gan_amd/csrc/gconv.h b/signature-gan_amd/csrc/gconv.h
--- a/signature-gan_amd/csrc/gconv.h
+++ b/signature-gan_amd/csrc/gconv.h
@@ -43,6 +43,7 @@
     int64_t slab_floats;
     size_t slab_stride;
     const float* zeros;
+    int cfg_M;
 };
 
 struct BnBwdParams { f32x4 sc, sf, mu, rs; };
@@ -78,6 +79,8 @@
     int K;
     int kchunk;
     const float* zeros;
+    int z0, nz;
+    float* carry;
 };
 
 struct Prof {
@@ -98,5 +101,9 @@
 void launch_gconv16(int cfg, const GConvArgs& a, dim3 grid, hipStream_t st, hipEvent_t e0, hipEvent_t e1, int kq = 1);
 void launch_wgrad16(bool small, const WgradArgs& a, dim3 grid, hipStream_t st, hipEvent_t e0, hipEvent_t e1);
 int launch_wgrad(WgradArgs a, int max_splits, hipStream_t st);
+enum { WG_HALF_NONE = 0, WG_HALF_SLABS = 1, WG_HALF_CARRY = 2 };
+int wgrad_half_mode(const WgradArgs& a, int max_splits);
+int64_t wgrad_half_floats(const WgradArgs& a, int max_splits);
+int launch_wgrad_half(WgradArgs a, int max_splits, int half, hipStream_t st);
 
 }
diff --git a/signature-gan_amd/csrc/gconv.hip b/signature-gan_amd/csrc/gconv.hip
--- a/signature-gan_amd/csrc/gconv.hip
+++ b/signature-gan_amd/csrc/gconv.hip
@@ -586,7 +586,8 @@
     GConvArgs a = a_in;
     if (a.epi == EPI_BN_BWD_STATS && (a.stat0 == nullptr || a.stat_cap <= 0)) return -1;
     const int ncls = a.form == 0 ? 1 : 4;
-    auto blocks = [&](int bm, int bn) { return ((a.M + bm - 1) / bm) * (a.Co / bn) * ncls; };
+    const int Mc = a.cfg_M > 0 ? a.cfg_M : a.M;
+    auto blocks = [&](int bm, int bn) { return ((Mc + bm - 1) / bm) * (a.Co / bn) * ncls; };
     const int nk = (a.form == 0 ? 16 : 4) * (a.Ci / BK);
     auto splits = [&](int nblk) {
         int ns = 1;
@@ -594,7 +595,7 @@
             ns = (512 + nblk - 1) / nblk;
             if (ns > nk / 4) ns = nk / 4;
             if (ns > 8) ns = 8;
-            const int64_t out_floats = (int64_t)a.B * a.Ho * a.Wo * a.Co;
+            const int64_t out_floats = (int64_t)(Mc >> (a.lgHr + a.lgWr)) * a.Ho * a.Wo * a.Co;
             if (ns > 1 && (int64_t)ns * out_floats > a.slab_floats) ns = (int)(a.slab_floats / out_floats);
             if (ns < 1) ns = 1;
         }
@@ -609,7 +610,7 @@
         return launch_cfg<64, 64, 2, 2, 32, 1>(a, st, 2, ns);
     }
     if (a.dt == DT_F32 && a.form == 1 && a.Co == 32 && (a.epi == EPI_RAW || a.epi == EPI_AFFINE_RELU) && (a.Ci == 32 || a.Ci == 64) &&
-        a.M / 128 >= (a.Ci == 32 ? 384 : 768) && a.M % 128 == 0 &&
+        Mc / 128 >= (a.Ci == 32 ? 384 : 768) && a.M % 128 == 0 && Mc % 128 == 0 &&
         ((1 << (a.lgHr + a.lgWr)) % 128) == 0 && a.lgWr >= 4 && a.lgWr <= 6) {
         dim3 grid(a.M / 128);
         if (g_prof) {
@@ -630,7 +631,8 @@
     return launch_cfg<128, 32, 4, 1, 32, 1>(a, st, 3, ns);
 }
 
-template <int BM, int BN, int WM, int WN>
+enum { WG_WHOLE = 0, WG_RANGE = 1, WG_CARRY_OUT = 2, WG_CARRY_IN = 3 };
+template <int BM, int BN, int WM, int WN, int MODE = WG_WHOLE>
 __global__ __launch_bounds__(256) void k_wgrad(const WgradArgs a) {
     constexpr int TM = BM / (32 * WM), TN = BN / (32 * WN);
     constexpr int LDA = BM + PAD, LDB = BN + PAD;
@@ -704,11 +706,26 @@
         for (int j = 0; j < TN; ++j)
 #pragma unroll
             for (int r = 0; r < 16; ++r) acc[i][j][r] = 0.f;
+    f32x4* const cacc = (MODE == WG_CARRY_IN || MODE == WG_CARRY_OUT)
+                            ? reinterpret_cast<f32x4*>(a.carry + ((size_t)bx * 256 + tid) * (TM * TN * 16)) : nullptr;
+    if constexpr (MODE == WG_CARRY_IN) {
+#pragma unroll
+        for (int i = 0; i < TM; ++i)
+#pragma unroll
+            for (int j = 0; j < TN; ++j)
+#pragma unroll
+                for (int q = 0; q < 4; ++q) {
+                    const f32x4 v = cacc[(i * TN + j) * 4 + q];
+#pragma unroll
+                    for (int e = 0; e < 4; ++e) acc[i][j][4 * q + e] = v[e];
+                }
+    }
 
     constexpr int NQ = 256 / BM, KQ = BK / NQ;
     const bool bias_blk = a.db != nullptr && j0 == 0;
     const int bcol = tid % BM, kq = tid / BM;
     float bsum = 0.f;
+    if constexpr (MODE == WG_CARRY_IN) { if (bias_blk) bsum = a.carry[(size_t)a.Cs * N + (size_t)(i0 / BM) * 256 + tid]; }
 #define WG_TILE(BUF, ST, LD)                                                                          \
     {                                                                                                 \
         if (bias_blk) {                                                                               \
@@ -772,6 +789,19 @@
 
 #undef WG_LOAD_TILE
 #undef WG_STORE_TILE
+    if constexpr (MODE == WG_CARRY_OUT) {
+        if (bias_blk) a.carry[(size_t)a.Cs * N + (size_t)(i0 / BM) * 256 + tid] = bsum;
+#pragma unroll
+        for (int i = 0; i < TM; ++i)
+#pragma unroll
+            for (int j = 0; j < TN; ++j)
+#pragma unroll
+                for (int q = 0; q < 4; ++q)
+                    cacc[(i * TN + j) * 4 + q] = f32x4{acc[i][j][4 * q], acc[i][j][4 * q + 1], acc[i][j][4 * q + 2], acc[i][j][4 * q + 3]};
+        return;
+    }
+    const int nz = MODE == WG_RANGE ? a.nz : (int)gridDim.z, zs = MODE == WG_RANGE ? bz + a.z0 : bz;
+    const bool direct = MODE != WG_RANGE && gridDim.z == 1;
     if (bias_blk) {
         smem[kq * BM + bcol] = bsum;
         __syncthreads();
@@ -779,11 +809,11 @@
             float t = smem[tid];
 #pragma unroll
             for (int q = 1; q < NQ; ++q) t += smem[q * BM + tid];
-            if (gridDim.z == 1) a.db[i0 + tid] = t;
-            else a.slab[(size_t)gridDim.z * a.Cs * N + (size_t)bz * a.Cs + i0 + tid] = t;
-        }
-    }
-    if (gridDim.z == 1 && a.dw) {
+            if (direct) a.db[i0 + tid] = t;
+            else a.slab[(size_t)nz * a.Cs * N + (size_t)zs * a.Cs + i0 + tid] = t;
+        }
+    }
+    if (direct && a.dw) {
 #pragma unroll
         for (int i = 0; i < TM; ++i)
 #pragma unroll
@@ -797,7 +827,7 @@
             }
         return;
     }
-    float* const out = a.slab + (size_t)bz * a.Cs * N;
+    float* const out = a.slab + (size_t)zs * a.Cs * N;
 #pragma unroll
     for (int i = 0; i < TM; ++i)
 #pragma unroll
@@ -811,20 +841,30 @@
 
 static void launch_wgrad_reduce(const float* slab, float* dw, float* db, int nsplit, int Cs, int Cl, hipStream_t st);
 
-int launch_wgrad(WgradArgs a, int max_splits, hipStream_t st) {
+struct WgradPlan { bool small; int tiles, nsplit, kchunk; };
+static WgradPlan wgrad_plan(const WgradArgs& a, int max_splits) {
     const int N = 16 << a.lgCl;
-    const bool small = a.Cs < 64;
-    const int tiles = small ? (N / 128) : (a.Cs / 64) * (N / 64);
+    WgradPlan p;
+    p.small = a.Cs < 64;
+    p.tiles = p.small ? (N / 128) : (a.Cs / 64) * (N / 64);
     int ktiles = (a.K + BK - 1) / BK;
-    int nsplit = (512 + tiles - 1) / tiles;
+    int nsplit = (512 + p.tiles - 1) / p.tiles;
     if (nsplit > ktiles / 4) nsplit = ktiles / 4;
     if (nsplit > max_splits) nsplit = max_splits;
     if (nsplit < 1) nsplit = 1;
     int per = (ktiles + nsplit - 1) / nsplit;
-    a.kchunk = per * BK;
-    nsplit = (ktiles + per - 1) / per;
+    p.kchunk = per * BK;
+    p.nsplit = (ktiles + per - 1) / per;
+    return p;
+}
+
+int launch_wgrad(WgradArgs a, int max_splits, hipStream_t st) {
+    const WgradPlan pl = wgrad_plan(a, max_splits);
+    const bool small = pl.small;
+    const int tiles = pl.tiles, nsplit = pl.nsplit;
+    a.kchunk = pl.kchunk;
     dim3 grid(tiles, 1, nsplit);
-    if (g_prof) g_prof->begin(small ? 6 : 4, 2.0 * a.Cs * (double)N * a.K, wgrad_bytes(a), st);
+    if (g_prof) g_prof->begin(small ? 6 : 4, 2.0 * a.Cs * (double)(16 << a.lgCl) * a.K, wgrad_bytes(a), st);
     hipEvent_t e0 = g_prof ? g_prof->recs.back().e0 : nullptr, e1 = g_prof ? g_prof->recs.back().e1 : nullptr;
     if (a.dt != DT_F32) {
         launch_wgrad16(small, a, grid, st, e0, e1);
@@ -838,6 +878,38 @@
     }
     if (nsplit > 1) launch_wgrad_reduce(a.slab, a.dw, a.db, nsplit, a.Cs, 1 << a.lgCl, st);
     return nsplit;
+}
+
+int wgrad_half_mode(const WgradArgs& a, int max_splits) {
+    if (a.dt != DT_F32 || a.Cs < 64 || (a.B & 1) || a.B < 2 || a.K < 2 || (a.K & 1)) return WG_HALF_NONE;
+    const WgradPlan pl = wgrad_plan(a, max_splits);
+    const int Kh = a.K / 2;
+    if (pl.nsplit == 1) return Kh % BK == 0 ? WG_HALF_CARRY : WG_HALF_NONE;
+    if ((pl.nsplit & 1) == 0 && (int64_t)Kh == (int64_t)(pl.nsplit / 2) * pl.kchunk) return WG_HALF_SLABS;
+    return WG_HALF_NONE;
+}
+int64_t wgrad_half_floats(const WgradArgs& a, int max_splits) {
+    const WgradPlan pl = wgrad_plan(a, max_splits);
+    return (int64_t)pl.nsplit * a.Cs * ((16 << a.lgCl) + 1) + 4 * (int64_t)a.Cs;
+}
+int launch_wgrad_half(WgradArgs a, int max_splits, int half, hipStream_t st) {
+    const int mode = wgrad_half_mode(a, max_splits);
+    if (mode == WG_HALF_NONE) return mode;
+    const WgradPlan pl = wgrad_plan(a, max_splits);
+    const int Kh = a.K / 2, Cl = 1 << a.lgCl;
+    a.S = static_cast<const float*>(a.S) + (size_t)half * Kh * a.Cs;
+    a.L = static_cast<const float*>(a.L) + (size_t)half * Kh * 4 * Cl;
+    a.K = Kh; a.B /= 2;
+    if (mode == WG_HALF_SLABS) {
+        a.kchunk = pl.kchunk; a.nz = pl.nsplit; a.z0 = half * (pl.nsplit / 2);
+        hipLaunchKernelGGL((k_wgrad<64, 64, 2, 2, WG_RANGE>), dim3(pl.tiles, 1, pl.nsplit / 2), dim3(256), 0, st, a);
+        if (half) launch_wgrad_reduce(a.slab, a.dw, a.db, pl.nsplit, a.Cs, Cl, st);
+    } else {
+        a.kchunk = Kh; a.carry = a.slab;
+        if (half) hipLaunchKernelGGL((k_wgrad<64, 64, 2, 2, WG_CARRY_IN>), dim3(pl.tiles, 1, 1), dim3(256), 0, st, a);
+        else hipLaunchKernelGGL((k_wgrad<64, 64, 2, 2, WG_CARRY_OUT>), dim3(pl.tiles, 1, 1), dim3(256), 0, st, a);
+    }
+    return mode;
 }
 
 __global__ __launch_bounds__(1024) void k_wgrad_reduce(const float* __restrict__ slab, float* __restrict__ dw, float* __restrict__ db,
diff --git a/signature-gan_amd/csrc/siggan.hip b/signature-gan_amd/csrc/siggan.hip
--- a/signature-gan_amd/csrc/siggan.hip
+++ b/signature-gan_amd/csrc/siggan.hip
@@ -105,11 +105,14 @@
     int pack;
     int ride;
     int rode;
+    int dbwd;
+    float ls_d;
     float ls, clip, gs;
     bool operator==(const PhaseKey& o) const {
         return phase == o.phase && B == o.B && has_z == o.has_z && has_masks == o.has_masks && g_dirty == o.g_dirty &&
                d_dirty == o.d_dirty && spec_g == o.spec_g && has_zg == o.has_zg && pre_real == o.pre_real && variant == o.variant && coll == o.coll && mt == o.mt && lr == o.lr && beta1 == o.beta1 && beta2 == o.beta2 && eps == o.eps && ls == o.ls &&
-               clip == o.clip && gs == o.gs && fused_t == o.fused_t && pack == o.pack && ride == o.ride && rode == o.rode;
+               clip == o.clip && gs == o.gs && fused_t == o.fused_t && pack == o.pack && ride == o.ride && rode == o.rode && dbwd == o.dbwd &&
+               ls_d == o.ls_d;
     }
 };
 
@@ -168,6 +171,15 @@
     float* slab_b;
     const float* staged_src;
     int dreal_B;
+    float* dreal_slab[MAXL + 1];
+    int64_t dreal_slab_floats[MAXL + 1];
+    hipEvent_t ev_dreal_bwd;
+    int dbwd_B;
+    float dbwd_ls;
+    int dbwd_mode[MAXL + 1];
+    bool dbwd_orphan;
+    float d_ls_last; bool d_ls_known;
+    int dbwd_taken_B, dbwd_taken_mode[MAXL + 1];
     int zg_stash;
     int g_fwd_pending;
     int conv1_rode;
@@ -334,6 +346,16 @@
             carve(&c->sn_g[0], c->d_total); carve(&c->sn_g[1], c->d_total);
             carve(&c->d_w1s, (int64_t)c->dC[1] * 16);
         }
+        if (c->dt == DT_F32 && !c->sn) {
+            for (int l = 2; l <= c->Ld; ++l) {
+                const int64_t Cs = c->dC[l], N = 16 * (int64_t)c->dC[l - 1], tiles = (Cs / 64) * (N / 64);
+                int64_t ns = (512 + tiles - 1) / tiles;
+                if (ns > c->slab_floats / (Cs * (N + 1))) ns = c->slab_floats / (Cs * (N + 1));
+                if (ns < 1) ns = 1;
+                c->dreal_slab_floats[l] = ns * Cs * (N + 1) + 4 * Cs;
+                carve(&c->dreal_slab[l], c->dreal_slab_floats[l]);
+            }
+        }
         carve(&c->metrics, SIGGAN_M_COUNT);
         carve_t(&c->op_pack, (int64_t)512 * 512 * 16);
         carve(&c->zeros, 64);
@@ -364,6 +386,8 @@
     HIPCHK(hipStreamCreateWithFlags(&c->s_n, hipStreamNonBlocking));
     HIPCHK(hipEventCreateWithFlags(&c->ev_gfwd, EV_FLAGS));
     HIPCHK(hipEventCreateWithFlags(&c->ev_dreal, EV_FLAGS));
+    HIPCHK(hipEventCreateWithFlags(&c->ev_dreal_bwd, EV_FLAGS));
+    c->dbwd_B = c->dbwd_taken_B = 0; c->dbwd_orphan = false; c->d_ls_known = false;
     HIPCHK(hipEventCreateWithFlags(&c->ev_ar, hipEventDisableTiming));
     for (int i = 0; i < 2; ++i) HIPCHK(hipEventCreateWithFlags(&c->ev_sys[i], hipEventDisableTiming));
     c->early_ar = false;
@@ -403,6 +427,7 @@
     for (int i = 0; i < 2; ++i) if (c->ev_sys[i]) (void)hipEventDestroy(c->ev_sys[i]);
     if (c->ev_gfwd) (void)hipEventDestroy(c->ev_gfwd);
     if (c->ev_dreal) (void)hipEventDestroy(c->ev_dreal);
+    if (c->ev_dreal_bwd) (void)hipEventDestroy(c->ev_dreal_bwd);
     if (c->ws) (void)hipFree(c->ws);
     if (c->ride_late) (void)hipHostFree(c->ride_late);
     delete c;
@@ -432,12 +457,19 @@
 extern "C" int64_t siggan_workspace_bytes(const siggan_ctx* c) { return c ? (int64_t)c->ws_bytes : -1; }
 
 static void drop_dreal(siggan_ctx* c) {
-    if (c->dreal_B) { c->dreal_orphan = true; c->dreal_B = 0; }
+    if (c->dreal_B) {
+        c->dreal_orphan = true; c->dreal_B = 0;
+        if (c->dbwd_B) { c->dbwd_orphan = true; c->dbwd_B = 0; }
+    }
 }
 static int settle(siggan_ctx* c, hipStream_t s) {
     if (c->dreal_orphan) {
         HIPCHK(hipStreamWaitEvent(s, c->ev_dreal, 0));
         c->dreal_orphan = false;
+    }
+    if (c->dbwd_orphan) {
+        HIPCHK(hipStreamWaitEvent(s, c->ev_dreal_bwd, 0));
+        c->dbwd_orphan = false;
     }
     return SIGGAN_OK;
 }
@@ -761,9 +793,64 @@
 
 struct BceSpec { int n0; float y0, y1; float* mt; int is_g; };
 
+static WgradArgs d_wgrad_args(siggan_ctx* c, int l, int Bd, int r0, float* ga, float* slab) {
+    const int Ho = c->S >> l, Co = c->dC[l], Ci = c->dC[l - 1];
+    WgradArgs w; memset(&w, 0, sizeof w); w.zeros = c->zeros; w.dt = c->dt;
+    w.S = c->d_dv[l] + (size_t)((int64_t)r0 * Ho * Ho * Co) * c->es;
+    w.L = c->d_a[l - 1] + (size_t)((int64_t)r0 * 4 * Ho * Ho * Ci) * c->es;
+    w.slab = slab; w.dw = ga + c->d_off[di_w(l)]; w.B = Bd; w.Cs = Co; w.Cl = Ci;
+    w.lgHs = ilog2i(Ho); w.lgWs = w.lgHs; w.lgCl = ilog2i(Ci); w.K = Bd * Ho * Ho;
+    w.db = ga + c->d_off[di_b(l)];
+    return w;
+}
+static int d_wgrad_max_splits(const siggan_ctx* c, int l) {
+    return (int)(c->slab_floats / ((int64_t)c->dC[l] * (16 * c->dC[l - 1] + 1)));
+}
+static GConvArgs d_dgrad_args(siggan_ctx* c, int l, int Bd, int r0, bool dropout, int cfg_B = 0) {
+    const int Ho = c->S >> l, Hi = 2 * Ho, Co = c->dC[l], Ci = c->dC[l - 1];
+    GConvArgs a = gconv_args(c);
+    a.in = c->d_dv[l] + (size_t)((int64_t)r0 * Ho * Ho * Co) * c->es; a.wp = c->d_up[l];
+    a.out = c->d_dv[l - 1] + (size_t)((int64_t)r0 * Hi * Hi * Ci) * c->es;
+    a.B = Bd; a.Hi = Ho; a.Wi = Ho; a.Ci = Co; a.Co = Ci;
+    a.lgHr = ilog2i(Ho); a.lgWr = a.lgHr; a.Ho = Hi; a.Wo = Hi; a.form = 1; a.M = Bd * Ho * Ho; a.cfg_M = cfg_B * Ho * Ho;
+    a.epi = EPI_LRELU_BWD; a.aref = c->d_a[l - 1] + (size_t)((int64_t)r0 * Hi * Hi * Ci) * c->es;
+    a.noise = dropout ? c->d_noise[l - 1] + (int64_t)r0 * Ci : nullptr; a.slope = c->cfg.leaky_slope;
+    return a;
+}
+
+static bool dreal_bwd_rule(siggan_ctx* c, int B, int* modes) {
+    for (int l = 0; l <= MAXL; ++l) modes[l] = WG_HALF_NONE;
+    if (c->dt != DT_F32 || c->sn || c->comm || c->variant != SIGGAN_STEP_TRAINER || g_prof != nullptr ||
+        (c->mode & SIGGAN_MODE_OVERLAP) == 0 || (c->mode & SIGGAN_MODE_GRAPH) != 0 || c->Ld < 2 || !c->dreal_slab[2])
+        return false;
+    for (int l = 2; l <= c->Ld; ++l) {
+        const WgradArgs w = d_wgrad_args(c, l, 2 * B, 0, c->st.d_grads, c->dreal_slab[l]);
+        const int ms = d_wgrad_max_splits(c, l);
+        modes[l] = wgrad_half_mode(w, ms);
+        if (modes[l] == WG_HALF_NONE || wgrad_half_floats(w, ms) > c->dreal_slab_floats[l]) {
+            for (int k = 0; k <= MAXL; ++k) modes[k] = WG_HALF_NONE;
+            return false;
+        }
+    }
+    return true;
+}
+static void d_backward_real_half(siggan_ctx* c, hipStream_t s, int B, float ls) {
+    const int Ld = c->Ld;
+    const bool drop = c->cfg.dropout > 0.f;
+    const int P = c->lP[0];
+    launch_cls_bwd(c->dt, c->logits, B, ls, ls, c->wcp, c->d_a[Ld], drop ? c->d_noise[Ld] : nullptr, c->cfg.leaky_slope, c->d_dv[Ld], B,
+                   c->dC[Ld], s, c->gscale, nullptr, nullptr, nullptr, 0, false, P ? c->lparts : nullptr, P, DP(c, di_cls_b(c)));
+    for (int l = Ld; l >= 2; --l) {
+        launch_wgrad_half(d_wgrad_args(c, l, 2 * B, 0, c->st.d_grads, c->dreal_slab[l]), d_wgrad_max_splits(c, l), 0, s);
+        GConvArgs a = d_dgrad_args(c, l, B, 0, drop, 2 * B);
+        a.slab = c->slab_k2;
+        launch_gconv(a, s);
+    }
+}
+
 static void d_backward_pass(siggan_ctx* c, Lanes& L, const float* x0, int n0, const float* x1, int Bd, bool dropout,
                             bool want_wgrad, bool want_dimage, const BceSpec& bce, int r0 = 0, float* garena = nullptr,
-                            bool early_allreduce = false) {
+                            bool early_allreduce = false, bool staged_real = false) {
     const float slope = c->cfg.leaky_slope;
     const int Ld = c->Ld;
     float* const ga = garena ? garena : c->st.d_grads;
@@ -777,27 +864,35 @@
     if (P < 0) { c->lane_err = hipErrorInvalidValue; return; }
     const float* const parts = P ? c->lparts + (size_t)r0 * P : nullptr;
     const float* const bc = DP(c, di_cls_b(c));
+    const int rch = staged_real ? bce.n0 : r0, Bc = staged_real ? Bd - bce.n0 : Bd;
+    auto act_c = [&](int l) { const int64_t H = c->S >> l; return c->d_a[l] + (size_t)((int64_t)rch * H * H * c->dC[l]) * c->es; };
+    auto dvp_c = [&](int l) { const int64_t H = c->S >> l; return c->d_dv[l] + (size_t)((int64_t)rch * H * H * c->dC[l]) * c->es; };
     if (sb != L.m) {
         L.fork(L.b);
         launch_bce(c->logits + r0, Bd, bce.n0, bce.y0, bce.y1, c->probs + r0, c->dlogit + r0, bce.mt, bce.is_g, sb, c->gscale, parts, P, bc);
     }
+    if (staged_real)
+        launch_cls_bwd(c->dt, c->logits + rch, Bc, bce.y1, bce.y1, c->wcp, act_c(Ld), dropout ? c->d_noise[Ld] + (int64_t)rch * c->dC[Ld] : nullptr,
+                       slope, dvp_c(Ld), Bc, c->dC[Ld], L.m, c->gscale, nullptr, nullptr, nullptr, 0, false,
+                       P ? c->lparts + (size_t)rch * P : nullptr, P, bc);
+    else
     launch_cls_bwd(c->dt, c->logits + r0, bce.n0, bce.y0, bce.y1, c->wcp, act(Ld), nz(Ld), slope, dvp(Ld), Bd,
                    c->dC[Ld], L.m, c->gscale, c->probs + r0, c->dlogit + r0, bce.mt, bce.is_g, sb == L.m, parts, P, bc);
     if (want_wgrad)
         launch_cls_wgrad(c->dt, c->dlogit + r0, act(Ld), G_(di_cls_w(c)), G_(di_cls_b(c)), Bd, c->dC[Ld], sb);
     for (int l = Ld; l >= 2; --l) {
-        const int Ho = c->S >> l, Hi = 2 * Ho, Co = c->dC[l], Ci = c->dC[l - 1];
         const bool w_main = want_wgrad && l == 2 && c->dt != DT_F32 && garena == nullptr;
         auto wgrad_l = [&](hipStream_t st, float* slab) {
-            WgradArgs w; memset(&w, 0, sizeof w); w.zeros = c->zeros; w.dt = c->dt;
-            w.S = dvp(l); w.L = act(l - 1); w.slab = slab; w.dw = G_(di_w(l)); w.B = Bd; w.Cs = Co; w.Cl = Ci;
-            w.lgHs = ilog2i(Ho); w.lgWs = w.lgHs; w.lgCl = ilog2i(Ci); w.K = Bd * Ho * Ho;
-            w.db = G_(di_b(l));
-            const int max_splits = (int)(c->slab_floats / ((int64_t)Co * (16 * Ci + 1)));
-            launch_wgrad(w, max_splits, st);
+            if (staged_real) {
+                if (launch_wgrad_half(d_wgrad_args(c, l, Bd, r0, ga, c->dreal_slab[l]), d_wgrad_max_splits(c, l), 1, st) == WG_HALF_NONE)
+                    c->refused = "the staged Discriminator backward's second weight-gradient half was refused (dreal_bwd_rule)";
+                return;
+            }
+            launch_wgrad(d_wgrad_args(c, l, Bd, r0, ga, slab), d_wgrad_max_splits(c, l), st);
         };
         if (want_wgrad && !w_main) {
             L.fork(L.a);
+            if (staged_real && l == Ld) L.wait(L.a, c->ev_dreal_bwd);
             wgrad_l(L.a, c->slab);
             if (early_allreduce && l == Ld && c->comm && !c->comm_err && garena == nullptr) {
                 hipEvent_t ea = c->ev_sys[0], eb = c->ev_sys[1];
@@ -809,12 +904,7 @@
                 else { L.record(c->ev_ar, c->s_n); c->early_ar = true; }
             }
         }
-        GConvArgs a = gconv_args(c);
-        a.in = dvp(l); a.wp = c->d_up[l]; a.out = dvp(l - 1);
-        a.B = Bd; a.Hi = Ho; a.Wi = Ho; a.Ci = Co; a.Co = Ci;
-        a.lgHr = ilog2i(Ho); a.lgWr = a.lgHr; a.Ho = Hi; a.Wo = Hi; a.form = 1; a.M = Bd * Ho * Ho;
-        a.epi = EPI_LRELU_BWD; a.aref = act(l - 1); a.noise = nz(l - 1); a.slope = slope;
-        launch_gconv(a, L.m);
+        launch_gconv(d_dgrad_args(c, l, Bc, rch, dropout, staged_real ? Bd : 0), L.m);
         if (w_main) {
             L.fork(L.b);
             launch_conv1_wgrad(c->dt, dvp(1), x0, n0, x1, G_(di_w(1)), G_(di_b(1)), c->partial_b, Bd, c->S, c->dC[1], L.b);
@@ -825,6 +915,7 @@
         L.join(L.a);
         L.join(L.b);
     } else if (want_wgrad) {
+        if (staged_real) L.wait(L.m, c->ev_dreal_bwd);
         launch_conv1_wgrad(c->dt, dvp(1), x0, n0, x1, G_(di_w(1)), G_(di_b(1)), c->partial_b, Bd, c->S, c->dC[1], L.m);
         L.join(L.b);
         if (L.tail_wait) L.wait(L.m, L.tail_wait);
@@ -941,6 +1032,7 @@
     if (c->sn) return phase_d_grads_sn(c, L, k);
     const int B = k.B;
     const bool drop = c->cfg.dropout > 0.f;
+    if (k.dbwd == 1) L.wait(L.m, c->ev_dreal_bwd);
     const bool nolane = k.pre_real == 2 && !k.d_dirty && (!drop || c->dreal_noise2);
     const float* xreal = c->real_stage;
     if (nolane) {
@@ -988,7 +1080,7 @@
     }
     c->gfwd_joined = false;
     if (spec_fwd && c->dt == DT_F32) { L.tail_wait = c->ev_gfwd; c->gfwd_joined = true; }
-    d_backward_pass(c, L, xreal, B, fake, 2 * B, drop, true, false, BceSpec{B, k.ls, 0.f, k.mt, 0}, 0, nullptr, k.coll != 0);
+    d_backward_pass(c, L, xreal, B, fake, 2 * B, drop, true, false, BceSpec{B, k.ls, 0.f, k.mt, 0}, 0, nullptr, k.coll != 0, k.dbwd == 2);
     L.tail_wait = nullptr;
     if (spec_fwd && c->dt != DT_F32) { L.wait(L.m, c->ev_gfwd); c->gfwd_joined = true; }
 }
@@ -1033,6 +1125,10 @@
         c->dreal_noise2 = drop;
         d_forward_rows(c, c->staged_src, 0, B, drop, c->s_c, c->slab_k2, true);
         L.record(c->ev_dreal, c->s_c);
+        if (k.dbwd) {
+            d_backward_real_half(c, c->s_c, B, k.ls_d);
+            L.record(c->ev_dreal_bwd, c->s_c);
+        }
     }
     d_forward_rows(c, img, r0g, B, gdrop, L.m, c->slab_k, true, conv1_done);
     d_backward_pass(c, L, img, B, img, B, gdrop, false, true, BceSpec{B, gy, gy, k.mt, 1}, r0g);
@@ -1249,7 +1345,17 @@
     const size_t img_bytes = (size_t)B * c->S * c->S * sizeof(float);
     int pre_real = 0;
     if (!real_dev) pre_real = (c->dreal_B == B && !masks_dev) ? 2 : 1;
-    if (pre_real == 2) c->dreal_B = 0;
+    int dbwd = 0;
+    c->dbwd_taken_B = 0;
+    for (int l = 0; l <= MAXL; ++l) c->dbwd_taken_mode[l] = 0;
+    if (pre_real == 2 && c->dbwd_B) {
+        int modes[MAXL + 1];
+        bool use = c->dbwd_B == B && c->dbwd_ls == hp->label_smoothing && !c->d_dirty && !abl && dreal_bwd_rule(c, B, modes);
+        for (int l = 2; use && l <= c->Ld; ++l) use = modes[l] == c->dbwd_mode[l];
+        dbwd = use ? 2 : 1;
+        if (use) { c->dbwd_taken_B = B; for (int l = 2; l <= c->Ld; ++l) c->dbwd_taken_mode[l] = modes[l]; }
+    }
+    if (pre_real == 2) c->dreal_B = c->dbwd_B = 0;
     else drop_dreal(c);
     if ((rc = settle(c, s))) return rc;
     if (real_dev && real_dev != c->real_stage) HIPCHK(hipMemcpyAsync(c->real_stage, real_dev, img_bytes, hipMemcpyDeviceToDevice, s));
@@ -1263,11 +1369,12 @@
     c->zg_stash = (!spec_g && zg_dev) ? B : 0;
     PhaseKey k = make_key(c, 0, B, z_dev != nullptr, masks_dev != nullptr, hp, metrics_dev);
     c->metrics_last = k.mt;
-    k.spec_g = spec_g; k.has_zg = spec_g && zg_dev != nullptr; k.pre_real = pre_real; k.variant = c->variant;
+    k.spec_g = spec_g; k.has_zg = spec_g && zg_dev != nullptr; k.pre_real = pre_real; k.variant = c->variant; k.dbwd = dbwd;
     k.coll = apply_follows && c->comm != nullptr && (c->mode & SIGGAN_MODE_GRAPH) == 0;
     if ((rc = run_phase(c, k, s))) return rc;
     c->g_dirty = c->d_dirty = false;
     if (spec_g) { c->g_fwd_pending = B; c->g_dirty = true; }
+    c->d_ls_last = hp->label_smoothing; c->d_ls_known = true;
     c->pending = 1;
     return SIGGAN_OK;
 }
@@ -1373,9 +1480,13 @@
     c->abl_masks = false;
     k.pre_real = c->staged_B == B && c->dreal_B == 0 && (c->mode & SIGGAN_MODE_OVERLAP) != 0 && (c->mode & SIGGAN_MODE_GRAPH) == 0 &&
                  g_prof == nullptr && c->pending == 0 && !c->sn;
+    int modes[MAXL + 1];
+    k.dbwd = (k.pre_real && c->variant == SIGGAN_STEP_TRAINER && c->d_ls_known && !c->d_dirty && dreal_bwd_rule(c, B, modes)) ? 1 : 0;
+    k.ls_d = k.dbwd ? c->d_ls_last : 0.f;
     if ((rc = run_phase(c, k, s))) return rc;
     c->g_rode = k.rode ? B : 0; c->g_pre_real = k.pre_real ? B : 0;
     if (k.pre_real) c->dreal_B = B;
+    if (k.dbwd) { c->dbwd_B = B; c->dbwd_ls = k.ls_d; for (int l = 0; l <= MAXL; ++l) c->dbwd_mode[l] = modes[l]; }
     c->g_fwd_pending = 0;
     c->d_dirty = false;
     c->g_dirty = true;
@@ -1444,6 +1555,56 @@
     return SIGGAN_OK;
 }
 
+extern "C" int siggan_op_conv4x4s2_rows(siggan_ctx* c, const void* in_dev, const float* w_dev, void* out_dev, int32_t batch,
+                                        int32_t cfg_batch, int32_t h_in, int32_t c_in, int32_t c_out, void* stream) {
+    if (!c) return fail(SIGGAN_E_INVALID, "null context");
+    if (!in_dev || !w_dev || !out_dev) return fail(SIGGAN_E_INVALID, "null tensor");
+    if (!pow2(h_in) || !pow2(c_in) || !pow2(c_out) || c_in < 64 || c_out < 64 || c_in > 512 || c_out > 512 || batch < 1 || cfg_batch < batch)
+        return fail(SIGGAN_E_INVALID, "shape not in the Discriminator's family (pow2 dims, 64 <= C <= 512, cfg_batch >= batch)");
+    DevGuard dg_(c->cfg.device); HIPCHK(dg_.err);
+    hipStream_t s = (hipStream_t)stream;
+    GConvArgs a = gconv_args(c);
+    a.in = in_dev; a.wp = c->op_pack; a.out = out_dev; a.B = batch; a.Hi = h_in; a.Wi = h_in; a.Ci = c_in; a.Co = c_out;
+    a.form = 1; a.epi = EPI_RAW;
+    a.Ho = a.Wo = 2 * h_in; a.lgHr = a.lgWr = ilog2i(h_in); a.M = batch * h_in * h_in; a.cfg_M = cfg_batch * h_in * h_in;
+    PrepTable t; t.njobs = 0; t.overflow = 0;
+    PrepJob j; memset(&j, 0, sizeof j);
+    j.src = w_dev; j.dst = (float*)c->op_pack; j.dt = c->dt; j.type = PREP_PACK_UP; j.I = c_in; j.O = c_out;
+    prep_add(t, j, (long long)c_in * c_out * 16);
+    if (!launch_prepare(t, BN_EPS, s)) return fail(SIGGAN_E_STATE, "prepare table overflow");
+    launch_gconv(a, s);
+    LAUNCHCHK();
+    return SIGGAN_OK;
+}
+
+extern "C" int siggan_op_conv4x4s2_wgrad_halves(siggan_ctx* c, const void* small_dev, const void* large_dev, float* dw_dev,
+                                                float* db_dev, int32_t batch, int32_t h_small, int32_t c_small, int32_t c_large,
+                                                int32_t halves, int32_t* mode_out, void* stream) {
+    if (!c) return fail(SIGGAN_E_INVALID, "null context");
+    if (!small_dev || !large_dev || !dw_dev || !db_dev || !mode_out) return fail(SIGGAN_E_INVALID, "null tensor");
+    if (!pow2(h_small) || !pow2(c_small) || !pow2(c_large) || c_small < 64 || c_large < 32 || c_small > 512 || c_large > 512 ||
+        batch < 2 || (batch & 1))
+        return fail(SIGGAN_E_INVALID, "shape not in the model family (pow2 dims, 64 <= Cs <= 512, 32 <= Cl <= 512, an even batch)");
+    if (c->dt != DT_F32) return fail(SIGGAN_E_STATE, "the two-launch weight gradient is an fp32 path");
+    DevGuard dg_(c->cfg.device); HIPCHK(dg_.err);
+    hipStream_t s = (hipStream_t)stream;
+    WgradArgs w; memset(&w, 0, sizeof w); w.zeros = c->zeros; w.dt = c->dt;
+    w.S = small_dev; w.L = large_dev; w.slab = c->slab; w.dw = dw_dev; w.db = db_dev; w.B = batch; w.Cs = c_small; w.Cl = c_large;
+    w.lgHs = w.lgWs = ilog2i(h_small); w.lgCl = ilog2i(c_large); w.K = batch * h_small * h_small;
+    const int max_splits = (int)(c->slab_floats / ((int64_t)c_small * (16 * c_large + 1)));
+    *mode_out = wgrad_half_mode(w, max_splits);
+    if (!halves) {
+        launch_wgrad(w, max_splits, s);
+    } else {
+        if (*mode_out == WG_HALF_NONE) return fail(SIGGAN_E_STATE, "this problem's K split has no two-launch form");
+        if (wgrad_half_floats(w, max_splits) > c->slab_floats) return fail(SIGGAN_E_STATE, "the slab region is too small for this problem");
+        launch_wgrad_half(w, max_splits, 0, s);
+        launch_wgrad_half(w, max_splits, 1, s);
+    }
+    LAUNCHCHK();
+    return SIGGAN_OK;
+}
+
 extern "C" int siggan_op_adam(siggan_ctx* c, float* p, float* g, float* m, float* v, int64_t n, int32_t step,
                               const siggan_hyper* hp, void* stream) {
     if (!c) return fail(SIGGAN_E_INVALID, "null context");
@@ -1575,6 +1736,14 @@
     else if (!strcmp(name, "probs")) { *ptr = c->probs; *cap = Bd; typed = false; }
     else if (!strcmp(name, "dlogit")) { *ptr = c->dlogit; *cap = Bd; typed = false; }
     else if (!strcmp(name, "d_noise") && dl) { *ptr = c->d_noise[idx]; *cap = Bd * c->dC[idx]; typed = false; }
+    else if (!strcmp(name, "dreal_bwd")) {
+        if (n != 1 || idx < 0 || idx > c->Ld || idx == 1) return fail(SIGGAN_E_INVALID, "debug scalar dreal_bwd[%d]: index 0 or a block 2..%d, 1 float", idx, c->Ld);
+        DevGuard dg_(c->cfg.device); HIPCHK(dg_.err);
+        HIPCHK(hipStreamSynchronize((hipStream_t)stream));
+        const float v = idx == 0 ? (float)c->dbwd_taken_B : (float)c->dbwd_taken_mode[idx];
+        HIPCHK(hipMemcpy(out_dev, &v, sizeof v, hipMemcpyHostToDevice));
+        return SIGGAN_OK;
+    }
     else if (!strcmp(name, "rode") || !strcmp(name, "pre_real") || !strcmp(name, "ride_late")) {
         if (n != 1) return fail(SIGGAN_E_INVALID, "debug scalar %s holds 1 float, %lld asked", name, (long long)n);
         DevGuard dg_(c->cfg.device); HIPCHK(dg_.err);
```

After: 42840 images/s. 0.979x the previous value.
